# ogulcanaydogan/llm-slo-ebpf-toolkit

Measured on AMD Instinct MI355X. Metric: fault-replay attribution throughput through the agent's BPF-ring -> GPU path (events/s, node-wide); held-out attribution macro-F1 and agent CPU overhead % reported alongside, higher is better.
Workload: dtype fp64 posteriors / fp32 features (exact-int64 time joins)

## Files before the change

llm_slo_ebpf_toolkit_amd/ops/csrc/agent_bindings.cpp:

```cpp
#include <pybind11/numpy.h>
#include <pybind11/pybind11.h>
#include <pybind11/stl.h>

#include <cstring>
#include <memory>
#include <stdexcept>

#include "decodesli.h"
#include "drift.h"
#include "engine.h"
#include "errsli.h"
#include "exemplars.h"
#include "loadsli.h"
#include "satcurve.h"
#include "onset.h"
#include "openreq.h"
#include "podrank.h"
#include "retrsli.h"
#include "slisketch.h"

namespace py = pybind11;
using namespace mislo;

namespace {
// ... 1285 lines not shown
  });
  m.def("loadsli_device_bytes", [](int bins, int64_t span_cap, int group_cap) {
    return loadsli::device_bytes(bins, (int)span_cap, group_cap);
  });
  m.def("loadsli_ring_records_max", [](int bins, int64_t bin_us) { return loadsli::default_ring_records_max(bins, bin_us); });
  py::class_<PyLoadSliTracker>(m, "LoadSliTracker")
      .def(py::init<int, int64_t, int64_t, int64_t, int64_t, int64_t, int64_t, int64_t, int64_t, int64_t, int, int, int64_t,
                    bool>(),
           py::arg("device") = 0, py::arg("bins") = 1024, py::arg("bin_us") = 500000, py::arg("settle_bins") = 30,
           py::arg("recent_bins") = 30, py::arg("min_base_bins") = 60, py::arg("factor_milli") = 1500,
           py::arg("min_requests") = 20, py::arg("min_conc_milli") = 1000, py::arg("span_cap") = 16384,
           py::arg("group_cap") = 64, py::arg("n_buffers") = 3,
           py::arg("ring_records_max") = loadsli::default_ring_records_max(1024, 500000), py::arg("lds") = true)
      .def("step", &PyLoadSliTracker::step, py::arg("spans"), py::arg("cut_ns"), py::arg("n_groups"))
      .def("query", &PyLoadSliTracker::query)
      .def("results", &PyLoadSliTracker::results)
      .def("block", &PyLoadSliTracker::block)
      .def("step_ms", &PyLoadSliTracker::step_ms)
      .def("resident", &PyLoadSliTracker::resident)
      .def("sync", &PyLoadSliTracker::sync)
      .def("close", &PyLoadSliTracker::close);
  m.attr("SATCURVE_ROW_BYTES") = satcurve::kRowBytes;
  m.attr("SATCURVE_STATS") = (int)satcurve::kStats;
  m.attr("SATCURVE_LEVELS") = satcurve::kK;
  m.attr("SATCURVE_LDS_SLOTS") = satcurve::kLdsSlots;
  m.attr("SATCURVE_BINS") = py::make_tuple(satcurve::kMinBins, satcurve::kMaxBins);
  m.attr("SATCURVE_CURVE_RECORDS_MAX") = satcurve::kMaxCurveRecords;
  m.def("satcurve_level", [](int64_t busy_us, int64_t span_us) {
    if (span_us < 1) throw std::invalid_argument("saturation curve level: empty span");
    const uint32_t u = satcurve::u_of(busy_us, span_us);
    return py::make_tuple(u, satcurve::level_of_u(u));
  });
  m.def("satcurve_lower", [](uint32_t level) { return satcurve::lower_u(level); });
  m.def("satcurve_knee", [](py::array_t<uint64_t, py::array::c_style | py::array::forcecast> curve, int64_t budget_ppm,
                            int64_t min_requests) {
    if (curve.size() != satcurve::kK * 2) throw std::invalid_argument("saturation curve knee: the curve is [160, 2]");
    const satcurve::Knee k = satcurve::knee_of(curve.data(), budget_ppm, min_requests);
    return py::make_tuple(k.level, k.n, k.b, k.valid);
  });
  m.def("satcurve_state", [](bool recent_known, uint64_t n_total, int64_t min_requests, bool knee_valid, uint32_t recent_level,
                             uint32_t knee_level) {
    return satcurve::state_of(recent_known, n_total, min_requests, knee_valid, recent_level, knee_level);
  });
  m.def("satcurve_age", [](uint32_t state, uint32_t prev_age) { return satcurve::age_of(state, prev_age); });
  m.def("satcurve_fold", [](int64_t prev, int64_t q_hi, int64_t q_first, uint32_t bins) {
    const satcurve::Fold f = satcurve::fold_of(prev, q_hi, q_first, bins);
    return py::make_tuple(f.first, f.count, f.lo, f.hi);
  });
  m.def("satcurve_layout", [](int group_cap) {
    const satcurve::Layout l = satcurve::layout(group_cap);
    py::dict d;
    d["rows"] = l.rows, d["curve"] = l.curve, d["stats"] = l.stats, d["words"] = l.words;
    return d;
  });
  m.def("satcurve_device_bytes", [](int bins, int64_t span_cap, int group_cap) {
    return satcurve::device_bytes(bins, (int)span_cap, group_cap);
  });
  m.def("satcurve_ring_after", [](uint32_t bins, const std::vector<std::pair<int64_t, int64_t>>& steps, int64_t q_hi, int64_t n) {
    satcurve::RingPopulation p(bins, INT64_MAX);
    for (const auto& s : steps) p.take(s.first, (size_t)s.second);
    return p.after(q_hi, (size_t)n);
  });
  m.def("satcurve_curve_after", [](int64_t epoch_bins, const std::vector<std::pair<int64_t, int64_t>>& steps, int64_t q_hi,
                                   int64_t n) {
    if (epoch_bins < 1) throw std::invalid_argument("saturation curve: epoch_bins");
    satcurve::CurvePopulation p(epoch_bins, INT64_MAX);
    for (const auto& s : steps) p.take(s.first, (size_t)s.second);
    return p.after(q_hi, (size_t)n);
  });
  py::class_<PySaturationTracker>(m, "SaturationTracker")
      .def(py::init<int, int64_t, int64_t, int64_t, int64_t, int64_t, int64_t, int64_t, double, int64_t, int, int, int64_t,
                    int64_t, bool>(),
           py::arg("device") = 0, py::arg("bins") = 1024, py::arg("bin_us") = 500000, py::arg("settle_bins") = 30,
           py::arg("recent_bins") = 30, py::arg("epoch_bins") = 43200, py::arg("budget_ppm") = 10000,
           py::arg("min_requests") = 200, py::arg("slo_ms") = 800.0, py::arg("span_cap") = 16384, py::arg("group_cap") = 64,
           py::arg("n_buffers") = 3, py::arg("ring_records_max") = loadsli::default_ring_records_max(1024, 500000),
           py::arg("curve_records_max") = satcurve::kMaxCurveRecords, py::arg("lds") = true)
      .def("step", &PySaturationTracker::step, py::arg("spans"), py::arg("cut_ns"), py::arg("n_groups"))
      .def("query", &PySaturationTracker::query)
      .def("results", &PySaturationTracker::results)
      .def("block", &PySaturationTracker::block)
      .def("step_ms", &PySaturationTracker::step_ms)
      .def("resident", &PySaturationTracker::resident)
      .def("sync", &PySaturationTracker::sync)
      .def("close", &PySaturationTracker::close);
  m.attr("RETRSLI_K") = retrsli::kK;
  m.attr("RETRSLI_STATS") = (int)retrsli::kStats;
  m.attr("RETRSLI_CELLS") = retrsli::kCells;
  m.attr("RETRSLI_LDS_SLOTS") = retrsli::kLdsSlots;
  m.attr("RETRSLI_UNIT_MAX") = retrsli::kUnitMax;
  m.def("retrsli_units_of_ms", [](float ms) { return retrsli::units_of_ms(ms); });
  m.def("retrsli_budget_units", [](double ms) { return retrsli::budget_units(ms); });
  m.def("retrsli_cell_of", [](bool tb, uint32_t r, uint32_t m_u, uint32_t slo_u, uint32_t budget_u) {
    return retrsli::cell_of(tb, r, m_u, slo_u, budget_u);
  });
  m.def("retrsli_state_of", [](const std::vector<uint32_t>& cells, uint32_t sli, uint32_t min_requests, uint32_t coverage_ppm,
                               uint32_t budget_ppm, uint32_t dominance_ppm) {
    if (cells.size() != (size_t)retrsli::kCells) throw std::invalid_argument("retrieval sli: six cells");
    retrsli::Thresholds th;
    th.min_requests = min_requests;
    th.coverage_ppm = coverage_ppm;
    th.budget_ppm = budget_ppm;
    th.dominance_ppm = dominance_ppm;
    return retrsli::state_of(cells.data(), sli, th);
  });
  m.def("retrsli_age_of", [](uint32_t state, uint32_t prev_state, uint32_t prev_age) {
    return retrsli::age_of(state, prev_state, prev_age);
  });
  m.def("retrsli_layout", [](int group_cap) {
    const retrsli::Layout l = retrsli::layout(group_cap);
    return std::vector<size_t>{l.cells, l.cells_roll, l.sum_r, l.sum_t, l.sum_r_roll, l.sum_t_roll, l.sli, l.sli_roll, l.q_r_win,
                               l.q_r_roll, l.q_m_win, l.q_m_roll, l.state, l.age, l.stats, l.words};
  });
  py::class_<PyRetrievalSliTracker>(m, "RetrievalSliTracker")
      .def(py::init<int, int64_t, int, int, int, double, double, int64_t, int64_t, int64_t, int64_t, bool>(),
           py::arg("device") = 0, py::arg("span_cap") = 16384, py::arg("group_cap") = 64, py::arg("windows") = 150,
           py::arg("n_buffers") = 3, py::arg("slo_ms") = 800.0, py::arg("retrieval_budget_ms") = 200.0,
           py::arg("budget_ppm") = 10000, py::arg("coverage_ppm") = 500000, py::arg("dominance_ppm") = 667000,
           py::arg("min_requests") = 200, py::arg("lds") = true)
      .def("step", &PyRetrievalSliTracker::step, py::arg("spans"), py::arg("n_groups"))
      .def("query", &PyRetrievalSliTracker::query)
      .def("results", &PyRetrievalSliTracker::results)
      .def("block", &PyRetrievalSliTracker::block)
      .def("step_ms", &PyRetrievalSliTracker::step_ms)
      .def("resident", &PyRetrievalSliTracker::resident)
      .def("sync", &PyRetrievalSliTracker::sync)
      .def("close", &PyRetrievalSliTracker::close);
  py::class_<PyEngine>(m, "WindowEngine")
      .def(py::init<int, int, int, int, int, int, int, double, double, int, int, bool, bool, int, float, double, int,
                    int, int, int, int, bool>(),
           py::arg("device") = 0, py::arg("sig_cap") = 1 << 20, py::arg("span_cap") = 16384, py::arg("group_cap") = 64,
           py::arg("user_cap") = 1 << 18, py::arg("n_buffers") = 3, py::arg("max_ahead") = 3,
           py::arg("window_ms") = 2000.0, py::arg("threshold") = 0.7, py::arg("fanout") = 3, py::arg("group_mode") = 1,
           py::arg("use_graphs") = true, py::arg("device_refit") = true, py::arg("n_dom") = 10,
           py::arg("ttft_slo_ms") = 800.0f, py::arg("halo_ms") = 0.0, py::arg("import_cap") = 0,
           py::arg("xchg_cap") = 0, py::arg("shard_rank") = 0, py::arg("shard_world") = 1,
           py::arg("halo_windows") = 3, py::arg("split_rings") = false)
      .def("register_host", &PyEngine::register_host)
      .def("submit", &PyEngine::submit, py::arg("k"), py::arg("kernel"), py::arg("user"), py::arg("spans"),
           py::arg("n_groups"), py::arg("labels") = py::none(), py::arg("bases") = std::vector<int64_t>{},
           py::arg("with_labels") = true, py::arg("learn") = false, py::arg("user_rec") = 64)
      .def("submit_copy", &PyEngine::submit_copy, py::arg("k"), py::arg("kernel"), py::arg("user"), py::arg("spans"),
           py::arg("n_groups"), py::arg("labels") = py::none(), py::arg("bases") = std::vector<int64_t>{},
           py::arg("user_rec") = 64)
      .def("submit_chain", &PyEngine::submit_chain, py::arg("k"), py::arg("n_groups"), py::arg("with_labels") = true,
           py::arg("learn") = false)
      .def("h2d_done", &PyEngine::h2d_done)
      .def("wait_h2d", &PyEngine::wait_h2d)
      .def("query", &PyEngine::query)
      .def("wait", &PyEngine::wait)
      .def("packet", &PyEngine::packet)
      .def("results", &PyEngine::results)
      .def("window_ms", &PyEngine::window_ms)
      .def("copy_ms", [](PyEngine& p, int64_t k) {
        py::gil_scoped_release nogil;
        return p.eng().copy_ms(k);
      })
      .def("set_model_bytes", &PyEngine::set_model_bytes)
      .def("set_app_model", &PyEngine::set_app_model)
      .def("set_p0", &PyEngine::set_p0)
      .def("set_refit", &PyEngine::set_refit, py::arg("alpha") = 2.0, py::arg("prior_pseudo") = 1.0,
           py::arg("inv_temp") = 1.0, py::arg("min_count") = 0.0, py::arg("cap_dom") = -1, py::arg("ceil") = 1.0)
      .def("refit_now", &PyEngine::refit_now)
      .def("set_device_refit", [](PyEngine& p, bool on) { p.eng().set_device_refit(on); })
      .def("score", &PyEngine::score, py::arg("feat"), py::arg("labels") = py::none(), py::arg("app") = py::none())
      .def("set_pods", &PyEngine::set_pods)
      .def("inject_remote", &PyEngine::inject_remote)
      .def("results_all", &PyEngine::results_all)
      .def("set_join_params", &PyEngine::set_join_params)
      .def("init_comm", &PyEngine::init_comm)
      .def("totals", &PyEngine::totals)
      .def("reset_totals", &PyEngine::reset_totals)
      .def("stats_acc", &PyEngine::stats_acc)
      .def("model_bytes", &PyEngine::model_bytes)
      .def("restore", &PyEngine::restore)
      .def("sync", &PyEngine::sync)
      .def("import_state", &PyEngine::import_state)
      .def("sent_block", &PyEngine::sent_block)
      .def("close", &PyEngine::close)
      .def_property_readonly("buffers", &PyEngine::buffers)
      .def_property_readonly("copy_lanes", [](PyEngine& p) { return p.eng().copy_lanes(); })
      .def_property_readonly("copy_ahead", [](PyEngine& p) { return p.eng().copy_ahead(); })
      .def("take_copy_lanes", [](PyEngine& p) {
        py::gil_scoped_release nogil;
        return p.eng().take_copy_lanes();
      })
      .def_property_readonly("windows_folded", &PyEngine::folded)
      .def_property_readonly("graphs", &PyEngine::graphs)
      .def_property_readonly("host_issue_us", &PyEngine::host_issue_us)
      .def_property_readonly("host_wait_us", &PyEngine::host_wait_us)
      .def_property_readonly("host_dma_issue_us", &PyEngine::host_dma_issue_us)
      .def_property_readonly("host_launch_us", &PyEngine::host_launch_us)
      .def_property_readonly("host_pre_us", [](PyEngine& p) { return p.eng().host_pre_us(); })
      .def_property_readonly("host_dma_split_us", [](PyEngine& p) { return p.eng().host_dma_split_us(); })
      .def_property_readonly("host_tail_us", [](PyEngine& p) { return p.eng().host_tail_us(); })
      .def_property_readonly("has_comm", &PyEngine::has_comm)
      .def_property_readonly("rank", [](PyEngine& p) { return p.eng().rank(); })
      .def_property_readonly("world", [](PyEngine& p) { return p.eng().world(); })
      .def_property_readonly("staged_bytes", &PyEngine::staged_bytes)
      .def_property_readonly("direct_bytes", &PyEngine::direct_bytes);
}
```

llm_slo_ebpf_toolkit_amd/ops/csrc/decode.hip:

```cpp
#include "mislo_common.h"
#include "mislo_launch.h"
#include <stdexcept>

namespace mislo {

__constant__ Tables c_tab;

struct DecodeOut {
  SignalCols cols;
  uint32_t* hist;
  uint32_t* status_cnt;
  uint32_t* part_cnt;
  unsigned long long* misc;
  int blk_base = 0;
  uint32_t* sel_cnt = nullptr;
  unsigned long long* sel_mask = nullptr;
  int sel_stride = 0;
};

constexpr int kMiscSums = 2;

template <int NT>
__device__ __forceinline__ void store_counts(const uint32_t* lds, uint32_t* dst) {
  for (int i = threadIdx.x; i < kKeyTypes * kParts; i += NT) dst[i] = lds[i];
}

struct DecodeLds {
  alignas(16) Tables tab;
  static constexpr int kRep = 8, kPartRep = 4;
  static constexpr int kHS = kSlots * kBuckets + 1, kSS = kSlots * 3 + 1, kUS = kSlots + 1;
  static constexpr int kPS = kKeyTypes * kParts + 1;
  uint32_t hist[kRep * kHS];
  uint32_t status[kRep * kSS];
  uint32_t part[kPartRep * kPS];
  unsigned long long sum[kRep * kUS];
};

template <int NT>
__device__ __forceinline__ void lds_init(DecodeLds& L) {
  static_assert(sizeof(Tables) % 4 == 0 && offsetof(Tables, edges) % 16 == 0, "table layout");
  {
    const uint32_t* src = reinterpret_cast<const uint32_t*>(&c_tab);
    uint32_t* dst = reinterpret_cast<uint32_t*>(&L.tab);
    for (int i = threadIdx.x; i < (int)(sizeof(Tables) / 4); i += NT) dst[i] = src[i];
  }
  for (int i = threadIdx.x; i < DecodeLds::kPartRep * DecodeLds::kPS; i += NT) L.part[i] = 0;
  for (int i = threadIdx.x; i < DecodeLds::kRep * DecodeLds::kUS; i += NT) L.sum[i] = 0;
  for (int i = threadIdx.x; i < DecodeLds::kRep * DecodeLds::kHS; i += NT) L.hist[i] = 0;
  for (int i = threadIdx.x; i < DecodeLds::kRep * DecodeLds::kSS; i += NT) L.status[i] = 0;
  __syncthreads();
}

struct LdsLane {
  uint32_t *hist, *status, *part;
  unsigned long long* sum;
  const Tables* tab;
};
__device__ __forceinline__ LdsLane lds_lane(DecodeLds& L) {
  const int r = threadIdx.x & (DecodeLds::kRep - 1), q = threadIdx.x & (DecodeLds::kPartRep - 1);
  return LdsLane{L.hist + r * DecodeLds::kHS, L.status + r * DecodeLds::kSS, L.part + q * DecodeLds::kPS,
                 L.sum + r * DecodeLds::kUS, &L.tab};
}

template <int NT>
__device__ __forceinline__ void lds_flush(DecodeLds& L, const DecodeOut& o, int unsupported, int zero_ts) {
  __syncthreads();
  for (int i = threadIdx.x; i < kSlots * kBuckets; i += NT) {
    uint32_t v = 0;
#pragma unroll
    for (int r = 0; r < DecodeLds::kRep; ++r) v += L.hist[r * DecodeLds::kHS + i];
    if (v) atomicAdd(o.hist + i, v);
  }
  for (int i = threadIdx.x; i < kSlots * 3; i += NT) {
    uint32_t v = 0;
#pragma unroll
    for (int r = 0; r < DecodeLds::kRep; ++r) v += L.status[r * DecodeLds::kSS + i];
    if (v) atomicAdd(o.status_cnt + i, v);
  }
  if (threadIdx.x < kSlots) {
    unsigned long long v = 0;
#pragma unroll
    for (int r = 0; r < DecodeLds::kRep; ++r) v += L.sum[r * DecodeLds::kUS + threadIdx.x];
    if (v) atomicAdd(&o.misc[kMiscSums + threadIdx.x], v);
  }
  uint32_t* dst = o.part_cnt + (size_t)(o.blk_base + blockIdx.x) * kKeyTypes * kParts;
  for (int i = threadIdx.x; i < kKeyTypes * kParts; i += NT) {
    uint32_t v = 0;
#pragma unroll
    for (int q = 0; q < DecodeLds::kPartRep; ++q) v += L.part[q * DecodeLds::kPS + i];
    dst[i] = v;
  }
  for (int off = 32; off > 0; off >>= 1) {
    unsupported += __shfl_xor(unsupported, off);
    zero_ts += __shfl_xor(zero_ts, off);
  }
  if ((threadIdx.x & 63) == 0) {
    if (unsupported) atomicAdd(&o.misc[0], (unsigned long long)unsupported);
    if (zero_ts) atomicAdd(&o.misc[1], (unsigned long long)zero_ts);
  }
}

__device__ __forceinline__ void decode_one(int i, int cap, int64_t ts, float val, int slot,
                                           uint64_t trace_h, uint32_t pod, uint32_t pid, uint32_t svcnode,
                                           uint64_t conn_h, const DecodeOut& o, const LdsLane& l,
                                           int& unsupported, int& zero_ts, bool local, void* rec_dst,
                                           uint64_t* t_range = nullptr) {
  uint8_t st = 0;
  if (slot >= 0 && local) {
    const Tables& t = *l.tab;
    st = val >= t.err[slot] ? 2 : (val >= t.warn[slot] ? 1 : 0);
    const float4* row = reinterpret_cast<const float4*>(t.edges[slot]);
    const float4 r0 = row[0], r1 = row[1], r2 = row[2], r3 = row[3];
    const int b = (val > r0.x) + (val > r0.y) + (val > r0.z) + (val > r0.w) + (val > r1.x) + (val > r1.y) +
                  (val > r1.z) + (val > r1.w) + (val > r2.x) + (val > r2.y) + (val > r2.z) + (val > r2.w) +
                  (val > r3.x) + (val > r3.y) + (val > r3.z);
    atomicAdd(&l.hist[slot * kBuckets + b], 1u);
    atomicAdd(&l.status[slot * 3 + st], 1u);
    const double milli = rint((double)val * 1000.0);
    if (milli > 0.0) atomicAdd(&l.sum[slot], (unsigned long long)milli);
  } else if (slot >= 0) {
    st = val >= l.tab->err[slot] ? 2 : (val >= l.tab->warn[slot] ? 1 : 0);
  } else if (local) {
    ++unsupported;
  }
  o.cols.status[i] = st;
  {
    SigRec r;
    r.ts = ts;
    r.tr = trace_h;
    r.cn = conn_h;
    r.pod = pod;
    r.pid = pid;
    r.sn = svcnode;
    r.val = val;
    r.slot = slot >= 0 ? (uint32_t)slot : kNoSlot;
    const uint4* rs = reinterpret_cast<const uint4*>(&r);
    uint4* rd = static_cast<uint4*>(rec_dst);
#pragma unroll
    for (int q = 0; q < 4; ++q) rd[q] = rs[q];
  }
  const bool joinable = slot >= 0 && ts != 0;
  if (ts == 0 && local) ++zero_ts;
  if (t_range && joinable) {
    t_range[0] = min(t_range[0], ts_image(ts));
    t_range[1] = max(t_range[1], ts_image(ts));
  }
  PartCodes pc;
#pragma unroll
  for (int k = 0; k < kKeyTypes; ++k) {
    const uint64_t h = joinable ? key_hash(k, trace_h, pod, pid, conn_h, svcnode) : 0ull;
    pc.p[k] = h ? (uint16_t)part_of(h) : kNoPart;
    if (h) atomicAdd(&l.part[k * kParts + part_of(h)], 1u);
  }
  o.cols.part[i] = pc;
}

template <int NT>
__global__ __launch_bounds__(NT) void k_decode_events(const Event* __restrict__ ev, const int* __restrict__ n_ptr,
                                                      int cap, DecodeOut o) {
  __shared__ DecodeLds L;
  lds_init<NT>(L);
  const LdsLane l = lds_lane(L);

  const int n = min(*n_ptr, cap);
  const int n_local = n_ptr[3] > 0 ? min(n_ptr[3], n) : n;
  const int chunk = (n + gridDim.x - 1) / gridDim.x;
  const int beg = blockIdx.x * chunk, end = min(n, beg + chunk);
  int unsupported = 0, zero_ts = 0;
  for (int i = beg + threadIdx.x; i < end; i += NT) {
    const Event e = ev[i];
    const int st = e.signal_type;
    const int slot = st < kMaxTypes ? (int)L.tab.type_slot[st] : -1;
    const float val = slot >= 0 ? (float)((double)e.value * (double)L.tab.scale[slot]) : (float)e.value;
    const uint64_t ch = e.conn_h ? e.conn_h : conn_hash(e.src_port, e.dst_port, e.dst_ip);
    const uint32_t svcnode = ((uint32_t)e.svc_id << 16) | e.node_id;
    decode_one(i, cap, e.ts_ns, val, slot, e.trace_h, e.pod_id, e.pid, svcnode, ch, o, l, unsupported, zero_ts, i < n_local, o.cols.rec + i);
  }
  lds_flush<NT>(L, o, unsupported, zero_ts);
}

__device__ __forceinline__ bool shard_owns(uint32_t svcnode, int rank, int world) {
  if (world <= 1) return true;
  const uint32_t svc = svcnode >> 16;
  return (svc ? (int)((svc - 1u) % (uint32_t)world) : 0) == rank;
}

__device__ __forceinline__ uint64_t wire_trace(const EventC16& e) { return (uint64_t)(e.trace_id & kTraceIdMask); }
__device__ __forceinline__ int64_t wire_ts(const EventC16& e, const int64_t* base) {
  return e.ts_off == kTsZero ? 0 : base[e.trace_id >> kEpochTagShift] + (int64_t)e.ts_off;
}

template <int NT, class Rec>
__global__ __launch_bounds__(NT) void k_decode_wire(const Rec* __restrict__ ev, const int* __restrict__ n_ptr,
                                                    int cap, const uint4* __restrict__ ctx_tab, int n_ctx,
                                                    DecodeOut o) {
  __shared__ DecodeLds L;
  lds_init<NT>(L);
  const LdsLane l = lds_lane(L);

  const int n = min(*n_ptr, cap);
  const int n_local = n_ptr[3] > 0 ? min(n_ptr[3], n) : n;
  auto base_at = [&](int lo) { return (int64_t)(((uint64_t)(uint32_t)n_ptr[lo + 1] << 32) | (uint32_t)n_ptr[lo]); };
  const int64_t t_base[4] = {base_at(4), base_at(8), base_at(10), base_at(12)};
  if (n_ptr[6] > 0) n_ctx = min(n_ptr[6], n_ctx);
  const int chunk = (n + gridDim.x - 1) / gridDim.x;
  const int beg = blockIdx.x * chunk, end = min(n, beg + chunk);
  int unsupported = 0, zero_ts = 0;
  auto ctx_of = [&](const Rec& r) {
    const uint32_t cid = r.ctx_type >> 8;
    return cid < (uint32_t)n_ctx ? ctx_tab[cid] : make_uint4(0u, 0u, 0u, 0u);
  };
  __shared__ uint4 s_stage[NT * 5];
  const int lane = threadIdx.x & 63, wbase = threadIdx.x & ~63;
  const int trips = end > beg ? (end - beg + NT - 1) / NT : 0;
  int i = beg + threadIdx.x;
  Rec e_nx{};
  uint4 cx_nx = make_uint4(0u, 0u, 0u, 0u);
  if (i < end) {
    e_nx = ev[i];
    cx_nx = ctx_of(e_nx);
  }
  for (int it = 0; it < trips; ++it, i += NT) {
    const Rec e = e_nx;
    const uint4 cx = cx_nx;
    if (i + NT < end) {
      e_nx = ev[i + NT];
      cx_nx = ctx_of(e_nx);
    }
    if (i < end) {
      const int st = (int)(e.ctx_type & 0xFFu);
      const int slot = st < kMaxTypes ? (int)L.tab.type_slot[st] : -1;
      const float val = (float)((double)e.value_milli * 1e-3);
      const int64_t ts = wire_ts(e, t_base);
      const uint64_t tr = wire_trace(e);
      decode_one(i, cap, ts, val, slot, tr, cx.x, cx.y, cx.w, (uint64_t)cx.z, o, l, unsupported, zero_ts,
                 i < n_local, &s_stage[threadIdx.x * 5]);
    }
    __syncthreads();
    const int first = i - lane;
    const int nv = min(64, end - first);
    if (nv > 0) {
      const uint4* src = &s_stage[wbase * 5];
      uint4* dst = reinterpret_cast<uint4*>(o.cols.rec + first);
#pragma unroll
      for (int j = 0; j < 4; ++j) {
        const int q = lane + 64 * j;
        if ((q >> 2) < nv) dst[q] = src[(q >> 2) * 5 + (q & 3)];
      }
    }
    __syncthreads();
  }
  lds_flush<NT>(L, o, unsupported, zero_ts);
}


__global__ __launch_bounds__(256) void k_ring_defs(const uint8_t* __restrict__ framed, const int* __restrict__ n_ptr,
                                                   uint4* __restrict__ ctx_tab, uint32_t ctx_rows,
                                                   const uint32_t* __restrict__ pod_sn, uint32_t n_pods, TraceIds tt,
                                                   uint32_t* __restrict__ rs) {
  const int n = n_ptr[15];
  uint32_t foreign = 0, dctx = 0, dtr = 0, disc = 0, busy = 0xFFFFFFFFu;
  constexpr int kU = 4;
  const int stride = gridDim.x * 256;
  for (int i0 = blockIdx.x * 256 + threadIdx.x; i0 < n; i0 += stride * kU) {
    uint2 h[kU], a[kU], b[kU];
#pragma unroll
    for (int u = 0; u < kU; ++u) {
      const int i = i0 + u * stride;
      if (i < n) {
        const uint2* sl = reinterpret_cast<const uint2*>(framed + slot_off(i));
        h[u] = *reinterpret_cast<const uint2*>(framed + rec_off(i));
        a[u] = sl[0];
        b[u] = sl[1];
      } else {
        h[u] = make_uint2(kRecPayload, 0u);
        a[u] = b[u] = make_uint2(0u, 0u);
      }
    }
#pragma unroll
    for (int u = 0; u < kU; ++u) {
      const int i = i0 + u * stride;
      if (i >= n) continue;
      if (h[u].x & kRbBusy) {
        busy = min(busy, (uint32_t)i);
        continue;
      }
      if ((h[u].x & ~(kRbBusy | kRbDiscard)) != kRecPayload) {
        foreign += (i & 7) == 0;
        continue;
      }
      if (h[u].x & kRbDiscard) {
        disc += (i & 7) == 0;
        continue;
      }
      const uint32_t type = a[u].y & 0xFFu;
      if (type == kDefCtx) {
        const uint32_t id = a[u].y >> 8;
        if (id && id < ctx_rows) {
          ctx_tab[id] = make_uint4(b[u].x, b[u].y, a[u].x, b[u].x < n_pods ? pod_sn[b[u].x] : 0u);
          ++dctx;
        }
      } else if (type == kDefTrace) {
        const unsigned long long hash = (unsigned long long)b[u].x | ((unsigned long long)b[u].y << 32);
        if (hash && a[u].x && a[u].x < tt.n) {
          tt.hash[a[u].x] = hash;
          ++dtr;
        }
      }
    }
  }
  for (int off = 32; off > 0; off >>= 1) {
    foreign += __shfl_xor(foreign, off);
    dctx += __shfl_xor(dctx, off);
    dtr += __shfl_xor(dtr, off);
    disc += __shfl_xor(disc, off);
    busy = min(busy, (uint32_t)__shfl_xor((int)busy, off));
  }
  __shared__ uint32_t s_acc[5];
  if (threadIdx.x < 5) s_acc[threadIdx.x] = threadIdx.x == 0 ? 0xFFFFFFFFu : 0u;
  __syncthreads();
  if ((threadIdx.x & 63) == 0) {
    if (busy != 0xFFFFFFFFu) atomicMin(&s_acc[0], busy);
    if (foreign) atomicAdd(&s_acc[1], foreign);
    if (dctx) atomicAdd(&s_acc[2], dctx);
    if (dtr) atomicAdd(&s_acc[3], dtr);
    if (disc) atomicAdd(&s_acc[4], disc);
  }
  __syncthreads();
  if (threadIdx.x == 0) {
    if (s_acc[0] != 0xFFFFFFFFu) atomicMin(&rs[kRsFirstBusy], s_acc[0]);
    if (s_acc[1]) atomicAdd(&rs[kRsForeign], s_acc[1]);
    if (s_acc[2]) atomicAdd(&rs[kRsDefCtx], s_acc[2]);
    if (s_acc[3]) atomicAdd(&rs[kRsDefTrace], s_acc[3]);
    if (s_acc[4]) atomicAdd(&rs[kRsDiscard], s_acc[4]);
  }
}

template <int NT>
__global__ __launch_bounds__(NT) void k_decode_window(const uint8_t* __restrict__ framed,
                                                      const Event* __restrict__ user, const int* __restrict__ n_ptr,
                                                      const int* __restrict__ rows, int cap,
                                                      const SigRec* __restrict__ imp,
                                                      const uint4* __restrict__ ctx_tab, int n_ctx, TraceIds tt,
                                                      uint32_t* __restrict__ rs, unsigned long long* __restrict__ tmax,
                                                      const uint32_t* __restrict__ pod_sn, uint32_t n_pods, int seg,
                                                      int sh_rank, int sh_world, DecodeOut o) {
  __shared__ DecodeLds L;
  __shared__ uint32_t s_cnt2[3];
  __shared__ unsigned long long s_t[3];
  if (threadIdx.x == 0) {
    s_cnt2[0] = s_cnt2[1] = s_cnt2[2] = 0u;
    s_t[0] = 0ull;
    s_t[1] = ~0ull;
    s_t[2] = 0ull;
  }
  lds_init<NT>(L);
  const LdsLane l = lds_lane(L);
  const int r0 = min(rows[0], cap);
  const int seg_beg = seg ? r0 : 0;
  const int n = seg ? max(r0, min(rows[1], cap)) : r0;
  const int n_loc = min(n_ptr[0], r0);
  const int n_k = min(n_ptr[15], n_loc);
  const int user_rec = n_ptr[6];
  const int valid_k = min((int)min((uint32_t)n_k, rs[kRsFirstBusy]), n_k);
  auto base_at = [&](int lo) { return (int64_t)(((uint64_t)(uint32_t)n_ptr[lo + 1] << 32) | (uint32_t)n_ptr[lo]); };
  const int64_t t_base[4] = {base_at(4), base_at(8), base_at(10), base_at(12)};
  const int64_t u_base = max(max(t_base[0], t_base[1]), max(t_base[2], t_base[3]));
  const int chunk = (n - seg_beg + gridDim.x - 1) / gridDim.x;
  const int beg = seg_beg + blockIdx.x * chunk, end = min(n, beg + chunk);
  int unsupported = 0, zero_ts = 0, events = 0, other = 0;
  uint32_t n_sel = 0;
  unsigned long long t_hi = 0;
  uint64_t tr[2] = {~0ull, 0ull};
  const uint32_t cur = cur_slot(o.cols);
  SigRec* const rec_out = o.cols.rec + (size_t)cur * (size_t)o.cols.stride;
  __shared__ uint4 s_stage[NT * 5];
  const int lane = threadIdx.x & 63, wbase = threadIdx.x & ~63;
  const int trips = end > beg ? (end - beg + NT - 1) / NT : 0;
  int i = beg + threadIdx.x;
  for (int it = 0; it < trips; ++it, i += NT) {
    if (i < end) {
      if (i >= n_loc) {
        const SigRec& m = imp[i - n_loc];
        decode_one(i, cap, m.ts, m.val, m.slot == kNoSlot ? -1 : (int)m.slot, m.tr, m.pod, m.pid, m.sn, m.cn, o, l,
                   unsupported, zero_ts, false, &s_stage[threadIdx.x * 5], tr);
      } else if (i < n_k) {
        const uint2 h = *reinterpret_cast<const uint2*>(framed + rec_off(i));
        const uint2* sl = reinterpret_cast<const uint2*>(framed + slot_off(i));
        const uint2 a = sl[0], b = sl[1];
        const EventC16 e{a.x, a.y, b.x, b.y};
        bool ok = i < valid_k && h.x == kRecPayload && (e.ctx_type & 0xFFu) < kDefFirst;
        const uint32_t cid = e.ctx_type >> 8;
        uint4 cx = ok && cid < (uint32_t)n_ctx ? ctx_tab[cid] : make_uint4(0u, 0u, 0u, 0u);
        const uint32_t sn_now = cx.x < n_pods ? pod_sn[cx.x] : 0u;
        if (sn_now) cx.w = sn_now;
        if (ok && !shard_owns(cx.w, sh_rank, sh_world)) {
          ok = false;
          ++other;
        }
        if (ok) {
          const int st = (int)(e.ctx_type & 0xFFu);
          const int slot = st < kMaxTypes ? (int)L.tab.type_slot[st] : -1;
          const int64_t ts = wire_ts(e, t_base);
          decode_one(i, cap, ts, (float)((double)e.value_milli * 1e-3), slot, trace_of(tt, (uint32_t)wire_trace(e)),
                     cx.x, cx.y, cx.w, (uint64_t)cx.z, o, l, unsupported, zero_ts, true, &s_stage[threadIdx.x * 5], tr);
          if (slot >= 0 && ts > 0) t_hi = max(t_hi, (unsigned long long)ts);
          ++events;
        } else {
          decode_one(i, cap, 0, 0.f, -1, 0, 0, 0, 0, 0, o, l, unsupported, zero_ts, false, &s_stage[threadIdx.x * 5], tr);
        }
      } else if (user_rec == 16) {
        const int j = i - n_k;
        const uint4 u = reinterpret_cast<const uint4*>(user)[j];
        const uint32_t pod = u.w & 0xFFFFFu;
        const uint32_t sn = pod < n_pods ? pod_sn[pod] : 0u;
        if (u.z == kUser16Cont) {
          decode_one(i, cap, 0, 0.f, -1, 0, 0, 0, 0, 0, o, l, unsupported, zero_ts, false, &s_stage[threadIdx.x * 5], tr);
        } else if (!shard_owns(sn, sh_rank, sh_world)) {
          ++other;
          decode_one(i, cap, 0, 0.f, -1, 0, 0, 0, 0, 0, o, l, unsupported, zero_ts, false, &s_stage[threadIdx.x * 5], tr);
        } else {
          uint64_t trh = 0;
          if ((u.z & kUser16Trace) && i + 1 < n_loc) {
            const uint4 c = reinterpret_cast<const uint4*>(user)[j + 1];
            if (c.z == kUser16Cont) trh = ((uint64_t)c.y << 32) | c.x;
          }
          const uint32_t ps = u.z & ~kUser16Trace;
          const int st = (int)((ps >> 22) & 0x7Fu);
          const int slot = (int)L.tab.type_slot[st];
          const int64_t ts = user24_ts(u.x, u.w, ps, u_base);
          decode_one(i, cap, ts, (float)((double)u.y * 1e-3), slot, trh, pod, ps & 0x3FFFFFu, sn, 0ull, o, l,
                     unsupported, zero_ts, true, &s_stage[threadIdx.x * 5], tr);
          if (slot >= 0 && ts > 0) t_hi = max(t_hi, (unsigned long long)ts);
          ++events;
        }
      } else if (user_rec == 24) {
        const uint2* u = reinterpret_cast<const uint2*>(reinterpret_cast<const uint8_t*>(user) + (size_t)(i - n_k) * 24);
        const uint2 a = u[0], b = u[1], c = u[2];
        const int st = (int)((c.x >> 22) & 0x7Fu);
        const int slot = (int)L.tab.type_slot[st];
        const uint32_t pod = c.y & 0xFFFFFu;
        const uint32_t sn = pod < n_pods ? pod_sn[pod] : 0u;
        const int64_t ts = user24_ts(b.y, c.y, c.x, u_base);
        if (!shard_owns(sn, sh_rank, sh_world)) {
          ++other;
          decode_one(i, cap, 0, 0.f, -1, 0, 0, 0, 0, 0, o, l, unsupported, zero_ts, false, &s_stage[threadIdx.x * 5], tr);
        } else {
        decode_one(i, cap, ts, (float)((double)b.x * 1e-3), slot, ((uint64_t)a.y << 32) | a.x, pod, c.x & 0x3FFFFFu, sn,
                   0ull, o, l, unsupported, zero_ts, true, &s_stage[threadIdx.x * 5], tr);
        if (slot >= 0 && ts > 0) t_hi = max(t_hi, (unsigned long long)ts);
        ++events;
        }
      } else if (user_rec == 32) {
        const User32 e = reinterpret_cast<const User32*>(user)[i - n_k];
        const int st = e.signal_type;
        const int slot = st < kMaxTypes ? (int)L.tab.type_slot[st] : -1;
        const uint32_t sn = e.pod_id < n_pods ? pod_sn[e.pod_id] : 0u;
        if (!shard_owns(sn, sh_rank, sh_world)) {
          ++other;
          decode_one(i, cap, 0, 0.f, -1, 0, 0, 0, 0, 0, o, l, unsupported, zero_ts, false, &s_stage[threadIdx.x * 5], tr);
        } else {
        decode_one(i, cap, e.ts_ns, (float)((double)e.value_milli * 1e-3), slot, e.trace_h, e.pod_id, e.pid, sn, 0ull,
                   o, l, unsupported, zero_ts, true, &s_stage[threadIdx.x * 5], tr);
        if (slot >= 0 && e.ts_ns > 0) t_hi = max(t_hi, (unsigned long long)e.ts_ns);
        ++events;
        }
      } else {
        const Event e = user[i - n_k];
        const int st = e.signal_type;
        const int slot = st < kMaxTypes ? (int)L.tab.type_slot[st] : -1;
        const float val = slot >= 0 ? (float)((double)e.value * (double)L.tab.scale[slot]) : (float)e.value;
        const uint64_t ck = e.conn_h ? e.conn_h : conn_hash(e.src_port, e.dst_port, e.dst_ip);
        const uint32_t svcnode = ((uint32_t)e.svc_id << 16) | e.node_id;
        if (!shard_owns(svcnode, sh_rank, sh_world)) {
          ++other;
          decode_one(i, cap, 0, 0.f, -1, 0, 0, 0, 0, 0, o, l, unsupported, zero_ts, false, &s_stage[threadIdx.x * 5], tr);
        } else {
          decode_one(i, cap, e.ts_ns, val, slot, e.trace_h, e.pod_id, e.pid, svcnode, conn32(ck), o, l, unsupported,
                     zero_ts, true, &s_stage[threadIdx.x * 5], tr);
          if (slot >= 0 && e.ts_ns > 0) t_hi = max(t_hi, (unsigned long long)e.ts_ns);
          ++events;
        }
      }
    }
    __syncthreads();
    if (o.sel_mask) {
      bool sel = false;
      if (i < end && i < n_loc) {
        const SigRec& r = *reinterpret_cast<const SigRec*>(&s_stage[threadIdx.x * 5]);
        sel = r.slot != kNoSlot && r.ts != 0 && r.tr != 0 && (r.val >= L.tab.err[r.slot] || r.val >= L.tab.warn[r.slot]);
      }
      const unsigned long long m = __ballot(sel);
      if (lane == 0) {
        o.sel_mask[(size_t)blockIdx.x * o.sel_stride + (size_t)it * (NT / 64) + (threadIdx.x >> 6)] = m;
        n_sel += (uint32_t)__popcll(m);
      }
    }
    const int first = i - lane;
    const int nv = min(64, end - first);
    if (nv > 0) {
      const uint4* src = &s_stage[wbase * 5];
      uint4* dst = reinterpret_cast<uint4*>(rec_out + first);
#pragma unroll
      for (int j = 0; j < 4; ++j) {
        const int q = lane + 64 * j;
        if ((q >> 2) < nv) dst[q] = src[(q >> 2) * 5 + (q & 3)];
      }
    }
    __syncthreads();
  }
  for (int off = 32; off > 0; off >>= 1) {
    events += __shfl_xor(events, off);
    other += __shfl_xor(other, off);
    t_hi = max(t_hi, (unsigned long long)__shfl_xor((long long)t_hi, off));
    tr[0] = min(tr[0], (uint64_t)__shfl_xor((long long)tr[0], off));
    tr[1] = max(tr[1], (uint64_t)__shfl_xor((long long)tr[1], off));
  }
  if ((threadIdx.x & 63) == 0) {
    if (events) atomicAdd(&s_cnt2[0], (uint32_t)events);
    if (other) atomicAdd(&s_cnt2[1], (uint32_t)other);
    if (n_sel) atomicAdd(&s_cnt2[2], n_sel);
    if (t_hi) atomicMax(&s_t[0], t_hi);
    if (tr[0] <= tr[1]) {
      atomicMin(&s_t[1], (unsigned long long)tr[0]);
      atomicMax(&s_t[2], (unsigned long long)tr[1]);
    }
  }
  lds_flush<NT>(L, o, unsupported, zero_ts);
  if (threadIdx.x == 0) {
    if (s_cnt2[0]) atomicAdd(&rs[kRsEvents], s_cnt2[0]);
    if (s_cnt2[1]) atomicAdd(&rs[kRsOtherShard], s_cnt2[1]);
    if (o.sel_cnt) o.sel_cnt[blockIdx.x] = s_cnt2[2];
    if (s_t[0]) atomicMax(tmax, s_t[0]);
    if (o.cols.gen && s_t[1] <= s_t[2]) {
      atomicMin(reinterpret_cast<unsigned long long*>(&o.cols.gen->tlo[cur]), s_t[1]);
      atomicMax(reinterpret_cast<unsigned long long*>(&o.cols.gen->thi[cur]), s_t[2]);
    }
  }
}

template <int NT>
__global__ __launch_bounds__(NT) void k_decode_ref(const RefEvent* __restrict__ ev, const int* __restrict__ n_ptr,
                                                   int cap, uint32_t pod, uint32_t svcnode, uint64_t trace_h,
                                                   DecodeOut o) {
  __shared__ DecodeLds L;
  lds_init<NT>(L);
  const LdsLane l = lds_lane(L);
  const int n = min(*n_ptr, cap);
  const int n_local = n_ptr[3] > 0 ? min(n_ptr[3], n) : n;
  const int chunk = (n + gridDim.x - 1) / gridDim.x;
  const int beg = blockIdx.x * chunk, end = min(n, beg + chunk);
  int unsupported = 0, zero_ts = 0;
  for (int i = beg + threadIdx.x; i < end; i += NT) {
    const RefEvent e = ev[i];
    const uint32_t st = e.signal_type;
    int slot = (st >= 1 && st <= 9) ? (int)L.tab.type_slot[st] : -1;
    float val;
    if (st == 2 || st == 6) val = (float)e.value_ns;
    else val = (float)((double)e.value_ns / 1e6);
    const uint64_t ch = conn_hash(e.conn_src_port, e.conn_dst_port, e.conn_dst_ip);
    decode_one(i, cap, (int64_t)e.timestamp_ns, val, slot, trace_h, pod, e.pid, svcnode, ch, o, l, unsupported, zero_ts, i < n_local, o.cols.rec + i);
  }
  lds_flush<NT>(L, o, unsupported, zero_ts);
}

constexpr int kSliLds = 1024;

template <int NT>
__global__ __launch_bounds__(NT) void k_decode_spans(const void* __restrict__ sp_raw, const int* __restrict__ n_ptr,
                                                     int cap, SpanCols c, uint32_t* part_cnt,
                                                     const uint4* __restrict__ ctx_tab, int n_ctx, SpanMap sm) {
  const Span* __restrict__ sp = static_cast<const Span*>(sp_raw);
  const SpanC20* __restrict__ sp20 = static_cast<const SpanC20*>(sp_raw);
  const bool compact = n_ptr[6] == 20;
  if (n_ptr[5] > 0) n_ctx = min(n_ptr[5], n_ctx);
  __shared__ uint32_t s_part[kKeyTypes * kParts];
  __shared__ uint32_t s_sli[2 * kSliLds];
  __shared__ uint32_t s_app[2 * kSliLds];
  __shared__ uint32_t s_late[kSliLds];
  const bool sli_lds = sm.grp_sli && sm.n_groups <= kSliLds;
  const bool app_lds = sm.grp_app && sm.n_groups <= kSliLds;
  for (int i = threadIdx.x; i < kKeyTypes * kParts; i += NT) s_part[i] = 0;
  if (sli_lds)
    for (int i = threadIdx.x; i < 2 * sm.n_groups; i += NT) s_sli[i] = 0;
  if (app_lds)
    for (int i = threadIdx.x; i < 2 * sm.n_groups; i += NT) s_app[i] = 0;
  const bool late_lds = sm.grp_late && sm.n_groups <= kSliLds;
  if (late_lds)
    for (int i = threadIdx.x; i < sm.n_groups; i += NT) s_late[i] = 0;
  __syncthreads();
  const int n = min(*n_ptr, cap);
  const int chunk = (n + gridDim.x - 1) / gridDim.x;
  const int beg = blockIdx.x * chunk, end = min(n, beg + chunk);
  uint64_t t_lo = ~0ull, t_hi = 0ull;
  for (int i = beg + threadIdx.x; i < end; i += NT) {
    SpanRec r;
    if (compact) {
      const SpanC20 s = sp20[i];
      const uint4 cx = s.ctx_id < (uint32_t)n_ctx ? ctx_tab[s.ctx_id] : make_uint4(0u, 0u, 0u, 0u);
      r.ts = s.ts_ns;
      r.tr = s.trace_id;
      r.cn = cx.z;
      r.pod = cx.x;
      r.pid = cx.y;
      r.sn = cx.w;
      r.grp = s.group_id;
      if (sm.sh_world > 1) {
        if (r.grp % (uint32_t)sm.sh_world != (uint32_t)sm.sh_rank) r.ts = 0;
        r.grp /= (uint32_t)sm.sh_world;
      }
    } else {
      const Span s = sp[i];
      r.ts = s.ts_ns;
      r.tr = s.trace_h;
      r.cn = sm.native ? (uint64_t)conn32(s.conn_h) : s.conn_h;
      uint32_t grp = s.group_id;
      bool mine = true;
      if (sm.sh_world > 1) {
        mine = grp % (uint32_t)sm.sh_world == (uint32_t)sm.sh_rank;
        grp /= (uint32_t)sm.sh_world;
        if (!mine) r.ts = 0;
      }
      if (mine && sm.grp_sli && grp < (uint32_t)sm.n_groups && !(s.flags & kSpanNoSli)) {
        const bool breach = s.ttft_ms > sm.ttft_slo_ms;
        if (breach && (s.flags & kSpanLate) && sm.grp_late) {
          if (late_lds) atomicAdd(&s_late[grp], 1u);
          else atomicAdd(&sm.grp_late[2 * grp], 1u);
        } else {
          uint32_t* sli = sli_lds ? s_sli : sm.grp_sli;
          atomicAdd(&sli[2 * grp], 1u);
          if (breach) atomicAdd(&sli[2 * grp + 1], 1u);
        }
      }
      if (mine && sm.grp_app && grp < (uint32_t)sm.n_groups && s.retr_ms > 0.f && s.retr_ms < 1e7f) {
        uint32_t* app = app_lds ? s_app : sm.grp_app;
        atomicAdd(&app[2 * grp], 1u);
        atomicAdd(&app[2 * grp + 1], (uint32_t)rint((double)s.retr_ms * kAppUnitsPerMs));
      }
      r.pod = s.pod_id;
      r.pid = s.pid;
      r.sn = ((uint32_t)s.svc_id << 16) | s.node_id;
      r.grp = grp;
    }
    c.rec[i] = r;
    if (r.ts != 0) {
      t_lo = min(t_lo, ts_image(r.ts));
      t_hi = max(t_hi, ts_image(r.ts));
    }
    PartCodes pc;
#pragma unroll
    for (int k = 0; k < kKeyTypes; ++k) {
      const uint64_t h = r.ts != 0 ? key_hash(k, r.tr, r.pod, r.pid, r.cn, r.sn) : 0ull;
      pc.p[k] = h ? (uint16_t)part_of(h) : kNoPart;
      if (h) atomicAdd(&s_part[k * kParts + part_of(h)], 1u);
    }
    c.part[i] = pc;
  }
  if (sm.gen) {
    for (int off = 32; off > 0; off >>= 1) {
      t_lo = min(t_lo, (uint64_t)__shfl_xor((long long)t_lo, off));
      t_hi = max(t_hi, (uint64_t)__shfl_xor((long long)t_hi, off));
    }
    if ((threadIdx.x & 63) == 0 && t_lo <= t_hi) {
      atomicMin(reinterpret_cast<unsigned long long*>(&sm.gen->span_lo), (unsigned long long)t_lo);
      atomicMax(reinterpret_cast<unsigned long long*>(&sm.gen->span_hi), (unsigned long long)t_hi);
    }
  }
  __syncthreads();
  store_counts<NT>(s_part, part_cnt + (size_t)blockIdx.x * kKeyTypes * kParts);
  if (sli_lds)
    for (int i = threadIdx.x; i < 2 * sm.n_groups; i += NT)
      if (s_sli[i]) atomicAdd(&sm.grp_sli[i], s_sli[i]);
  if (app_lds)
    for (int i = threadIdx.x; i < 2 * sm.n_groups; i += NT)
      if (s_app[i]) atomicAdd(&sm.grp_app[i], s_app[i]);
  if (late_lds)
    for (int i = threadIdx.x; i < sm.n_groups; i += NT)
      if (s_late[i]) atomicAdd(&sm.grp_late[2 * i], s_late[i]);
}

constexpr int kDecodeNT = 1024;

int decode_sel_stride(int cap) {
  const long long g = decode_grid(cap), chunk = ((long long)cap + g - 1) / g;
  return (int)((chunk + kDecodeNT - 1) / kDecodeNT) * (kDecodeNT / 64);
}

int decode_grid(int cap) {
  long long g = ((long long)cap + 1023) / 1024;
  if (g < 1) g = 1;
  if (g > kPartBlocks) g = kPartBlocks;
  return (int)g;
}

void set_tables(const Tables* host_tables) {
  (void)hipMemcpyToSymbol(HIP_SYMBOL(c_tab), host_tables, sizeof(Tables), 0, hipMemcpyHostToDevice);
}

void launch_decode_events(const void* ev, const int* n_dev, int cap, const SignalCols& cols, uint32_t* hist,
                          uint32_t* status_cnt, uint32_t* part_cnt, unsigned long long* misc, hipStream_t stream) {
  DecodeOut o{cols, hist, status_cnt, part_cnt, misc};
  constexpr int NT = kDecodeNT;
  hipLaunchKernelGGL((k_decode_events<NT>), dim3(decode_grid(cap)), dim3(NT), 0, stream,
                     (const Event*)ev, n_dev, cap, o);
}

void launch_decode_wire(const void* ev, const int* n_dev, int cap, const uint32_t* ctx_tab, int n_ctx,
                        const SignalCols& cols, uint32_t* hist, uint32_t* status_cnt, uint32_t* part_cnt,
                        unsigned long long* misc, hipStream_t stream) {
  DecodeOut o{cols, hist, status_cnt, part_cnt, misc};
  constexpr int NT = kDecodeNT;
  hipLaunchKernelGGL((k_decode_wire<NT, EventC16>), dim3(decode_grid(cap)), dim3(NT), 0, stream,
                     (const EventC16*)ev, n_dev, cap, reinterpret_cast<const uint4*>(ctx_tab), n_ctx, o);
}

void launch_decode_ref(const void* ev, const int* n_dev, int cap, uint32_t pod, uint32_t svcnode, uint64_t trace_h,
                       const SignalCols& cols, uint32_t* hist, uint32_t* status_cnt, uint32_t* part_cnt,
                       unsigned long long* misc, hipStream_t stream) {
  DecodeOut o{cols, hist, status_cnt, part_cnt, misc};
  constexpr int NT = kDecodeNT;
  hipLaunchKernelGGL((k_decode_ref<NT>), dim3(decode_grid(cap)), dim3(NT), 0, stream,
                     (const RefEvent*)ev, n_dev, cap, pod, svcnode, trace_h, o);
}

void launch_decode_spans(const void* sp, const int* n_dev, int cap, const SpanCols& cols, uint32_t* part_cnt,
                         const uint32_t* ctx_tab, int n_ctx, hipStream_t stream, const SpanMap* sm) {
  constexpr int NT = 1024;
  SpanMap m{};
  if (sm) m = *sm;
  hipLaunchKernelGGL((k_decode_spans<NT>), dim3(decode_grid(cap)), dim3(NT), 0, stream, sp, n_dev, cap, cols,
                     part_cnt, reinterpret_cast<const uint4*>(ctx_tab), n_ctx, m);
}

void launch_ring_defs(const uint8_t* framed, const int* n_dev, int cap, uint32_t* ctx_tab, uint32_t ctx_rows,
                      const uint32_t* pod_sn, uint32_t n_pods, const TraceIds& tt, uint32_t* ring_state,
                      hipStream_t stream) {
  int g = (cap + 1023) / 1024;
  g = g < 1 ? 1 : (g > 2048 ? 2048 : g);
  hipLaunchKernelGGL(k_ring_defs, dim3(g), dim3(256), 0, stream, framed, n_dev, reinterpret_cast<uint4*>(ctx_tab),
                     ctx_rows, pod_sn, n_pods, tt, ring_state);
}

void launch_decode_window(const uint8_t* framed, const void* user, const int* n_dev, const int* rows, int cap,
                          const SigRec* imp, const uint32_t* ctx_tab, int n_ctx, const TraceIds& tt,
                          uint32_t* ring_state, unsigned long long* tmax, const uint32_t* pod_sn, uint32_t n_pods,
                          const SignalCols& cols, uint32_t* hist, uint32_t* status_cnt, uint32_t* part_cnt,
                          unsigned long long* misc, hipStream_t stream, int seg, int grid, int blk_base, int sh_rank,
                          int sh_world, uint32_t* sel_cnt, unsigned long long* sel_mask, int sel_stride) {
  if (sel_mask != nullptr && (grid != 0 || sel_stride != decode_sel_stride(cap)))
    throw std::invalid_argument("launch_decode_window: the fused selection needs the default decode grid");
  DecodeOut o{cols, hist, status_cnt, part_cnt, misc, blk_base, sel_cnt, sel_mask, sel_stride};
  constexpr int NT = kDecodeNT;
  hipLaunchKernelGGL((k_decode_window<NT>), dim3(grid > 0 ? grid : decode_grid(cap)), dim3(NT), 0, stream, framed,
                     (const Event*)user, n_dev, rows, cap, imp, reinterpret_cast<const uint4*>(ctx_tab), n_ctx, tt,
                     ring_state, tmax, pod_sn, n_pods, seg, sh_rank, sh_world, o);
}

}
```

llm_slo_ebpf_toolkit_amd/ops/csrc/engine.h:

```cpp
#pragma once

#include <hip/hip_runtime.h>
#include <rccl/rccl.h>

#include <map>
#include <tuple>
#include <type_traits>
#include <vector>

#include "copylanes.h"
#include "mislo_launch.h"
#include "mislo_packet.h"

namespace mislo {

constexpr uint32_t kCtxRows = 1u << 24;
constexpr uint32_t kPodRows = 1u << 20;
constexpr uint32_t kTraceIdRows = 1u << 24;
constexpr int kHeadBytes = 64;

struct Seg {
  const void* ptr;
  size_t bytes;
};

struct EngineConfig {
  int device = 0;
  int sig_cap = 1 << 20, span_cap = 16384, group_cap = 64;
  int user_cap = 1 << 18;
  int n_buffers = 3, max_ahead = 3;
  double window_ms = 2000.0, threshold = 0.7;
  int fanout = 3, group_mode = 1;
  bool use_graphs = true;
  bool device_refit = true;
  double alpha = 2.0, prior_pseudo = 1.0;
  double inv_temp = 1.0, min_count = 0.0;
  int cap_dom = -1;
  double lik_ceil = 1.0;
  int n_dom = 10;
  float ttft_slo_ms = 800.0f;
  double halo_ms = 0.0;
  int halo_windows = 3;
  int import_cap = 0;
  int xchg_cap = 0;
  int shard_rank = 0, shard_world = 1;
  bool split_rings = false;
};

template <class Byte>
struct ResultViewT {
  template <class T>
  using P = std::conditional_t<std::is_const_v<Byte>, const T, T>*;
  P<double> post;
  P<double> gconf;
  P<float> feat;
  P<int32_t> pred;
  P<uint32_t> evbits;
  P<uint32_t> sli;
  P<uint32_t> app;
  P<uint32_t> late;
};
using ResultView = ResultViewT<const uint8_t>;

struct ResultLayout {
  size_t G;
  size_t gconf() const { return 16 * G * 8; }
  size_t feat() const { return gconf() + G * 8; }
  size_t pred() const { return feat() + 16 * G * 4; }
  size_t evbits() const { return pred() + G * 4; }
  size_t sli() const { return evbits() + 16 * G * 4; }
  size_t bytes() const { return sli() + 6 * G * 4; }
  template <class Byte>
  ResultViewT<Byte> view(Byte* r) const {
    ResultViewT<Byte> v;
    auto set = [r](auto& p, size_t off) { p = reinterpret_cast<std::remove_reference_t<decltype(p)>>(r + off); };
    set(v.post, 0), set(v.gconf, gconf()), set(v.feat, feat()), set(v.pred, pred()), set(v.evbits, evbits());
    set(v.sli, sli()), set(v.app, sli() + 2 * G * 4), set(v.late, sli() + 4 * G * 4);
    return v;
  }
};

struct WindowInput {
  std::vector<Seg> kernel;
  std::vector<Seg> user;
  int user_rec = 64;
  std::vector<Seg> spans;
  int n_groups = 0;
  const int32_t* labels = nullptr;
  int64_t bases[4] = {0, 0, 0, 0};
};

class WindowEngine {
 public:
  explicit WindowEngine(const EngineConfig& cfg);
  ~WindowEngine();
  WindowEngine(const WindowEngine&) = delete;
  WindowEngine& operator=(const WindowEngine&) = delete;

  const EngineConfig& config() const { return cfg_; }
  int buffers() const { return nb_; }

  bool register_host(const void* ptr, size_t bytes);
  void submit(int64_t k, const WindowInput& in, bool with_labels, bool learn);
  void submit_copy(int64_t k, const WindowInput& in);
  void submit_chain(int64_t k, int n_groups, bool with_labels, bool learn);
  bool copy_ahead() const { return copy_ahead_; }
  bool h2d_done(int64_t k);
  void wait_h2d(int64_t k);
  int copy_lanes() const { return lanes_; }
  bool take_copy_lanes();
  bool query(int64_t k);
  void wait(int64_t k);
  const double* packet(int64_t k) const { return bufs_[k % nb_].packet_host; }
  ResultView results(int64_t k) const { return layout().view<const uint8_t>(bufs_[k % nb_].res_host); }
  ResultLayout layout() const { return ResultLayout{(size_t)cfg_.group_cap}; }
  std::pair<float, float> window_ms(int64_t k);
  std::vector<float> copy_ms(int64_t k);

  void set_model_bytes(const void* bytes, size_t n);
  void set_refit(double alpha, double prior_pseudo, double inv_temp, double min_count, int cap_dom = -1,
                 double ceil = 1.0);
  void refit_now();
  void set_device_refit(bool on) { cfg_.device_refit = on; }
  void score_features(const float* feat, int n, const int32_t* labels, double* post, int32_t* pred, double* conf,
                      uint32_t* evbits, uint32_t* confusion, const uint32_t* app_cnt = nullptr);
  void set_app_model(const void* bytes, size_t n);
  void set_p0(const double* p0, size_t n);
  void set_pods(const uint32_t* pods, const uint32_t* svcnode, size_t n);
  void inject_remote(const void* blocks, size_t stride, int world, int me);
  void set_join_params(double window_ms, double threshold, int fanout, int group_mode);
  void init_comm(const ncclUniqueId& id, int rank, int world);
  bool has_comm() const { return comm_ != nullptr; }
  int rank() const { return rank_; }
  int world() const { return world_; }
  const uint8_t* results_all(int64_t k) const { return comm_ ? bufs_[k % nb_].res_all_host : bufs_[k % nb_].res_host; }
  size_t result_bytes() const { return layout().bytes(); }

  void totals(double* out);
  void reset_totals();
  void stats_acc(double* out);
  void restore(const double* stats, const void* model, size_t model_bytes, int64_t folded);
  void model_bytes(void* out);
  void sync();
  std::vector<int64_t> import_state();
  std::vector<uint8_t> sent_block();
  int64_t windows_folded() const { return folded_; }
  size_t staged_bytes() const { return staged_bytes_; }
  size_t direct_bytes() const { return direct_bytes_; }
  size_t graphs() const { return graphs_.size(); }
  double host_issue_us() const { return issue_n_ ? issue_us_ / issue_n_ : 0.0; }
  double host_wait_us() const { return issue_n_ ? wait_us_ / issue_n_ : 0.0; }
  double host_dma_issue_us() const { return issue_n_ ? dma_us_ / issue_n_ : 0.0; }
  double host_launch_us() const { return issue_n_ ? launch_us_ / issue_n_ : 0.0; }
  double host_pre_us() const { return issue_n_ ? pre_us_ / issue_n_ : 0.0; }
  double host_tail_us() const { return issue_n_ ? tail_us_ / issue_n_ : 0.0; }

 private:
  int rec_shard_rank() const { return cfg_.split_rings ? 0 : cfg_.shard_rank; }
  int rec_shard_world() const { return cfg_.split_rings ? 1 : cfg_.shard_world; }
  struct Buf;
  enum class Stage : int { Window, Records, Join, XchgSpans, XchgHead, Front, Back };
  static constexpr int kStageSlots = 8;
  void alloc();
  void enable_span_branch();
  void run_begin(const Buf& buf, hipStream_t st);
  void run_part1(const Buf& buf, hipStream_t st, bool xchg);
  void run_join_front(const Buf& buf, hipStream_t st, bool xchg);
  void run_join_back(const Buf& buf, int n_groups, bool with_labels, bool learn, hipStream_t st);
  void run_span_branch(const Buf& buf, hipStream_t st);
  void run_spans(const Buf& buf, hipStream_t st);
  void launch_part(Stage part, const Buf& buf, int n_groups, bool with_labels, bool learn);
  void merge_remote(const Buf& buf, const uint8_t* blocks, size_t stride, int world, int me, hipStream_t st);
  void refit(const double* add);
  SignalCols sig_cols(const Buf& buf) const;
  SpanCols span_cols(const Buf& buf) const;
  bool registered(const void* p, size_t n) const;
  size_t dma(const std::vector<Seg>& segs, uint8_t* dst, size_t cap, uint8_t*& staging, size_t& st_off,
             hipStream_t st);
  struct Owner {
    std::vector<hipEvent_t> events;
    std::vector<void*> dev, host;
    std::vector<hipStream_t> streams;
    void free_dev(void* p);
    ~Owner();
  } own_;
  template <class T>
  T* dalloc(size_t n, bool zero = false);
  void* host_alloc(size_t bytes, unsigned flags);
  void* host_block(size_t bytes);
  hipEvent_t mk_event(unsigned flags);
  hipStream_t mk_stream(bool high_priority = false);

  EngineConfig cfg_;
  int nb_, max_ahead_;
  size_t off_kern_ = 0, off_user_ = 0, off_span_ = 0, in_bytes_ = 0;
  size_t kern_bytes() const { return (size_t)kRecStride * (((size_t)cfg_.sig_cap + kBatchSlots - 1) / kBatchSlots); }
  std::vector<std::pair<const uint8_t*, size_t>> registered_;
  size_t staged_bytes_ = 0, direct_bytes_ = 0;
  uint32_t *pod_sn_ = nullptr, *pod_host_ = nullptr;
  unsigned long long* trace_hash_ = nullptr;
  AppModel* app_dev_ = nullptr;
  int n_rows_ = 0;
  int gens_ = 1;
  int slots_ = 1;
  unsigned long long* tmax_ = nullptr;
  KeyTs* g_keys_ = nullptr;
  uint32_t *remote_n_ = nullptr, *sel_cnt_ = nullptr, *sel_off_ = nullptr;
  unsigned long long* sel_mask_ = nullptr;
  int sel_stride_ = 0;
  uint8_t *xsend_ = nullptr, *xrecv_ = nullptr;
  size_t xstride_ = 0, xrecv_bytes_ = 0;
  int nblk_imp_ = 0;
  bool spin_ = false;
  std::vector<uint8_t> inject_;
  size_t inject_stride_ = 0;
  int inject_world_ = 0, inject_me_ = 0;
  int rank_ = 0, world_ = 1;
  hipStream_t side_ = nullptr;
  hipStream_t front_ = nullptr;
  bool overlap_ = false;
  struct BufSet {
    GenMeta* gen;
    int* rows;
    uint32_t *ring_state, *hist, *status, *confusion, *cnt, *gcnt;
    unsigned long long *misc, *dbg, *top3, *gsum;
    double *stats, *stats_count;
    SpanRec* s_rec;
    PartCodes* s_part;
    uint32_t *s_items, *s_part_base, *probe_work;
    PreSpan* s_pre;
  };
  std::vector<BufSet> sets_;
  struct Buf {
    int b;
    uint8_t* in;
    uint8_t* head_host;
    uint8_t* staging;
    double *packet_dev, *packet_host;
    uint8_t *res_dev, *res_host;
    uint8_t *res_all_dev, *res_all_host;
    ResultViewT<uint8_t> res;
    SigRec* imp;
    uint32_t* remote_n;
    const BufSet* set;
    const GenMeta* gen_prev;
    hipEvent_t head_done, front_done, compute_done, comm_done, xchg_done;
    hipEvent_t t_comp0, t_comp1, t_end;
    const int* counts() const { return reinterpret_cast<const int*>(in); }
  };
  std::vector<Buf> bufs_;
  struct CopyMark {
    hipEvent_t t_start, h2d_done;
  };
  std::vector<CopyMark> marks_;
  const CopyMark& mark(int64_t k) const { return marks_[copy_mark_slot(k, nb_)]; }
  hipEvent_t ev_fork_ = nullptr, ev_sigbase_ = nullptr, ev_spans_ = nullptr;
  bool branch_ = false;
  bool xspan_ = false;
  bool exchange() const { return comm_ && cfg_.xchg_cap > 0 && cfg_.import_cap > 0; }
  JoinParams jp_{};
  int nblk_sig_ = 1, nblk_span_ = 1;
  hipStream_t copy_[kMaxCopyLanes] = {nullptr, nullptr};
  int lanes_ = 1;
  bool copy_ahead_ = false;
  bool lane_on_request_ = false;
  bool copy_open_ = false;
  int copy_groups_ = 0;
  int64_t copied_windows() const { return submitted_ + (copy_open_ ? 1 : 0); }
  CopiedUpTo copied_;
  bool copied_ready(int64_t w, bool block);
  hipStream_t compute_ = nullptr, comm_stream_ = nullptr;
  ncclComm_t comm_ = nullptr;
  ncclComm_t xcomm_ = nullptr;
  uint32_t* ctx_tab_ = nullptr;
  double *totals_ = nullptr, *stats_acc_ = nullptr, *p0_ = nullptr;
  uint8_t* model_dev_ = nullptr;
  std::vector<uint8_t*> model_host_;
  int model_slot_ = 0;
  uint8_t* g_status_ = nullptr;
  PartCodes* g_part_ = nullptr;
  uint32_t *g_part_blk_ = nullptr, *g_part_off_ = nullptr, *g_part_tot_ = nullptr, *g_part_base_ = nullptr,
           *g_items_ = nullptr;
  SigRec* g_rec_ = nullptr;
  uint32_t *s_part_blk_ = nullptr, *s_part_off_ = nullptr, *s_part_tot_ = nullptr;
  float *attrs_ = nullptr, *conf_ = nullptr, *kernel_ms_ = nullptr;
  std::map<std::tuple<int, int, bool, bool>, hipGraphExec_t> graphs_;
  std::vector<bool> warm_;
  std::vector<hipGraph_t> graph_defs_;
  int64_t submitted_ = 0, folded_ = 0;
  double issue_us_ = 0, wait_us_ = 0, dma_us_ = 0, launch_us_ = 0, pre_us_ = 0, tail_us_ = 0;
  double split_us_[4] = {0, 0, 0, 0};

 public:
  std::vector<double> host_dma_split_us() const {
    std::vector<double> v;
    for (double x : split_us_) v.push_back(issue_n_ ? x / issue_n_ : 0.0);
    return v;
  }

 private:
  int64_t issue_n_ = 0;
};

void engine_set_tables(const Tables& t);

}
```

llm_slo_ebpf_toolkit_amd/ops/csrc/engine.hip:

```cpp
#include "engine.h"
#include "mislo_packet_kernels.h"

#include <algorithm>
#include <chrono>
#include <cstdlib>
#include <cmath>
#include <cstring>
#include <stdexcept>
#include <string>

namespace mislo {

namespace {

#define HIPCHECK(x)                                                                                  \
  do {                                                                                               \
    hipError_t _e = (x);                                                                             \
    if (_e != hipSuccess) throw std::runtime_error(std::string("HIP error: ") + hipGetErrorString(_e) + \
                                                   " at " #x);                                       \
  } while (0)

#define NCCLCHECK(x)                                                                                        \
  do {                                                                                                      \
    ncclResult_t _r = (x);                                                                                  \
// ... 15 lines not shown
                                                    const unsigned long long* misc, const unsigned long long* dbg,
                                                    const uint32_t* confusion, const double* stats, const double* count,
                                                    const uint32_t* ring, double* __restrict__ packet,
                                                    double* __restrict__ totals, double* __restrict__ packet_host,
                                                    const uint4* __restrict__ res, uint4* __restrict__ res_host,
                                                    size_t res16) {
  const size_t t = blockIdx.x * (size_t)blockDim.x + threadIdx.x, stride = (size_t)gridDim.x * blockDim.x;
  if (t < (size_t)kPacketLen) {
    const double v = packet_value((int)t, hist, status, misc, dbg, confusion, stats, count, ring);
    packet[t] = v;
    totals[t] += v;
    packet_host[t] = v;
  }
  for (size_t i = t; i < res16; i += stride) res_host[i] = res[i];
}

__global__ void k_to_host(const uint4* __restrict__ src, uint4* __restrict__ dst, size_t n16) {
  for (size_t i = blockIdx.x * (size_t)blockDim.x + threadIdx.x; i < n16; i += (size_t)gridDim.x * blockDim.x)
    dst[i] = src[i];
}

void to_host(const void* src, void* dst, size_t bytes, hipStream_t st) {
  const size_t n16 = (bytes + 15) / 16;
  const int g = (int)std::min<size_t>(64, (n16 + 255) / 256);
  hipLaunchKernelGGL(k_to_host, dim3(g > 0 ? g : 1), dim3(256), 0, st, static_cast<const uint4*>(src),
                     static_cast<uint4*>(dst), n16);
}

constexpr int kCopyAheadDefault = 1;
constexpr unsigned kEvWait = hipEventDisableTiming | hipEventBlockingSync;
int env_int(const char* name, int unset) {
  const char* v = getenv(name);
  return v ? atoi(v) : unset;
}

struct Lap {
  using clock = std::chrono::steady_clock;
  clock::time_point t = clock::now();
  void operator()(double& acc) {
    const auto n = clock::now();
    acc += std::chrono::duration<double, std::micro>(n - t).count();
    t = n;
  }
};

}

void engine_set_tables(const Tables& t) { set_tables(&t); }

template <class T>
T* WindowEngine::dalloc(size_t n, bool zero) {
  void* p = nullptr;
  HIPCHECK(hipMalloc(&p, n * sizeof(T) + 64));
  own_.dev.push_back(p);
  if (zero) HIPCHECK(hipMemset(p, 0, n * sizeof(T)));
  return static_cast<T*>(p);
}

void* WindowEngine::host_alloc(size_t bytes, unsigned flags) {
  void* h = nullptr;
  HIPCHECK(hipHostMalloc(&h, bytes, flags));
  own_.host.push_back(h);
  return h;
}

void* WindowEngine::host_block(size_t bytes) {
  void* h = host_alloc((bytes + 15) & ~size_t(15), hipHostMallocCoherent | hipHostMallocMapped);
  std::memset(h, 0, bytes);
  return h;
}

hipEvent_t WindowEngine::mk_event(unsigned flags) {
  hipEvent_t e;
  HIPCHECK(hipEventCreateWithFlags(&e, flags));
  own_.events.push_back(e);
  return e;
}

hipStream_t WindowEngine::mk_stream(bool high_priority) {
  hipStream_t s;
  int lo = 0, hi = 0;
  if (high_priority) {
    HIPCHECK(hipDeviceGetStreamPriorityRange(&lo, &hi));
    HIPCHECK(hipStreamCreateWithPriority(&s, hipStreamNonBlocking, hi));
  } else {
    HIPCHECK(hipStreamCreateWithFlags(&s, hipStreamNonBlocking));
  }
  own_.streams.push_back(s);
  return s;
}

void WindowEngine::Owner::free_dev(void* p) {
  if (!p) return;
  dev.erase(std::find(dev.begin(), dev.end(), p));
  HIPCHECK(hipFree(p));
}

WindowEngine::Owner::~Owner() {
  for (hipEvent_t e : events) (void)hipEventDestroy(e);
  for (void* p : host) (void)hipHostFree(p);
  for (void* p : dev) (void)hipFree(p);
  for (hipStream_t s : streams) (void)hipStreamDestroy(s);
}

WindowEngine::WindowEngine(const EngineConfig& cfg) : cfg_(cfg) {
  if (cfg.sig_cap <= 0 || cfg.span_cap <= 0 || cfg.group_cap <= 0 || cfg.group_cap > 4096)
    throw std::invalid_argument("capacities out of range");
  if (cfg.sig_cap >= (1 << 27)) throw std::invalid_argument("sig_cap must be < 2^27 (top-3 key packing)");
  nb_ = std::max(2, cfg.n_buffers);
  max_ahead_ = std::min(nb_, std::max(1, cfg.max_ahead));
  if (cfg.user_cap <= 0 || cfg.user_cap > cfg.sig_cap) throw std::invalid_argument("user_cap must be in [1, sig_cap]");
  if (cfg.import_cap < 0 || cfg.xchg_cap < 0 || cfg.halo_ms < 0) throw std::invalid_argument("negative import sizes");
  if (cfg.halo_windows < 1 || cfg.halo_windows >= kMaxGens)
    throw std::invalid_argument("halo_windows must be in [1, 3] (resident generations)");
  gens_ = cfg.halo_ms > 0 ? 1 + cfg.halo_windows : 1;
  if (2LL * gens_ * ((long long)cfg.sig_cap + cfg.import_cap) >= (1LL << 27))
    throw std::invalid_argument("2 x generations x (sig_cap + import_cap) must be < 2^27 (top-3 key packing)");
  HIPCHECK(hipSetDevice(cfg.device));
  set_join_params(cfg.window_ms, cfg.threshold, cfg.fanout, cfg.group_mode);
  alloc();
}

void WindowEngine::set_join_params(double window_ms, double threshold, int fanout, int group_mode) {
  const int64_t ms = 1000000;
  int64_t outer = (int64_t)llround(window_ms * ms);
  if (outer <= 0) outer = 2000 * ms;
  if (outer >= (1LL << 35)) throw std::invalid_argument("window too large for top-3 key packing (< 34 s)");
  jp_.outer_ns = outer;
  const int64_t tw[4] = {outer, 100 * ms, 250 * ms, 500 * ms};
  for (int k = 0; k < 4; ++k) jp_.win_ns[k] = std::min(outer, tw[k]);
  const float cf[4] = {1.0f, 0.9f, 0.8f, 0.65f};
  for (int k = 0; k < 4; ++k) jp_.conf[k] = cf[k];
  jp_.threshold = threshold > 0 ? (float)threshold : 0.7f;
  if (fanout <= 0) fanout = 3;
  if (fanout > 3) throw std::invalid_argument("GPU join keeps at most 3 candidates per span");
  jp_.fanout = fanout;
  jp_.group_mode = group_mode;
  graphs_.clear();
}

void WindowEngine::alloc() {
  const int64_t S = cfg_.span_cap, G = cfg_.group_cap;
  n_rows_ = cfg_.sig_cap + cfg_.import_cap;
  const int64_t N = n_rows_;
  nblk_sig_ = decode_grid((int)N);
  nblk_span_ = decode_grid((int)S);
  const bool one_stream = env_int("MISLO_ONE_STREAM", 0) == 1;
  compute_ = mk_stream();
  copy_[0] = one_stream ? compute_ : mk_stream();
  spin_ = env_int("MISLO_SPIN_WAIT", 0) == 1;
  overlap_ = env_int("MISLO_WINDOW_OVERLAP", !one_stream) == 1 && !one_stream &&
             !(cfg_.xchg_cap > 0 && cfg_.import_cap > 0);
  if (overlap_) front_ = mk_stream();
  copy_ahead_ = overlap_ && env_int("MISLO_COPY_AHEAD", kCopyAheadDefault) == 1;
  const char* lanes_env = getenv("MISLO_COPY_LANES");
  lanes_ = overlap_ && (lanes_env ? atoi(lanes_env) == 2 : nb_ >= 4) ? 2 : 1;
  lane_on_request_ = copy_ahead_ && !lanes_env && lanes_ == 1 && nb_ >= 3;
  copy_[1] = lanes_ == 2 ? mk_stream(env_int("MISLO_COPY_LANE_PRIO", 1) != 0) : copy_[0];
  slots_ = gens_ + (overlap_ ? 1 : 0);
  {
    if (env_int("MISLO_SPAN_STREAM", !one_stream && !overlap_) == 1) enable_span_branch();
  }
  comm_stream_ = compute_;
  const size_t head = (kHeadBytes + 4 * (size_t)G + 63) & ~size_t(63);
  off_kern_ = head;
  off_user_ = (off_kern_ + kern_bytes() + 63) & ~size_t(63);
  off_span_ = off_user_ + 64 * (size_t)cfg_.user_cap;
  in_bytes_ = off_span_ + 64 * (size_t)S;
  const ResultLayout lay = layout();
  bufs_.assign(nb_, Buf{});
  for (Buf& buf : bufs_) {
    buf.in = dalloc<uint8_t>(in_bytes_, true);
    buf.head_host = static_cast<uint8_t*>(host_block(head));
    buf.packet_dev = dalloc<double>(kPacketLen, true);
    buf.packet_host = static_cast<double*>(host_block(kPacketLen * sizeof(double)));
    for (hipEvent_t* e : {&buf.head_done, &buf.compute_done, &buf.comm_done, &buf.front_done, &buf.xchg_done})
      *e = mk_event(kEvWait);
    for (hipEvent_t* e : {&buf.t_comp0, &buf.t_comp1, &buf.t_end}) *e = mk_event(hipEventDefault);
    buf.res_host = static_cast<uint8_t*>(host_block(lay.bytes()));
    buf.res_dev = dalloc<uint8_t>(lay.bytes(), true);
    buf.res = lay.view(buf.res_dev);
    buf.imp = cfg_.import_cap ? dalloc<SigRec>(cfg_.import_cap) : nullptr;
  }
  marks_.assign((size_t)copy_mark_slots(nb_), CopyMark{});
  for (CopyMark& m : marks_) {
    m.t_start = mk_event(hipEventDefault);
    m.h2d_done = mk_event(hipEventBlockingSync);
  }
  warm_.assign(kStageSlots * nb_, false);
  pod_sn_ = dalloc<uint32_t>(kPodRows, true);
  pod_host_ = static_cast<uint32_t*>(host_alloc(kPodRows * 4, hipHostMallocDefault));
  std::memset(pod_host_, 0, kPodRows * 4);
  trace_hash_ = dalloc<unsigned long long>(kTraceIdRows, true);
  tmax_ = dalloc<unsigned long long>(1, true);
  remote_n_ = dalloc<uint32_t>(nb_, true);
  for (int i = 0; i < (overlap_ ? nb_ : 1); ++i) {
    BufSet s{};
    s.rows = dalloc<int>(16, true);
    s.ring_state = dalloc<uint32_t>(kRsLen);
    s.gen = dalloc<GenMeta>(1);
    GenMeta g{};
    g.cur = (uint32_t)slots_ - 1;
    for (int a = 0; a < kMaxGens; ++a) g.cut[a] = INT64_MAX;
    HIPCHECK(hipMemcpy(s.gen, &g, sizeof(g), hipMemcpyHostToDevice));
    s.s_part = dalloc<PartCodes>(S);
    s.s_part_base = dalloc<uint32_t>(kKeyTypes * kParts + 1);
    s.s_items = dalloc<uint32_t>(kKeyTypes * S);
    s.s_pre = dalloc<PreSpan>((size_t)kKeyTypes * S);
    s.s_rec = dalloc<SpanRec>(S);
    s.probe_work = dalloc<uint32_t>(kProbeWorkLen, true);
    s.top3 = dalloc<unsigned long long>(3 * S);
    s.cnt = dalloc<uint32_t>(S);
    s.gsum = dalloc<unsigned long long>((size_t)kGroupStripes * G * kSlots);
    s.gcnt = dalloc<uint32_t>((size_t)kGroupStripes * G * kSlots);
    s.hist = dalloc<uint32_t>(kSlots * kBuckets);
    s.status = dalloc<uint32_t>(kSlots * 3);
    s.misc = dalloc<unsigned long long>(kPacketMisc);
    s.dbg = dalloc<unsigned long long>(kPacketDbg);
    s.confusion = dalloc<uint32_t>(kMaxDomains * kMaxDomains);
    s.stats = dalloc<double>(32 * 32);
    s.stats_count = dalloc<double>(kMaxDomains);
    sets_.push_back(s);
  }
  for (int b = 0; b < nb_; ++b) {
    bufs_[b].b = b;
    bufs_[b].set = &sets_[overlap_ ? b : 0];
    bufs_[b].gen_prev = sets_[overlap_ ? (b + nb_ - 1) % nb_ : 0].gen;
    bufs_[b].remote_n = remote_n_ + b;
  }
  sel_cnt_ = dalloc<uint32_t>(1024);
  sel_off_ = dalloc<uint32_t>(1024);
  xstride_ = sizeof(XRec) * (1 + (size_t)cfg_.xchg_cap);
  if (cfg_.xchg_cap) {
    xsend_ = dalloc<uint8_t>(xstride_, true);
    if (env_int("MISLO_SEL_TWO_PASS", 0) != 1) {
      sel_stride_ = decode_sel_stride(n_rows_);
      sel_mask_ = dalloc<unsigned long long>((size_t)decode_grid(n_rows_) * (size_t)sel_stride_);
    }
  }
  ctx_tab_ = dalloc<uint32_t>((size_t)kCtxRows * 4, true);
  totals_ = dalloc<double>(kPacketLen, true);
  stats_acc_ = dalloc<double>(kStatsLen, true);
  p0_ = dalloc<double>(2 * kSlots * 16, true);
  model_dev_ = dalloc<uint8_t>(sizeof(PosteriorModel), true);
  app_dev_ = dalloc<AppModel>(1, true);
  for (int i = 0; i < max_ahead_ + 2; ++i)
    model_host_.push_back(static_cast<uint8_t*>(host_alloc(sizeof(PosteriorModel), hipHostMallocDefault)));
  g_status_ = dalloc<uint8_t>(N);
  g_part_ = dalloc<PartCodes>(N);
  nblk_imp_ = cfg_.xchg_cap ? decode_grid(7 * cfg_.xchg_cap) : 0;
  g_part_blk_ = dalloc<uint32_t>((size_t)(nblk_sig_ + nblk_imp_) * kKeyTypes * kParts);
  g_part_off_ = dalloc<uint32_t>((size_t)(nblk_sig_ + nblk_imp_) * kKeyTypes * kParts);
  g_part_tot_ = dalloc<uint32_t>(kKeyTypes * kParts);
  g_part_base_ = dalloc<uint32_t>((size_t)slots_ * kBaseLen);
  g_items_ = dalloc<uint32_t>((size_t)slots_ * kKeyTypes * N);
  g_keys_ = dalloc<KeyTs>((size_t)slots_ * kKeyTypes * N);
  g_rec_ = dalloc<SigRec>((size_t)slots_ * N);
  s_part_blk_ = dalloc<uint32_t>((size_t)nblk_span_ * kKeyTypes * kParts);
  s_part_off_ = dalloc<uint32_t>((size_t)nblk_span_ * kKeyTypes * kParts);
  s_part_tot_ = dalloc<uint32_t>(kKeyTypes * kParts);
  attrs_ = dalloc<float>(S * kSlots);
  conf_ = dalloc<float>(S);
  kernel_ms_ = dalloc<float>(S);
  HIPCHECK(hipDeviceSynchronize());
}

WindowEngine::~WindowEngine() {
  (void)hipDeviceSynchronize();
  for (auto& kv : graphs_) (void)hipGraphExecDestroy(kv.second);
  for (auto g : graph_defs_) (void)hipGraphDestroy(g);
  if (xcomm_) ncclCommDestroy(xcomm_);
  if (comm_) ncclCommDestroy(comm_);
  for (auto& r : registered_) (void)hipHostUnregister(const_cast<uint8_t*>(r.first));
}

void WindowEngine::enable_span_branch() {
  if (branch_) return;
  side_ = mk_stream(env_int("MISLO_SPAN_STREAM_PRIO", 0) == 1);
  for (hipEvent_t* e : {&ev_fork_, &ev_sigbase_, &ev_spans_}) *e = mk_event(hipEventDisableTiming);
  xspan_ = env_int("MISLO_XCHG_SPAN_SIDE", 1) != 0;
  branch_ = true;
}

SignalCols WindowEngine::sig_cols(const Buf& buf) const {
  return SignalCols{g_rec_, g_status_, g_part_, g_items_, g_keys_, g_part_base_, buf.set->gen, (int64_t)n_rows_, gens_,
                    slots_};
}
SpanCols WindowEngine::span_cols(const Buf& buf) const { return SpanCols{buf.set->s_rec, buf.set->s_part}; }

bool WindowEngine::register_host(const void* ptr, size_t bytes) {
  if (!ptr || !bytes) return false;
  if (registered(ptr, bytes)) return true;
  if (hipHostRegister(const_cast<void*>(ptr), bytes, hipHostRegisterDefault) != hipSuccess) {
    (void)hipGetLastError();
    return false;
  }
  registered_.emplace_back(static_cast<const uint8_t*>(ptr), bytes);
  return true;
}

bool WindowEngine::registered(const void* p, size_t n) const {
  const uint8_t* q = static_cast<const uint8_t*>(p);
  for (const auto& r : registered_)
    if (q >= r.first && q + n <= r.first + r.second) return true;
  return false;
}

size_t WindowEngine::dma(const std::vector<Seg>& segs, uint8_t* dst, size_t cap, uint8_t*& staging, size_t& st_off,
                         hipStream_t st) {
  size_t off = 0;
  for (const Seg& s : segs) {
    if (!s.bytes) continue;
    if (off + s.bytes > cap) throw std::invalid_argument("window input exceeds the engine's capacity");
    const void* src = s.ptr;
    if (!registered(s.ptr, s.bytes)) {
      if (!staging) staging = static_cast<uint8_t*>(host_alloc(in_bytes_ - off_kern_, hipHostMallocDefault));
      std::memcpy(staging + st_off, s.ptr, s.bytes);
      src = staging + st_off;
      st_off += s.bytes;
      staged_bytes_ += s.bytes;
    } else {
      direct_bytes_ += s.bytes;
    }
    HIPCHECK(hipMemcpyAsync(dst + off, src, s.bytes, hipMemcpyHostToDevice, st));
    off += s.bytes;
  }
  return off;
}

bool WindowEngine::copied_ready(int64_t w, bool block) {
  const hipEvent_t ev = mark(w).h2d_done;
  if (block) {
    HIPCHECK(hipEventSynchronize(ev));
    return true;
  }
  const hipError_t e = hipEventQuery(ev);
  if (e == hipErrorNotReady) return false;
  HIPCHECK(e);
  return true;
}

bool WindowEngine::h2d_done(int64_t k) {
  if (k < 0 || k >= copied_windows()) return false;
  return copied_.done(k, lanes_, [this](int64_t w) { return copied_ready(w, false); });
}

void WindowEngine::wait_h2d(int64_t k) {
  if (k < 0 || k >= copied_windows()) throw std::invalid_argument("wait_h2d: the window has not been submitted");
  copied_.done(k, lanes_, [this](int64_t w) { return copied_ready(w, true); });
}

void WindowEngine::run_begin(const Buf& buf, hipStream_t st) {
  const BufSet& s = *buf.set;
  const int S = cfg_.span_cap, G = cfg_.group_cap;
  FillList fl{};
  auto add = [&](void* p, size_t bytes, uint32_t v) { fl.seg[fl.count++] = FillSeg{(uint32_t*)p, (uint32_t)(bytes / 4), v}; };
  add(s.hist, kSlots * kBuckets * 4, 0);
  add(s.status, kSlots * 3 * 4, 0);
  add(s.misc, kPacketMisc * 8, 0);
  add(s.dbg, kPacketDbg * 8, 0);
  add(s.confusion, kMaxDomains * kMaxDomains * 4, 0);
  add(s.stats, 32 * 32 * 8, 0);
  add(s.stats_count, kMaxDomains * 8, 0);
  add(s.top3, 3 * (size_t)S * 8, 0xFFFFFFFFu);
  add(s.cnt, (size_t)S * 4, 0);
  add(s.gsum, (size_t)kGroupStripes * G * kSlots * 8, 0);
  add(s.gcnt, (size_t)kGroupStripes * G * kSlots * 4, 0);
  add(buf.res.sli, (size_t)G * 6 * 4, 0);
  launch_window_begin(fl, s.gen, buf.gen_prev, tmax_, gens_, slots_, (long long)llround(cfg_.halo_ms * 1e6),
                      s.ring_state, buf.remote_n, buf.counts(), n_rows_, s.rows, st);
}

void WindowEngine::run_part1(const Buf& buf, hipStream_t st, bool xchg) {
  const BufSet& s = *buf.set;
  const int* counts = buf.counts();
  const int N = n_rows_;
  if (!(xchg && xspan_)) run_begin(buf, st);
  if (branch_ && !xchg) run_span_branch(buf, st);
  const TraceIds tt{trace_hash_, kTraceIdRows};
  launch_ring_defs(buf.in + off_kern_, counts, cfg_.sig_cap, ctx_tab_, kCtxRows, pod_sn_, kPodRows, tt, s.ring_state,
                   st);
  const bool fused_sel = xchg && sel_mask_;
  launch_decode_window(buf.in + off_kern_, buf.in + off_user_, counts, s.rows, N, buf.imp, ctx_tab_, (int)kCtxRows, tt,
                       s.ring_state, tmax_, pod_sn_, kPodRows, sig_cols(buf), s.hist, s.status, g_part_blk_, s.misc, st,
                       0, 0, 0, rec_shard_rank(), rec_shard_world(), fused_sel ? sel_cnt_ : nullptr,
                       fused_sel ? sel_mask_ : nullptr, sel_stride_);
  if (fused_sel)
    launch_select_masked(sig_cols(buf), s.rows, N, sel_cnt_, sel_off_, sel_mask_, sel_stride_,
                         reinterpret_cast<XRec*>(xsend_ + sizeof(XRec)), reinterpret_cast<uint32_t*>(xsend_),
                         (uint32_t)cfg_.xchg_cap, st, s.dbg + kDbgXchgDropped);
  else if (xchg)
    launch_select(sig_cols(buf), s.rows, counts, N, sel_cnt_, sel_off_, reinterpret_cast<XRec*>(xsend_ + sizeof(XRec)),
                  reinterpret_cast<uint32_t*>(xsend_), (uint32_t)cfg_.xchg_cap, st, s.dbg + kDbgXchgDropped);
}

void WindowEngine::run_join_front(const Buf& buf, hipStream_t st, bool xchg) {
  const BufSet& s = *buf.set;
  const int N = n_rows_;
  if (xchg) {
    const TraceIds tt{trace_hash_, kTraceIdRows};
    launch_decode_window(buf.in + off_kern_, buf.in + off_user_, buf.counts(), s.rows, N, buf.imp, ctx_tab_,
                         (int)kCtxRows, tt, s.ring_state, tmax_, pod_sn_, kPodRows, sig_cols(buf), s.hist, s.status,
                         g_part_blk_, s.misc, st, 1, nblk_imp_, nblk_sig_, rec_shard_rank(), rec_shard_world());
  }
  const bool branched = branch_ && !xchg;
  hipEvent_t sig_base = branched ? ev_sigbase_ : nullptr;
  if (!branched && !(xchg && xspan_)) run_spans(buf, st);
  const uint32_t* wspan = branched ? nullptr : s.s_part_base;
  const JoinParams* wjp = branched ? nullptr : &jp_;
  uint32_t* wlist = branched ? nullptr : s.probe_work;
  launch_partition_sig(sig_cols(buf), s.rows, N, nblk_sig_ + (xchg ? nblk_imp_ : 0), g_part_blk_, g_part_off_,
                       g_part_tot_, st, xchg ? nblk_sig_ : 0, sig_base, wspan, wjp, wlist);
  if (branched) {
    HIPCHECK(hipStreamWaitEvent(side_, ev_sigbase_, 0));
    launch_probe_work(s.s_part_base, sig_cols(buf), jp_, s.probe_work, side_);
    HIPCHECK(hipEventRecord(ev_spans_, side_));
    HIPCHECK(hipStreamWaitEvent(st, ev_spans_, 0));
  }
}

void WindowEngine::run_join_back(const Buf& buf, int n_groups, bool with_labels, bool learn, hipStream_t st) {
  const BufSet& s = *buf.set;
  const ResultViewT<uint8_t>& r = buf.res;
  const int* counts = buf.counts();
  const int32_t* labels = reinterpret_cast<const int32_t*>(buf.in + kHeadBytes);
  const int S = cfg_.span_cap, G = cfg_.group_cap;
  launch_probe(span_cols(buf), s.s_items, s.s_part_base, sig_cols(buf), S, jp_, s.top3, s.cnt, n_groups, s.gsum, s.gcnt,
               s.dbg, s.probe_work, s.s_pre, st);
  launch_finalize(counts + 1, S, s.top3, s.cnt, sig_cols(buf), span_cols(buf), jp_, nullptr, attrs_, conf_, kernel_ms_,
                  n_groups, s.gsum, s.gcnt, r.feat, s.dbg, st);
  const PosteriorModel* pm = reinterpret_cast<const PosteriorModel*>(model_dev_);
  if (learn)
    launch_posterior_stats(r.feat, counts + 2, G, pm, with_labels ? labels : nullptr, r.post, r.pred, r.gconf, r.evbits,
                           s.confusion, labels, nullptr, s.stats, s.stats_count, st, app_dev_, r.app);
  else
    launch_posterior(r.feat, counts + 2, G, pm, with_labels ? labels : nullptr, r.post, r.pred, r.gconf, r.evbits,
                     s.confusion, st, app_dev_, r.app);
  if (!comm_) {
    const size_t res16 = (result_bytes() + 15) / 16;
    const int g = (int)std::max<size_t>((kPacketLen + 255) / 256, std::min<size_t>(64, (res16 + 255) / 256));
    hipLaunchKernelGGL(k_window_end, dim3(g), dim3(256), 0, st, s.hist, s.status, s.misc, s.dbg, s.confusion, s.stats,
                       s.stats_count, s.ring_state, buf.packet_dev, totals_, buf.packet_host,
                       reinterpret_cast<const uint4*>(buf.res_dev), reinterpret_cast<uint4*>(buf.res_host), res16);
    return;
  }
  hipLaunchKernelGGL(k_pack, dim3((kPacketLen + 255) / 256), dim3(256), 0, st, s.hist, s.status, s.misc, s.dbg,
                     s.confusion, s.stats, s.stats_count, s.ring_state, buf.packet_dev);
}

void WindowEngine::run_spans(const Buf& buf, hipStream_t st) {
  const BufSet& s = *buf.set;
  const int* counts = buf.counts();
  const int S = cfg_.span_cap, G = cfg_.group_cap;
  const SpanMap sm{1, buf.res.sli, G, cfg_.ttft_slo_ms, cfg_.shard_rank, cfg_.shard_world,
                   s.gen, buf.res.app, buf.res.late};
  launch_decode_spans(buf.in + off_span_, counts + 1, S, span_cols(buf), s_part_blk_, ctx_tab_, (int)kCtxRows, st, &sm);
  launch_partition(s.s_part, counts + 1, S, nblk_span_, s_part_blk_, s_part_off_, s_part_tot_, s.s_part_base, s.s_items,
                   st);
  launch_span_sort(span_cols(buf), s.s_items, s.s_part_base, s.s_pre, st);
}

void WindowEngine::run_span_branch(const Buf& buf, hipStream_t st) {
  HIPCHECK(hipEventRecord(ev_fork_, st));
  HIPCHECK(hipStreamWaitEvent(side_, ev_fork_, 0));
  run_spans(buf, side_);
}

void WindowEngine::launch_part(Stage part, const Buf& buf, int n_groups, bool with_labels, bool learn) {
  hipStream_t cs = part == Stage::XchgSpans ? side_ : part == Stage::Front ? front_ : compute_;
  auto run = [&] {
    switch (part) {
      case Stage::Window:
        run_part1(buf, cs, false);
        run_join_front(buf, cs, false);
        return run_join_back(buf, n_groups, with_labels, learn, cs);
      case Stage::Records: return run_part1(buf, cs, true);
      case Stage::Join:
        run_join_front(buf, cs, true);
        return run_join_back(buf, n_groups, with_labels, learn, cs);
      case Stage::XchgSpans: return run_spans(buf, cs);
      case Stage::XchgHead: return run_begin(buf, cs);
      case Stage::Front:
        run_part1(buf, cs, false);
        return run_join_front(buf, cs, false);
      case Stage::Back: return run_join_back(buf, n_groups, with_labels, learn, cs);
    }
  };
  if (!cfg_.use_graphs) return run();
  const int slot = buf.b * kStageSlots + (int)part;
  auto key = part == Stage::Front ? std::make_tuple(slot, 0, false, false)
                                  : std::make_tuple(slot, n_groups, with_labels, learn);
  auto it = graphs_.find(key);
  if (it == graphs_.end() && !warm_[slot]) {
    run();
    warm_[slot] = true;
    return;
  }
  if (it == graphs_.end()) {
    hipGraph_t g;
    HIPCHECK(hipStreamBeginCapture(cs, hipStreamCaptureModeThreadLocal));
    run();
    HIPCHECK(hipStreamEndCapture(cs, &g));
    hipGraphExec_t ex;
    HIPCHECK(hipGraphInstantiate(&ex, g, nullptr, nullptr, 0));
    graph_defs_.push_back(g);
    it = graphs_.emplace(key, ex).first;
  }
  HIPCHECK(hipGraphLaunch(it->second, cs));
}

void WindowEngine::merge_remote(const Buf& buf, const uint8_t* blocks, size_t stride, int world, int me,
                                hipStream_t st) {
  launch_remote_merge(blocks, stride, world, me, buf.imp, buf.remote_n, (uint32_t)cfg_.import_cap, cfg_.xchg_cap, st,
                      buf.set->dbg + kDbgXchgDropped);
  launch_window_rows(buf.counts(), buf.remote_n, n_rows_, buf.set->rows, buf.set->gen, st);
}

void WindowEngine::refit(const double* add) {
  launch_refit_nb(stats_acc_, add, p0_, cfg_.alpha, cfg_.prior_pseudo, cfg_.n_dom,
                  reinterpret_cast<PosteriorModel*>(model_dev_), compute_, cfg_.inv_temp, cfg_.min_count,
                  p0_ + kSlots * 16, cfg_.cap_dom, cfg_.lik_ceil);
}

bool WindowEngine::take_copy_lanes() {
  if (!lane_on_request_ || copy_open_) return lanes_ == 2;
  lane_on_request_ = false;
  HIPCHECK(hipSetDevice(cfg_.device));
  const hipStream_t lane = mk_stream(env_int("MISLO_COPY_LANE_PRIO", 1) != 0);
  const size_t n = std::min<size_t>(in_bytes_ - off_kern_, size_t(64) << 20);
  void *h = nullptr, *d = nullptr;
  hipError_t e = hipHostMalloc(&h, 2 * n, hipHostMallocDefault);
  if (e == hipSuccess) e = hipMalloc(&d, 2 * n);
  if (e == hipSuccess) {
    std::memset(h, 0, 2 * n);
    uint8_t *hp = static_cast<uint8_t*>(h), *dp = static_cast<uint8_t*>(d);
    for (int round = 0; round < 2 && e == hipSuccess; ++round) {
      e = hipMemcpyAsync(dp, hp, n, hipMemcpyHostToDevice, copy_[0]);
      if (e == hipSuccess) e = hipMemcpyAsync(dp + n, hp + n, n, hipMemcpyHostToDevice, lane);
    }
    const hipError_t e0 = hipStreamSynchronize(copy_[0]), e1 = hipStreamSynchronize(lane);
    if (e == hipSuccess) e = e0 != hipSuccess ? e0 : e1;
  }
  if (d) (void)hipFree(d);
  if (h) (void)hipHostFree(h);
  HIPCHECK(e);
  copy_[1] = lane;
  lanes_ = 2;
  return true;
}

void WindowEngine::submit(int64_t k, const WindowInput& in, bool with_labels, bool learn) {
  submit_copy(k, in);
  submit_chain(k, in.n_groups, with_labels, learn);
}

void WindowEngine::submit_copy(int64_t k, const WindowInput& in) {
  Lap whole;
  if (k != submitted_) throw std::invalid_argument("windows must be submitted in order");
  if (copy_open_) throw std::logic_error("submit_copy: the window's chain phase has not been queued");
  const int n_groups = in.n_groups;
  if (n_groups < 0 || n_groups > cfg_.group_cap) throw std::invalid_argument("n_groups exceeds group capacity");
  size_t kb = 0, ub = 0, sb = 0;
  for (const Seg& s : in.kernel) kb += s.bytes;
  for (const Seg& s : in.user) ub += s.bytes;
  for (const Seg& s : in.spans) sb += s.bytes;
  if (in.user_rec != 64 && in.user_rec != 32 && in.user_rec != 24 && in.user_rec != 16)
    throw std::invalid_argument("user records are 64, 32, 24 or 16 bytes");
  if (kb % kRecStride || ub % in.user_rec || sb % 64) throw std::invalid_argument("segments must hold whole records");
  const size_t n_k = kb / kRecStride * kBatchSlots, n_u = ub / in.user_rec, n_s = sb / 64;
  if (n_k + n_u > (size_t)cfg_.sig_cap || n_u > (size_t)cfg_.user_cap || n_s > (size_t)cfg_.span_cap)
    throw std::invalid_argument("window exceeds the engine's capacity (events / user records / spans)");
  Buf& buf = bufs_[k % nb_];
  const CopyMark& mk = mark(k);
  Lap phase;
  if (!copy_ahead_ && k >= max_ahead_) HIPCHECK(hipEventSynchronize(bufs_[(k - max_ahead_) % nb_].compute_done));
  if (k >= nb_) {
    HIPCHECK(hipEventSynchronize(mark(k - nb_).h2d_done));
    copied_.reused(k, nb_);
    HIPCHECK(hipEventSynchronize(buf.head_done));
    if (copy_ahead_) HIPCHECK(hipEventSynchronize(buf.front_done));
  }
  phase(wait_us_);
  int32_t* c = reinterpret_cast<int32_t*>(buf.head_host);
  std::memset(c, 0, kHeadBytes);
  c[0] = (int32_t)(n_k + n_u);
  c[1] = (int32_t)n_s;
  c[2] = n_groups;
  c[4] = (int32_t)(uint32_t)(uint64_t)in.bases[0];
  c[5] = (int32_t)(uint32_t)((uint64_t)in.bases[0] >> 32);
  c[6] = in.user_rec;
  c[7] = 64;
  for (int q = 1; q < 4; ++q) {
    c[8 + 2 * (q - 1)] = (int32_t)(uint32_t)(uint64_t)in.bases[q];
    c[9 + 2 * (q - 1)] = (int32_t)(uint32_t)((uint64_t)in.bases[q] >> 32);
  }
  c[15] = (int32_t)n_k;
  int32_t* lab = reinterpret_cast<int32_t*>(buf.head_host + kHeadBytes);
  for (int g = 0; g < cfg_.group_cap; ++g) lab[g] = (in.labels && g < n_groups) ? in.labels[g] : -1;
  const hipStream_t cs = copy_[copy_lane(k, lanes_)];
  HIPCHECK(hipEventRecord(mk.t_start, cs));
  size_t st_off = 0;
  Lap part;
  dma(in.kernel, buf.in + off_kern_, kern_bytes(), buf.staging, st_off, cs);
  part(split_us_[0]);
  part(split_us_[1]);
  dma(in.user, buf.in + off_user_, 64 * (size_t)cfg_.user_cap, buf.staging, st_off, cs);
  part(split_us_[2]);
  dma(in.spans, buf.in + off_span_, 64 * (size_t)cfg_.span_cap, buf.staging, st_off, cs);
  part(split_us_[3]);
  HIPCHECK(hipEventRecord(mk.h2d_done, cs));
  phase(dma_us_);
  copy_open_ = true;
  copy_groups_ = n_groups;
  whole(issue_us_);
}

void WindowEngine::submit_chain(int64_t k, int n_groups, bool with_labels, bool learn) {
  Lap whole;
  if (!copy_open_ || k != submitted_) throw std::logic_error("submit_chain: not the window submit_copy queued last");
  if (n_groups != copy_groups_) throw std::invalid_argument("submit_chain: n_groups differs from the copy phase's");
  Buf& buf = bufs_[k % nb_];
  const CopyMark& mk = mark(k);
  Lap phase;
  if (copy_ahead_ && k >= max_ahead_) HIPCHECK(hipEventSynchronize(bufs_[(k - max_ahead_) % nb_].compute_done));
  phase(wait_us_);
  hipStream_t fs = overlap_ ? front_ : compute_;
  HIPCHECK(hipStreamWaitEvent(fs, mk.h2d_done, 0));
  if (overlap_ && k >= 2) HIPCHECK(hipStreamWaitEvent(fs, bufs_[(k - 2) % nb_].compute_done, 0));
  HIPCHECK(hipStreamWaitEvent(compute_, buf.comm_done, 0));
  const bool injected = !inject_.empty();
  if (injected) {
    HIPCHECK(hipMemcpyAsync(xrecv_, inject_.data(), inject_.size(), hipMemcpyHostToDevice, compute_));
    HIPCHECK(hipStreamSynchronize(compute_));
  }
  HIPCHECK(hipEventRecord(buf.t_comp0, fs));
  to_host(buf.head_host, buf.in, off_kern_, fs);
  HIPCHECK(hipEventRecord(buf.head_done, fs));
  if (cfg_.device_refit && k >= nb_) {
    refit(buf.packet_dev + kStatsOff);
    ++folded_;
  }
  const bool xchg = exchange() || injected;
  phase(pre_us_);
  if (overlap_) {
    if (xchg) throw std::logic_error("the exchange path does not run with overlapped windows");
    launch_part(Stage::Front, buf, n_groups, with_labels, learn);
    HIPCHECK(hipEventRecord(buf.front_done, front_));
    HIPCHECK(hipStreamWaitEvent(compute_, buf.front_done, 0));
    launch_part(Stage::Back, buf, n_groups, with_labels, learn);
  } else if (!xchg) {
    launch_part(Stage::Window, buf, n_groups, with_labels, learn);
  } else {
    if (xspan_) {
      launch_part(Stage::XchgHead, buf, n_groups, with_labels, learn);
      HIPCHECK(hipEventRecord(ev_fork_, compute_));
      HIPCHECK(hipStreamWaitEvent(side_, ev_fork_, 0));
      launch_part(Stage::XchgSpans, buf, n_groups, with_labels, learn);
      HIPCHECK(hipEventRecord(ev_spans_, side_));
    }
    launch_part(Stage::Records, buf, n_groups, with_labels, learn);
    if (injected) {
      merge_remote(buf, xrecv_, inject_stride_, inject_world_, inject_me_, compute_);
      inject_.clear();
    } else if (xcomm_) {
      NCCLCHECK(ncclAllGather(xsend_, xrecv_, xstride_, ncclUint8, xcomm_, compute_));
      merge_remote(buf, xrecv_, xstride_, world_, rank_, compute_);
    } else {
      HIPCHECK(hipEventRecord(buf.xchg_done, compute_));
      HIPCHECK(hipStreamWaitEvent(comm_stream_, buf.xchg_done, 0));
      NCCLCHECK(ncclAllGather(xsend_, xrecv_, xstride_, ncclUint8, comm_, comm_stream_));
      merge_remote(buf, xrecv_, xstride_, world_, rank_, comm_stream_);
      HIPCHECK(hipEventRecord(buf.xchg_done, comm_stream_));
      HIPCHECK(hipStreamWaitEvent(compute_, buf.xchg_done, 0));
    }
    if (xspan_) HIPCHECK(hipStreamWaitEvent(compute_, ev_spans_, 0));
    launch_part(Stage::Join, buf, n_groups, with_labels, learn);
  }
  phase(launch_us_);
  const size_t res_bytes = result_bytes();
  if (comm_) to_host(buf.res_dev, buf.res_host, res_bytes, compute_);
  HIPCHECK(hipEventRecord(buf.t_comp1, compute_));
  HIPCHECK(hipEventRecord(buf.compute_done, compute_));
  HIPCHECK(hipStreamWaitEvent(comm_stream_, buf.compute_done, 0));
  if (comm_) {
    NCCLCHECK(ncclGroupStart());
    NCCLCHECK(ncclAllReduce(buf.packet_dev, buf.packet_dev, kPacketLen - kPacketRing, ncclFloat64, ncclSum, comm_,
                            comm_stream_));
    NCCLCHECK(ncclAllGather(buf.res_dev, buf.res_all_dev, res_bytes, ncclUint8, comm_, comm_stream_));
    NCCLCHECK(ncclGroupEnd());
    to_host(buf.res_all_dev, buf.res_all_host, res_bytes * world_, comm_stream_);
    hipLaunchKernelGGL(k_accumulate, dim3((kPacketLen + 255) / 256), dim3(256), 0, comm_stream_, buf.packet_dev,
                       totals_, kPacketLen, buf.packet_host);
  }
  HIPCHECK(hipEventRecord(buf.t_end, comm_stream_));
  HIPCHECK(hipEventRecord(buf.comm_done, comm_stream_));
  ++submitted_;
  copy_open_ = false;
  phase(tail_us_);
  whole(issue_us_);
  ++issue_n_;
}

bool WindowEngine::query(int64_t k) {
  const hipError_t e = hipEventQuery(bufs_[k % nb_].comm_done);
  if (e == hipSuccess) return true;
  if (e == hipErrorNotReady) return false;
  HIPCHECK(e);
  return false;
}

void WindowEngine::wait(int64_t k) {
  if (spin_) {
    while (!query(k)) {
    }
    return;
  }
  HIPCHECK(hipEventSynchronize(bufs_[k % nb_].comm_done));
}

std::vector<float> WindowEngine::copy_ms(int64_t k) {
  const CopyMark& mk = mark(k);
  float dur = 0.f, gap = -1.f;
  HIPCHECK(hipEventSynchronize(mk.h2d_done));
  HIPCHECK(hipEventElapsedTime(&dur, mk.t_start, mk.h2d_done));
  if (k >= 1) HIPCHECK(hipEventElapsedTime(&gap, mark(k - 1).h2d_done, mk.t_start));
  return {dur, gap};
}

std::pair<float, float> WindowEngine::window_ms(int64_t k) {
  const Buf& buf = bufs_[k % nb_];
  float total = 0.f, comp = 0.f;
  HIPCHECK(hipEventSynchronize(buf.t_end));
  HIPCHECK(hipEventElapsedTime(&total, mark(k).t_start, buf.t_end));
  HIPCHECK(hipEventElapsedTime(&comp, buf.t_comp0, buf.t_comp1));
  return {total, comp};
}

void WindowEngine::set_model_bytes(const void* bytes, size_t n) {
  if (n != sizeof(PosteriorModel)) throw std::invalid_argument("model image must be POSTERIOR_MODEL_BYTES bytes");
  uint8_t* h = model_host_[model_slot_++ % model_host_.size()];
  std::memcpy(h, bytes, n);
  HIPCHECK(hipMemcpyAsync(model_dev_, h, n, hipMemcpyHostToDevice, compute_));
}

void WindowEngine::set_app_model(const void* bytes, size_t n) {
  if (n != sizeof(AppModel)) throw std::invalid_argument("application model must be APP_MODEL_BYTES bytes");
  uint8_t* h = model_host_[model_slot_++ % model_host_.size()];
  static_assert(sizeof(AppModel) <= sizeof(PosteriorModel), "the staging slots fit the application model");
  std::memcpy(h, bytes, n);
  HIPCHECK(hipMemcpyAsync(app_dev_, h, n, hipMemcpyHostToDevice, compute_));
}

void WindowEngine::set_p0(const double* p0, size_t n) {
  if (n != (size_t)kSlots * 16 && n != 2 * (size_t)kSlots * 16) throw std::invalid_argument("p0 must be f64[256] or [512]");
  HIPCHECK(hipMemset(p0_ + kSlots * 16, 0, kSlots * 16 * sizeof(double)));
  HIPCHECK(hipMemcpy(p0_, p0, n * sizeof(double), hipMemcpyHostToDevice));
}

void WindowEngine::set_refit(double alpha, double prior_pseudo, double inv_temp, double min_count, int cap_dom,
                             double ceil) {
  if (!(alpha > 0.0) || !(prior_pseudo >= 0.0) || !(inv_temp > 0.0) || !(min_count >= 0.0) || cap_dom >= cfg_.n_dom ||
      !(ceil > 0.0 && ceil <= 1.0))
    throw std::invalid_argument("refit parameters");
  cfg_.lik_ceil = ceil;
  cfg_.cap_dom = cap_dom < 0 ? -1 : cap_dom;
  cfg_.alpha = alpha;
  cfg_.prior_pseudo = prior_pseudo;
  cfg_.inv_temp = inv_temp;
  cfg_.min_count = min_count;
}

void WindowEngine::refit_now() { refit(nullptr); }

void WindowEngine::score_features(const float* feat, int n, const int32_t* labels, double* post, int32_t* pred,
                                  double* conf, uint32_t* evbits, uint32_t* confusion, const uint32_t* app_cnt) {
  if (n < 0) throw std::invalid_argument("n");
  sync();
  if (n == 0) return;
  const size_t o_n = (size_t)n * 16 * 4, o_lab = o_n + 64, o_post = (o_lab + (size_t)n * 4 + 63) & ~size_t(63);
  const size_t o_pred = o_post + (size_t)n * 16 * 8, o_conf = (o_pred + (size_t)n * 4 + 63) & ~size_t(63);
  const size_t o_ev = o_conf + (size_t)n * 8, o_cm = o_ev + (size_t)n * 16 * 4, o_app = o_cm + 16 * 16 * 4;
  const size_t bytes = o_app + (size_t)n * 2 * 4;
  uint8_t* d = dalloc<uint8_t>(bytes, true);
  HIPCHECK(hipMemcpy(d, feat, o_n, hipMemcpyHostToDevice));
  HIPCHECK(hipMemcpy(d + o_n, &n, sizeof(int), hipMemcpyHostToDevice));
  if (labels) HIPCHECK(hipMemcpy(d + o_lab, labels, (size_t)n * 4, hipMemcpyHostToDevice));
  if (app_cnt) HIPCHECK(hipMemcpy(d + o_app, app_cnt, (size_t)n * 2 * 4, hipMemcpyHostToDevice));
  launch_posterior(reinterpret_cast<const float*>(d), reinterpret_cast<const int*>(d + o_n), n,
                   reinterpret_cast<const PosteriorModel*>(model_dev_),
                   labels ? reinterpret_cast<const int32_t*>(d + o_lab) : nullptr, reinterpret_cast<double*>(d + o_post),
                   reinterpret_cast<int32_t*>(d + o_pred), reinterpret_cast<double*>(d + o_conf),
                   reinterpret_cast<uint32_t*>(d + o_ev), reinterpret_cast<uint32_t*>(d + o_cm), compute_,
                   app_cnt ? app_dev_ : nullptr, app_cnt ? reinterpret_cast<const uint32_t*>(d + o_app) : nullptr);
  HIPCHECK(hipStreamSynchronize(compute_));
  HIPCHECK(hipMemcpy(post, d + o_post, (size_t)n * 16 * 8, hipMemcpyDeviceToHost));
  HIPCHECK(hipMemcpy(pred, d + o_pred, (size_t)n * 4, hipMemcpyDeviceToHost));
  HIPCHECK(hipMemcpy(conf, d + o_conf, (size_t)n * 8, hipMemcpyDeviceToHost));
  HIPCHECK(hipMemcpy(evbits, d + o_ev, (size_t)n * 16 * 4, hipMemcpyDeviceToHost));
  HIPCHECK(hipMemcpy(confusion, d + o_cm, 16 * 16 * 4, hipMemcpyDeviceToHost));
  own_.free_dev(d);
}

void WindowEngine::set_pods(const uint32_t* pods, const uint32_t* svcnode, size_t n) {
  hipStream_t st = overlap_ ? front_ : compute_;
  HIPCHECK(hipStreamSynchronize(st));
  for (size_t i = 0; i < n; ++i)
    if (pods[i] < kPodRows) pod_host_[pods[i]] = svcnode[i];
  HIPCHECK(hipMemcpyAsync(pod_sn_, pod_host_, kPodRows * 4, hipMemcpyHostToDevice, st));
}

std::vector<uint8_t> WindowEngine::sent_block() {
  sync();
  std::vector<uint8_t> out(xsend_ ? xstride_ : 0);
  if (xsend_) HIPCHECK(hipMemcpy(out.data(), xsend_, xstride_, hipMemcpyDeviceToHost));
  return out;
}

std::vector<int64_t> WindowEngine::import_state() {
  sync();
  int rows[2];
  unsigned long long tmax = 0;
  GenMeta g{};
  std::vector<uint32_t> r(nb_);
  const BufSet& s = *bufs_[submitted_ ? (submitted_ - 1) % nb_ : 0].set;
  HIPCHECK(hipMemcpy(rows, s.rows, sizeof(rows), hipMemcpyDeviceToHost));
  HIPCHECK(hipMemcpy(&tmax, tmax_, 8, hipMemcpyDeviceToHost));
  HIPCHECK(hipMemcpy(&g, s.gen, sizeof(g), hipMemcpyDeviceToHost));
  HIPCHECK(hipMemcpy(r.data(), remote_n_, 4 * nb_, hipMemcpyDeviceToHost));
  std::vector<int64_t> out{rows[0], rows[1], (int64_t)tmax, gens_, g.cur, g.filled};
  for (int a = 0; a < kMaxGens; ++a) out.push_back(g.cut[a]);
  for (int a = 0; a < kMaxGens; ++a) out.push_back(a < gens_ ? g.n_rows[(g.cur + slots_ - a) % slots_] : 0);
  for (int b = 0; b < nb_; ++b) out.push_back(r[b]);
  return out;
}

void WindowEngine::inject_remote(const void* blocks, size_t stride, int world, int me) {
  if (!cfg_.import_cap || !cfg_.xchg_cap) throw std::logic_error("inject_remote needs import_cap and xchg_cap > 0");
  if (world < 1 || me < 0 || me >= world || stride < sizeof(XRec)) throw std::invalid_argument("bad exchange blocks");
  const uint8_t* h = static_cast<const uint8_t*>(blocks);
  for (int r = 0; r < world; ++r) {
    uint32_t c;
    std::memcpy(&c, h + (size_t)r * stride, 4);
    if ((size_t)c * sizeof(XRec) + sizeof(XRec) > stride) throw std::invalid_argument("block row count exceeds stride");
    if (r != me && c > (uint32_t)cfg_.xchg_cap) throw std::invalid_argument("block holds more rows than xchg_cap");
  }
  if (stride * world > xrecv_bytes_) {
    sync();
    own_.free_dev(xrecv_);
    xrecv_ = dalloc<uint8_t>(stride * world);
    xrecv_bytes_ = stride * world;
  }
  inject_.assign(h, h + stride * world);
  inject_stride_ = stride;
  inject_world_ = world;
  inject_me_ = me;
}

void WindowEngine::init_comm(const ncclUniqueId& id, int rank, int world) {
  if (comm_) throw std::logic_error("communicator already initialised");
  if (world < 1 || rank < 0 || rank >= world) throw std::invalid_argument("communicator rank / world");
  if (submitted_ || copy_open_) throw std::logic_error("init_comm before the first window");
  HIPCHECK(hipSetDevice(cfg_.device));
  if (overlap_) {
    HIPCHECK(hipStreamSynchronize(front_));
    overlap_ = false;
    copy_ahead_ = lane_on_request_ = false;
    lanes_ = 1;
    if (!getenv("MISLO_SPAN_STREAM")) enable_span_branch();
  }
  NCCLCHECK(ncclCommInitRank(&comm_, world, id, rank));
  {
    comm_stream_ = mk_stream(env_int("MISLO_COMM_STREAM_PRIO", 1) != 0);
  }
  rank_ = rank;
  world_ = world;
  for (Buf& buf : bufs_) {
    buf.res_all_dev = dalloc<uint8_t>(result_bytes() * world);
    buf.res_all_host = static_cast<uint8_t*>(host_block(result_bytes() * world));
  }
  if (cfg_.xchg_cap) {
    if (world > 8) throw std::invalid_argument("the exchange is sized for <= 8 GPUs per node");
    own_.free_dev(xrecv_);
    xrecv_bytes_ = xstride_ * world;
    xrecv_ = dalloc<uint8_t>(xrecv_bytes_, true);
    const char* xv = getenv("MISLO_XCHG_STREAM");
    int split = (xv && std::strcmp(xv, "compute") == 0) ? 1 : 0;
    int* d_split = dalloc<int>(1);
    HIPCHECK(hipMemcpy(d_split, &split, sizeof(int), hipMemcpyHostToDevice));
    NCCLCHECK(ncclBroadcast(d_split, d_split, 1, ncclInt32, 0, comm_, comm_stream_));
    HIPCHECK(hipStreamSynchronize(comm_stream_));
// ... 49 lines not shown
```

llm_slo_ebpf_toolkit_amd/ops/csrc/join.hip:

```cpp
#include <cstdlib>

#include "mislo_common.h"
#include "mislo_launch.h"

namespace mislo {

constexpr int kSigBits = 27;
constexpr int kChunk = 256;


constexpr int kScanCols = 32, kScanRG = 32;
__global__ __launch_bounds__(kScanCols * kScanRG) void k_part_scan(const uint32_t* __restrict__ part_blk, int nblk,
                                                                  uint32_t* __restrict__ part_off,
                                                                  uint32_t* __restrict__ part_tot) {
  __shared__ uint32_t s_sum[kScanRG][kScanCols];
  const int cl = threadIdx.x % kScanCols, r = threadIdx.x / kScanCols;
  const int c = blockIdx.x * kScanCols + cl;
  const int per = (nblk + kScanRG - 1) / kScanRG;
  const int b0 = min(nblk, r * per), b1 = min(nblk, b0 + per);
  constexpr size_t W = (size_t)kKeyTypes * kParts;
  uint32_t sum = 0;
  for (int b = b0; b < b1; ++b) sum += part_blk[(size_t)b * W + c];
  s_sum[r][cl] = sum;
  __syncthreads();
  uint32_t run = 0, tot = 0;
  for (int q = 0; q < kScanRG; ++q) {
    const uint32_t v = s_sum[q][cl];
    run += q < r ? v : 0u;
    tot += v;
  }
  for (int b = b0; b < b1; ++b) {
    const size_t idx = (size_t)b * W + c;
    const uint32_t v = part_blk[idx];
    part_off[idx] = run;
    run += v;
  }
  if (r == 0) part_tot[c] = tot;
}

constexpr int kBaseNT = kKeyTypes * kParts / 4;
__global__ __launch_bounds__(kBaseNT) void k_base_scan(const uint32_t* __restrict__ tot, uint32_t* __restrict__ base,
                                                      const GenMeta* __restrict__ gen) {
  if (gen) base += (size_t)gen->cur * kBaseLen;
  __shared__ uint32_t s[kBaseNT];
  const int t = threadIdx.x;
  uint32_t v[4];
  uint32_t sum = 0;
#pragma unroll
  for (int j = 0; j < 4; ++j) {
    v[j] = tot[t * 4 + j];
    sum += v[j];
  }
  s[t] = sum;
  __syncthreads();
  for (int off = 1; off < kBaseNT; off <<= 1) {
    uint32_t x = t >= off ? s[t - off] : 0;
    __syncthreads();
    s[t] += x;
    __syncthreads();
  }
  uint32_t run = s[t] - sum;
#pragma unroll
  for (int j = 0; j < 4; ++j) {
    base[t * 4 + j] = run;
    run += v[j];
  }
  if (t == kBaseNT - 1) base[kKeyTypes * kParts] = s[kBaseNT - 1];
}

template <int NT>
__global__ __launch_bounds__(NT) void k_scatter(const PartCodes* __restrict__ codes, const int* __restrict__ n_ptr,
                                                int cap, const uint32_t* __restrict__ part_off,
                                                const uint32_t* __restrict__ base, uint32_t* __restrict__ items,
                                                int nblk_a) {
  __shared__ uint32_t s_pos[kKeyTypes * kParts];
  {
    const uint32_t* my_off = part_off + (size_t)blockIdx.x * kKeyTypes * kParts;
    for (int i = threadIdx.x; i < kKeyTypes * kParts; i += NT) s_pos[i] = base[i] + my_off[i];
  }
  __syncthreads();
  const int n0 = min(n_ptr[0], cap);
  const bool two = nblk_a < (int)gridDim.x;
  const bool second = two && (int)blockIdx.x >= nblk_a;
  const int s_beg = second ? n0 : 0;
  const int s_end = second ? max(n0, min(n_ptr[1], cap)) : n0;
  const int g = two ? (second ? (int)gridDim.x - nblk_a : nblk_a) : (int)gridDim.x;
  const int bi = second ? (int)blockIdx.x - nblk_a : (int)blockIdx.x;
  const int chunk = (s_end - s_beg + g - 1) / g;
  const int beg = s_beg + bi * chunk, end = min(s_end, beg + chunk);
  for (int i = beg + threadIdx.x; i < end; i += NT) {
    const PartCodes pc = codes[i];
#pragma unroll
    for (int k = 0; k < kKeyTypes; ++k) {
      if (pc.p[k] == kNoPart) continue;
      items[atomicAdd(&s_pos[k * kParts + pc.p[k]], 1u)] = (uint32_t)i;
    }
  }
}

template <int NT>
__device__ __forceinline__ void scatter_sig_body(const SignalCols& gc, const int* __restrict__ n_ptr, int cap,
                                                 const uint32_t* __restrict__ part_off, int nblk_a, int bid,
                                                 int nblk, uint32_t* s_pos) {
  const uint32_t cur = cur_slot(gc);
  const SigRec* rec = gc.rec + (size_t)cur * (size_t)gc.stride;
  const uint32_t* base = gc.base + (size_t)cur * kBaseLen;
  uint32_t* items = gc.items + (size_t)cur * kKeyTypes * (size_t)gc.stride;
  KeyTs* keys = gc.keys + (size_t)cur * kKeyTypes * (size_t)gc.stride;
  {
    const uint32_t* my_off = part_off + (size_t)bid * kKeyTypes * kParts;
    for (int i = threadIdx.x; i < kKeyTypes * kParts; i += NT) s_pos[i] = base[i] + my_off[i];
  }
  __syncthreads();
  const int n0 = min(n_ptr[0], cap);
  const bool two = nblk_a < nblk;
  const bool second = two && bid >= nblk_a;
  const int s_beg = second ? n0 : 0;
  const int s_end = second ? max(n0, min(n_ptr[1], cap)) : n0;
  const int g = two ? (second ? nblk - nblk_a : nblk_a) : nblk;
  const int bi = second ? bid - nblk_a : bid;
  const int chunk = (s_end - s_beg + g - 1) / g;
  const int beg = s_beg + bi * chunk, end = min(s_end, beg + chunk);
  constexpr int kU = 4;
  const PartCodes* __restrict__ part = gc.part;
  for (int i0 = beg + threadIdx.x; i0 < end; i0 += NT * kU) {
    PartCodes pc[kU];
    uint4 a[kU], b[kU], c4[kU];
#pragma unroll
    for (int u = 0; u < kU; ++u) {
      const int i = i0 + u * NT;
      if (i < end) {
        pc[u] = part[i];
        const uint4* v = reinterpret_cast<const uint4*>(rec + i);
        a[u] = v[0];
        b[u] = v[1];
        c4[u] = v[2];
      } else {
        pc[u].p[0] = pc[u].p[1] = pc[u].p[2] = pc[u].p[3] = kNoPart;
      }
    }
#pragma unroll
    for (int u = 0; u < kU; ++u) {
      if ((pc[u].p[0] & pc[u].p[1] & pc[u].p[2] & pc[u].p[3]) == kNoPart) continue;
      const int64_t ts = (int64_t)(((uint64_t)a[u].y << 32) | a[u].x);
      const uint64_t tr = ((uint64_t)a[u].w << 32) | a[u].z, cn = ((uint64_t)b[u].y << 32) | b[u].x;
#pragma unroll
      for (int k = 0; k < kKeyTypes; ++k) {
        if (pc[u].p[k] == kNoPart) continue;
        const uint32_t pos = atomicAdd(&s_pos[k * kParts + pc[u].p[k]], 1u);
        items[pos] = (uint32_t)(i0 + u * NT);
        keys[pos] = KeyTs{key_hash(k, tr, b[u].z, b[u].w, cn, c4[u].x), ts};
      }
    }
  }
}

template <int NT>
__global__ __launch_bounds__(NT) void k_scatter_sig(SignalCols gc, const int* __restrict__ n_ptr, int cap,
                                                    const uint32_t* __restrict__ part_off, int nblk_a) {
  __shared__ uint32_t s_pos[kKeyTypes * kParts];
  scatter_sig_body<NT>(gc, n_ptr, cap, part_off, nblk_a, (int)blockIdx.x, (int)gridDim.x, s_pos);
}


__device__ __forceinline__ bool less_ht(uint64_t h1, int64_t t1, uint64_t h2, int64_t t2) {
  return h1 < h2 || (h1 == h2 && t1 < t2);
}

__device__ __forceinline__ void top3_insert(unsigned long long* slot3, unsigned long long key) {
#pragma unroll
  for (int j = 0; j < 3; ++j) {
    const unsigned long long old = atomicMin(slot3 + j, key);
    if (old == kEmpty) return;
    key = old > key ? old : key;
  }
}

__device__ __forceinline__ int64_t iabs64(int64_t x) { return x < 0 ? -x : x; }

struct SigHot {
  int64_t ts;
  uint64_t tr, cn;
  uint32_t pod, pid, sn;
  float val;
  uint32_t slot;
};
__device__ __forceinline__ SigHot load_hot(const SigRec* p) {
  const uint4* v = reinterpret_cast<const uint4*>(p);
  const uint4 a = v[0], b = v[1], c = v[2];
  SigHot h;
  h.ts = (int64_t)(((uint64_t)a.y << 32) | a.x);
  h.tr = ((uint64_t)a.w << 32) | a.z;
  h.cn = ((uint64_t)b.y << 32) | b.x;
  h.pod = b.z;
  h.pid = b.w;
  h.sn = c.x;
  h.val = __uint_as_float(c.y);
  h.slot = c.z;
  return h;
}

struct alignas(16) SpanKT {
  uint64_t h;
  int64_t t;
};
struct alignas(16) SpanTC {
  uint64_t tr;
  uint64_t cn;
};
struct alignas(16) SpanPP {
  uint32_t pod, pid, sn, grp;
};

constexpr int kLdsGroups = 64;
constexpr int kProbeGrid = 512;
constexpr int kSigPerItem = 6144;

__device__ __forceinline__ uint32_t probe_item_class(int k, uint32_t n_sig, uint32_t n_span) {
  constexpr uint32_t kPerSig[kKeyTypes] = {90, 40, 85, 60};
  const uint32_t cost = 24000u + 64u * min(n_span, 256u) + n_sig * kPerSig[k];
  return min(cost >> 13, 63u);
}

__device__ __forceinline__ void probe_work_body(const uint32_t* __restrict__ span_base, const SignalCols& gc,
                                                const JoinParams& jp, int sig_per_item, uint32_t* __restrict__ work,
                                                unsigned long long* s, unsigned long long* s2, uint32_t* s_cls) {
  const int p = threadIdx.x;
  if (p < 64) s_cls[p] = 0u;
  const uint32_t cur = cur_slot(gc);
  const GenMeta* gm = gc.gen;
  const int64_t s_lo = gm ? ts_of_image(gm->span_lo) : INT64_MIN, s_hi = gm ? ts_of_image(gm->span_hi) : INT64_MAX;
  uint32_t ns[kKeyTypes], ng[kKeyTypes][kMaxGens], n[kKeyTypes][kMaxGens], nk[kKeyTypes];
  uint32_t b_lo[kKeyTypes][kMaxGens], b_hi[kKeyTypes][kMaxGens];
#pragma unroll
  for (int a = 0; a < kMaxGens; ++a) {
    const uint32_t* b = gc.base + (size_t)(a < gc.gens ? age_slot(gc, cur, a) : 0u) * kBaseLen;
#pragma unroll
    for (int k = 0; k < kKeyTypes; ++k) {
      b_lo[k][a] = a < gc.gens ? b[k * kParts + p] : 0u;
      b_hi[k][a] = a < gc.gens ? b[k * kParts + p + 1] : 0u;
    }
  }
#pragma unroll
  for (int k = 0; k < kKeyTypes; ++k) {
    const int c = k * kParts + p;
    ns[k] = span_base[c + 1] - span_base[c];
    nk[k] = 0;
    const int64_t w = jp.win_ns[k];
#pragma unroll
    for (int a = 0; a < kMaxGens; ++a) {
// ... 84 lines not shown
__global__ __launch_bounds__(NT) void k_scatter_sig_work(SignalCols gc, const int* __restrict__ n_ptr, int cap,
                                                         const uint32_t* __restrict__ part_off, int nblk_a,
                                                         const uint32_t* __restrict__ span_base, JoinParams jp,
                                                         int sig_per_item, uint32_t* __restrict__ work) {
  static_assert(NT == kParts, "the work-list block runs one thread per partition");
  static_assert(2 * kParts * 8 + 64 * 4 >= kKeyTypes * kParts * 4, "one LDS buffer serves both");
  __shared__ unsigned long long s_buf[2 * kParts + 32];
  if (blockIdx.x == 0) {
    probe_work_body(span_base, gc, jp, sig_per_item, work, s_buf, s_buf + kParts,
                    reinterpret_cast<uint32_t*>(s_buf + 2 * kParts));
    return;
  }
  scatter_sig_body<NT>(gc, n_ptr, cap, part_off, nblk_a, (int)blockIdx.x - 1, (int)gridDim.x - 1,
                       reinterpret_cast<uint32_t*>(s_buf));
}

template <int NT>
__device__ __forceinline__ void block_inclusive_scan(int* v, int n, int* wsum) {
  const int t = threadIdx.x, lane = t & 63, wave = t >> 6;
  const int i0 = 2 * t, i1 = 2 * t + 1;
  const int a = i0 < n ? v[i0] : 0, b = i1 < n ? v[i1] : 0;
  const int local = a + b;
  int incl = local;
  for (int off = 1; off < 64; off <<= 1) {
    const int y = __shfl_up(incl, off);
    if (lane >= off) incl += y;
  }
  if (lane == 63) wsum[wave] = incl;
  __syncthreads();
  int base = 0;
  for (int w = 0; w < wave; ++w) base += wsum[w];
  const int excl = base + incl - local;
  if (i0 < n) v[i0] = excl + a;
  if (i1 < n) v[i1] = excl + a + b;
  __syncthreads();
}

__device__ __forceinline__ int lower_ht(const SpanKT* kt, int lo, int hi, uint64_t h0, int64_t t0) {
  while (lo < hi) {
    const int mid = (lo + hi) >> 1;
    const SpanKT e = kt[mid];
    if (less_ht(e.h, e.t, h0, t0)) lo = mid + 1; else hi = mid;
  }
  return lo;
}
__device__ __forceinline__ int upper_ht(const SpanKT* kt, int lo, int hi, uint64_t h0, int64_t t0) {
  while (lo < hi) {
    const int mid = (lo + hi) >> 1;
    const SpanKT e = kt[mid];
    if (less_ht(h0, t0, e.h, e.t)) hi = mid; else lo = mid + 1;
  }
  return lo;
}
__device__ __forceinline__ int lower_u16(const uint16_t* v, int n, int x) {
  int lo = 0, hi = n;
  while (lo < hi) {
    const int mid = (lo + hi) >> 1;
    if ((int)v[mid] < x) lo = mid + 1; else hi = mid;
  }
  return lo;
}

__device__ __forceinline__ void store_prespan(PreSpan* dst_p, uint64_t h, int64_t t, const SpanRec& rr, uint32_t idx,
                                              uint32_t run) {
  PreSpan ps;
  ps.h = h;
  ps.t = t;
  ps.tr = rr.tr;
  ps.cn = rr.cn;
  ps.pod = rr.pod;
  ps.pid = rr.pid;
  ps.sn = rr.sn;
  ps.grp = rr.grp;
  ps.idx = idx;
  ps.run = run;
  ps.pad[0] = ps.pad[1] = 0u;
  const uint4* src = reinterpret_cast<const uint4*>(&ps);
  uint4* dst = reinterpret_cast<uint4*>(dst_p);
#pragma unroll
  for (int q = 0; q < 4; ++q) dst[q] = src[q];
}

template <int NT>
__global__ __launch_bounds__(NT) void k_span_sort(SpanCols sc, const uint32_t* __restrict__ span_items,
                                                  const uint32_t* __restrict__ span_base, PreSpan* __restrict__ out) {
  static_assert(kChunk == NT, "one span per thread");
  __shared__ SpanKT s_kt[kChunk];
  __shared__ SpanTC s_tc[kChunk];
  __shared__ SpanPP s_pp[kChunk];
  __shared__ uint16_t s_pos[kChunk];
  __shared__ uint16_t s_inv[kChunk];
  __shared__ int s_aux[kChunk];
  __shared__ uint32_t s_ok[kChunk];
  __shared__ int s_wsum[NT / 64];
  const int c = blockIdx.x, k = c / kParts;
  const uint32_t sp0 = span_base[c], sp1 = span_base[c + 1];
  const int ti = threadIdx.x;
  for (uint32_t c0 = sp0; c0 < sp1; c0 += kChunk) {
    const int m = (int)min((uint32_t)kChunk, sp1 - c0);
    int M = 1;
    while (M < m) M <<= 1;
    __syncthreads();
    SpanRec rr{};
    uint32_t my_s = 0xFFFFFFFFu;
    if (ti < m) {
      my_s = span_items[c0 + ti];
      rr = sc.rec[my_s];
    }
    if (ti < M) {
      s_kt[ti] = ti < m ? SpanKT{key_hash(k, rr.tr, rr.pod, rr.pid, rr.cn, rr.sn), rr.ts} : SpanKT{~0ull, INT64_MAX};
      s_pos[ti] = (uint16_t)ti;
    }
    __syncthreads();
    for (int size = 2; size <= M; size <<= 1) {
      for (int stride = size >> 1; stride > 0; stride >>= 1) {
        for (int t = threadIdx.x; t < (M >> 1); t += NT) {
          const int i = 2 * t - (t & (stride - 1));
          const int j = i + stride;
          const bool up = (i & size) == 0;
          const SpanKT ei = s_kt[i], ej = s_kt[j];
          const bool gt = less_ht(ej.h, ej.t, ei.h, ei.t);
          if (gt == up) {
            s_kt[i] = ej; s_kt[j] = ei;
            const uint16_t tp = s_pos[i]; s_pos[i] = s_pos[j]; s_pos[j] = tp;
          }
        }
        __syncthreads();
      }
    }
    if (ti < m) s_inv[s_pos[ti]] = (uint16_t)ti;
    __syncthreads();
    int i = 0;
    if (ti < m) {
      i = s_inv[ti];
      s_tc[i] = SpanTC{rr.tr, rr.cn};
      s_pp[i] = SpanPP{rr.pod, rr.pid, rr.sn, rr.grp};
      s_ok[i] = 1u;
      s_aux[i] = (i == 0 || s_kt[i].h != s_kt[i - 1].h) ? 1 : 0;
    }
    __syncthreads();
    block_inclusive_scan<NT>(s_aux, m, s_wsum);
    if (ti < m && i > 0 && s_kt[i].h == s_kt[i - 1].h) {
      const SpanPP a = s_pp[i], b = s_pp[i - 1];
      const SpanTC x = s_tc[i], y = s_tc[i - 1];
      if (a.pod != b.pod || a.pid != b.pid || a.sn != b.sn || a.grp != b.grp || (k == 2 && x.cn != y.cn))
        atomicAnd(&s_ok[s_aux[i] - 1], 0u);
    }
    __syncthreads();
    if (ti < m) {
      const uint32_t rid = (uint32_t)(s_aux[i] - 1);
      store_prespan(out + c0 + i, s_kt[i].h, s_kt[i].t, rr, my_s, rid | (s_ok[rid] << 16));
    }
  }
}

template <int NT, bool LG>
__global__ __launch_bounds__(NT, LG ? 4 : 6) void k_probe(const PreSpan* __restrict__ pre,
                                              const uint32_t* __restrict__ span_base, SignalCols gc, int span_cap,
                                              JoinParams jp, unsigned long long* __restrict__ top3,
                                              uint32_t* __restrict__ cnt, int n_groups,
                                              unsigned long long* __restrict__ gsum, uint32_t* __restrict__ gcnt,
                                              unsigned long long* __restrict__ dbg, uint32_t* __restrict__ work,
                                              int phase) {
  static_assert(kChunk == NT, "staging keeps one span per thread");
  __shared__ SpanKT s_kt[kChunk];
  __shared__ SpanTC s_tc[kChunk];
  __shared__ SpanPP s_pp[kChunk];
  __shared__ uint32_t s_i[kChunk];
  __shared__ unsigned long long s_top[kChunk * 3];
  __shared__ unsigned long long s_seed3[kChunk];
  __shared__ int s_diff[kChunk + 1];
  __shared__ int s_aux[kChunk];
  __shared__ uint16_t s_rid[kChunk];
  __shared__ uint32_t s_runok[kChunk];
  __shared__ uint16_t s_needy[kChunk];
  __shared__ int s_wsum[NT / 64];
  __shared__ int s_nneedy;
  __shared__ uint32_t s_item;
  constexpr int kLg = LG ? kLdsGroups * kSlots : 1;
  __shared__ unsigned long long s_gsum[kLg];
  __shared__ uint32_t s_gcnt[kLg];

  {
    const size_t stripe = (size_t)(blockIdx.x & (kGroupStripes - 1)) * (size_t)n_groups * kSlots;
    gsum += stripe;
    gcnt += stripe;
  }
  const bool grp_lds = LG && n_groups <= kLdsGroups;
  const bool any_groups = jp.group_mode == 1 && n_groups > 0;
  if (grp_lds && any_groups) {
    for (int i = threadIdx.x; i < kLdsGroups * kSlots; i += NT) {
      s_gsum[i] = 0ull;
      s_gcnt[i] = 0u;
    }
  }
  const bool cand1 = jp.conf[1] >= jp.threshold, cand2 = jp.conf[2] >= jp.threshold;
  unsigned long long n_cand = 0, n_low = 0, n_overlap = 0;
  const uint32_t n_work = work[phase];
  const uint32_t* items = work + 4 + (phase ? kProbePhaseItems : 0);
  const uint32_t cur = cur_slot(gc);

  for (;;) {
    __syncthreads();
    if (threadIdx.x == 0) s_item = atomicAdd(&work[2 + phase], 1u);
    __syncthreads();
    const uint32_t it = s_item;
    if (it >= n_work) break;
#ifdef MISLO_PROBE_PROFILE
    unsigned long long pt = clock64(), p_stage = 0, p_sig = 0, p_flush = 0;
#endif
    const uint32_t code = items[it];
    const int k = (int)(code >> 30);
    const int age = (int)((code >> 28) & 3u);
    const int part = (int)((code >> 16) & 0x3FF);
    const uint32_t si = (code >> 8) & 0xFF, nsplit = code & 0xFF;
    const int c = k * kParts + part;
    const uint32_t sp0 = span_base[c], sp1 = span_base[c + 1];
    const uint32_t gslot = age_slot(gc, cur, age);
    const uint32_t* sig_base = gc.base + (size_t)gslot * kBaseLen;
    const uint32_t* sig_items = gc.items + (size_t)gslot * kKeyTypes * (size_t)gc.stride;
    const KeyTs* sig_keys = gc.keys + (size_t)gslot * kKeyTypes * (size_t)gc.stride;
    const SigRec* grec = gc.rec + (size_t)gslot * (size_t)gc.stride;
    const int64_t cut = gc.gen ? gc.gen->cut[age] : INT64_MIN;
    const uint32_t n_loc = gc.gen ? gc.gen->n_local[gslot] : 0xFFFFFFFFu;
    const uint32_t cls_loc = (uint32_t)age * (uint32_t)gc.stride;
    const uint32_t cls_rem = (uint32_t)(2 * gc.gens - 1 - age) * (uint32_t)gc.stride;
    const uint32_t gb0 = sig_base[c], gb1 = sig_base[c + 1];
    const uint32_t per = (gb1 - gb0 + nsplit - 1) / nsplit;
    const uint32_t sg0 = gb0 + si * per;
    const uint32_t sg1 = min(gb1, sg0 + per);

    const int64_t w = jp.win_ns[k];
    const bool cand_tier = jp.conf[k] >= jp.threshold;
    const bool count_only = (k == 3) && !cand_tier;
    const bool track_overlap = (k < 3) && (jp.conf[3] < jp.threshold);
    const bool do_groups = cand_tier && any_groups;
    const bool ranged = (k == 1 || k == 2);

    auto add_group = [&](uint32_t grp, int slot, unsigned long long milli, uint32_t n) {
      if (grp >= (uint32_t)n_groups || n == 0) return;
      if (grp_lds) {
        atomicAdd(&s_gsum[grp * kSlots + slot], milli * n);
        atomicAdd(&s_gcnt[grp * kSlots + slot], n);
      } else {
        atomicAdd(gsum + (size_t)grp * kSlots + slot, milli * n);
        atomicAdd(gcnt + (size_t)grp * kSlots + slot, n);
      }
    };
    auto add_range = [&](int a, int b) {
      if (a < b) {
        atomicAdd(&s_diff[a], 1);
        atomicAdd(&s_diff[b], -1);
      }
    };

  for (uint32_t c0 = sp0; c0 < sp1; c0 += kChunk) {
    const int m = (int)min((uint32_t)kChunk, sp1 - c0);
    __syncthreads();
    const int ti = threadIdx.x;
    if (ti < m) {
      const uint4* src = reinterpret_cast<const uint4*>(pre + c0 + ti);
      const uint4 a = src[0], b = src[1], cc = src[2], d = src[3];
      const uint32_t my_s = d.x;
      s_kt[ti] = SpanKT{((uint64_t)a.y << 32) | a.x, (int64_t)(((uint64_t)a.w << 32) | a.z)};
      s_i[ti] = my_s;
      if (!count_only) {
        s_tc[ti] = SpanTC{((uint64_t)b.y << 32) | b.x, ((uint64_t)b.w << 32) | b.z};
        s_pp[ti] = SpanPP{cc.x, cc.y, cc.z, cc.w};
        s_top[3 * ti] = kEmpty;
        s_top[3 * ti + 1] = kEmpty;
        s_top[3 * ti + 2] = kEmpty;
        s_seed3[ti] = k > 0 ? top3[3ull * my_s + 2] : kEmpty;
        s_diff[ti] = 0;
        s_rid[ti] = (uint16_t)(d.y & 0xFFFFu);
        s_runok[d.y & 0xFFFFu] = d.y >> 16;
      }
    }
    if (threadIdx.x == 0 && !count_only) s_diff[m] = 0;
    __syncthreads();
    if (!count_only) {
      if (ranged) {
        for (int i = threadIdx.x; i < m; i += NT) {
          const unsigned long long seed = s_seed3[i];
          s_aux[i] = (cand_tier && (seed == kEmpty || (int)(seed >> 62) >= k)) ? 1 : 0;
        }
        __syncthreads();
        block_inclusive_scan<NT>(s_aux, m, s_wsum);
        for (int i = threadIdx.x; i < m; i += NT) {
          const int prev = i ? s_aux[i - 1] : 0;
          if (s_aux[i] != prev) s_needy[prev] = (uint16_t)i;
        }
        if (threadIdx.x == 0) s_nneedy = s_aux[m - 1];
        __syncthreads();
      }
    }
    const int n_needy = ranged && !count_only ? s_nneedy : 0;
#ifdef MISLO_PROBE_PROFILE
    { const unsigned long long t = clock64(); p_stage += t - pt; pt = t; }
#endif

    constexpr int kDepth = 1;
    uint32_t q = sg0 + threadIdx.x;
    KeyTs kq[kDepth];
    uint32_t iq[kDepth];
#pragma unroll
    for (int d = 0; d < kDepth; ++d) {
// ... 232 lines not shown
    }
  }
  for (int off = 32; off > 0; off >>= 1) {
    n_cand += __shfl_xor(n_cand, off);
    n_low += __shfl_xor(n_low, off);
    n_overlap += __shfl_xor(n_overlap, off);
  }
  if ((threadIdx.x & 63) == 0) {
    if (n_cand) atomicAdd(&dbg[0], n_cand);
    if (n_low) atomicAdd(&dbg[1], n_low);
    if (n_overlap) atomicAdd(&dbg[2], n_overlap);
  }
}


template <int NT>
__global__ __launch_bounds__(NT) void k_finalize(const int* __restrict__ ns_ptr, int span_cap,
                                                 const unsigned long long* __restrict__ top3,
                                                 const uint32_t* __restrict__ cnt, SignalCols gc, SpanCols sc,
                                                 JoinParams jp, const float* __restrict__ base_attrs,
                                                 float* __restrict__ attrs, float* __restrict__ conf,
                                                 float* __restrict__ kernel_ms, int n_groups,
                                                 unsigned long long* __restrict__ gsum, uint32_t* __restrict__ gcnt,
                                                 unsigned long long* __restrict__ dbg) {
  const int ns = min(*ns_ptr, span_cap);
  const int s = blockIdx.x * NT + threadIdx.x;
  {
    const size_t stripe = (size_t)(blockIdx.x & (kGroupStripes - 1)) * (size_t)n_groups * kSlots;
    gsum += stripe;
    gcnt += stripe;
  }
  unsigned long long dropped = 0, enriched = 0;
  const uint32_t cur = cur_slot(gc);
  if (s < ns) {
    float a[kSlots];
#pragma unroll
    for (int j = 0; j < kSlots; ++j) a[j] = base_attrs ? base_attrs[(size_t)s * kSlots + j] : __builtin_nanf("");
    float mc = 0.f;
    const int keep = jp.fanout;
#pragma unroll
    for (int j = 0; j < 3; ++j) {
      const unsigned long long key = top3[3ull * s + j];
      if (key == kEmpty || j >= keep) continue;
      const int tier = (int)(key >> 62);
      const uint32_t g = (uint32_t)(key & ((1ull << kSigBits) - 1));
      const uint32_t cls = g / (uint32_t)gc.stride, row = g - cls * (uint32_t)gc.stride;
      const int age = (int)cls < gc.gens ? (int)cls : 2 * gc.gens - 1 - (int)cls;
      const SigRec& r = gc.rec[(size_t)age_slot(gc, cur, age) * (size_t)gc.stride + row];
      const int slot = (int)r.slot;
      const float v = r.val;
      float cur = a[0];
#pragma unroll
      for (int q = 0; q < kSlots; ++q) if (q == slot) cur = a[q];
      const bool take = (cur != cur) || v > cur;
#pragma unroll
      for (int q = 0; q < kSlots; ++q) if (q == slot && take) a[q] = v;
      mc = fmaxf(mc, jp.conf[tier]);
    }
    const uint32_t c = cnt[s];
    if ((int)c > keep) dropped = c - keep;
    if (mc > 0.f) enriched = 1;
    conf[s] = mc;
    float km = 0.f;
    if (a[0] == a[0]) km += a[0];
    if (a[3] == a[3]) km += a[3];
    if (a[5] == a[5]) km += a[5];
    kernel_ms[s] = km > 0.f ? km : __builtin_nanf("");
#pragma unroll
    for (int j = 0; j < kSlots; ++j) attrs[(size_t)s * kSlots + j] = a[j];
    const uint32_t grp = sc.rec[s].grp;
    if (jp.group_mode == 0 && n_groups > 0 && grp < (uint32_t)n_groups) {
#pragma unroll
      for (int j = 0; j < kSlots; ++j) {
        if (a[j] == a[j]) {
          atomicAdd(gsum + (size_t)grp * kSlots + j, milli_units(a[j]));
          atomicAdd(gcnt + (size_t)grp * kSlots + j, 1u);
        }
      }
    }
  }
  for (int off = 32; off > 0; off >>= 1) {
    dropped += __shfl_xor(dropped, off);
    enriched += __shfl_xor(enriched, off);
  }
  if ((threadIdx.x & 63) == 0) {
    if (dropped) atomicAdd(&dbg[3], dropped);
    if (enriched) atomicAdd(&dbg[4], enriched);
  }
}

__device__ __forceinline__ float group_feature(unsigned long long sum, uint32_t c) {
  return c ? (float)(((double)sum * 1e-3) / (double)c) : __builtin_nanf("");
}

__global__ __launch_bounds__(256) void k_fold_groups(int n, unsigned long long* __restrict__ gsum,
                                                     uint32_t* __restrict__ gcnt, float* __restrict__ feat) {
  const int i = blockIdx.x * 256 + threadIdx.x;
  if (i >= n) return;
  unsigned long long s = gsum[i];
  uint32_t c = gcnt[i];
#pragma unroll
  for (int r = 1; r < kGroupStripes; ++r) {
    s += gsum[(size_t)r * n + i];
    c += gcnt[(size_t)r * n + i];
  }
  gsum[i] = s;
  gcnt[i] = c;
  feat[i] = group_feature(s, c);
}

__global__ __launch_bounds__(256) void k_group_features(int n, const unsigned long long* __restrict__ gsum,
                                                        const uint32_t* __restrict__ gcnt, float* __restrict__ feat) {
  const int i = blockIdx.x * 256 + threadIdx.x;
  if (i >= n) return;
  feat[i] = group_feature(gsum[i], gcnt[i]);
}


static int probe_item_signals() {
  static const int per_item = [] {
    const char* v = getenv("MISLO_PROBE_ITEM");
    const int x = v ? atoi(v) : kSigPerItem;
    return x >= 1 ? x : kSigPerItem;
  }();
  return per_item;
}

void launch_partition_sig(const SignalCols& gc, const int* n_dev, int cap, int nblk, const uint32_t* part_blk,
                          uint32_t* part_off, uint32_t* part_tot, hipStream_t stream, int nblk_a, hipEvent_t bases_done,
                          const uint32_t* work_span_base, const JoinParams* work_jp, uint32_t* work) {
  hipLaunchKernelGGL(k_part_scan, dim3(kKeyTypes * kParts / kScanCols), dim3(kScanCols * kScanRG), 0, stream,
                     part_blk, nblk, part_off, part_tot);
  hipLaunchKernelGGL(k_base_scan, dim3(1), dim3(kBaseNT), 0, stream, part_tot, gc.base, gc.gen);
  if (bases_done) (void)hipEventRecord(bases_done, stream);
  const int na = nblk_a > 0 && nblk_a < nblk ? nblk_a : nblk;
  if (work != nullptr && work_jp != nullptr && work_span_base != nullptr)
    hipLaunchKernelGGL((k_scatter_sig_work<1024>), dim3(nblk + 1), dim3(1024), 0, stream, gc, n_dev, cap, part_off,
                       na, work_span_base, *work_jp, probe_item_signals(), work);
  else
    hipLaunchKernelGGL((k_scatter_sig<1024>), dim3(nblk), dim3(1024), 0, stream, gc, n_dev, cap, part_off, na);
}

void launch_partition(const PartCodes* codes, const int* n_dev, int cap, int nblk, const uint32_t* part_blk,
                      uint32_t* part_off, uint32_t* part_tot, uint32_t* part_base, uint32_t* items,
                      hipStream_t stream, int nblk_a) {
  static_assert((kKeyTypes * kParts) % kScanCols == 0, "scan columns tile the partition matrix");
  hipLaunchKernelGGL(k_part_scan, dim3(kKeyTypes * kParts / kScanCols), dim3(kScanCols * kScanRG), 0, stream,
                     part_blk, nblk, part_off, part_tot);
  hipLaunchKernelGGL(k_base_scan, dim3(1), dim3(kBaseNT), 0, stream, part_tot, part_base, nullptr);
  hipLaunchKernelGGL((k_scatter<1024>), dim3(nblk), dim3(1024), 0, stream, codes, n_dev, cap, part_off, part_base,
                     items, nblk_a > 0 && nblk_a < nblk ? nblk_a : nblk);
}

void launch_probe(const SpanCols& sc, const uint32_t* span_items, const uint32_t* span_base, const SignalCols& gc,
                  int span_cap, const JoinParams& jp, unsigned long long* top3, uint32_t* cnt, int n_groups,
                  unsigned long long* gsum, uint32_t* gcnt, unsigned long long* dbg, uint32_t* work,
                  PreSpan* span_pre, hipStream_t stream) {
  static const int grid = [] {
    const char* v = getenv("MISLO_PROBE_GRID");
    const int x = v ? atoi(v) : kProbeGrid;
    return x >= 1 && x <= 65536 ? x : kProbeGrid;
  }();
  static const int per_item = [] {
    const char* v = getenv("MISLO_PROBE_ITEM");
    const int x = v ? atoi(v) : kSigPerItem;
    return x >= 1 ? x : kSigPerItem;
  }();
  (void)sc, (void)span_items, (void)per_item;
  static const bool lds_groups = [] {
    const char* v = getenv("MISLO_PROBE_LDS_GROUPS");
    return !(v && atoi(v) == 0);
  }();
  for (int phase = 0; phase < 2; ++phase) {
    if (lds_groups)
      hipLaunchKernelGGL((k_probe<256, true>), dim3(grid), dim3(256), 0, stream, span_pre, span_base, gc, span_cap, jp,
                         top3, cnt, n_groups, gsum, gcnt, dbg, work, phase);
    else
      hipLaunchKernelGGL((k_probe<256, false>), dim3(grid), dim3(256), 0, stream, span_pre, span_base, gc, span_cap, jp,
                         top3, cnt, n_groups, gsum, gcnt, dbg, work, phase);
  }
}

void launch_span_sort(const SpanCols& sc, const uint32_t* span_items, const uint32_t* span_base, PreSpan* span_pre,
                      hipStream_t stream) {
  hipLaunchKernelGGL((k_span_sort<kChunk>), dim3(kKeyTypes * kParts), dim3(kChunk), 0, stream, sc, span_items,
                     span_base, span_pre);
}

void launch_probe_work(const uint32_t* span_base, const SignalCols& gc, const JoinParams& jp, uint32_t* work,
                       hipStream_t stream) {
  hipLaunchKernelGGL(k_probe_work, dim3(1), dim3(kParts), 0, stream, span_base, gc, jp, probe_item_signals(), work);
}

void launch_finalize(const int* ns_dev, int span_cap, const unsigned long long* top3, const uint32_t* cnt,
                     const SignalCols& gc, const SpanCols& sc, const JoinParams& jp, const float* base_attrs,
                     float* attrs, float* conf, float* kernel_ms, int n_groups, unsigned long long* gsum, uint32_t* gcnt,
                     float* feat, unsigned long long* dbg, hipStream_t stream) {
  hipLaunchKernelGGL((k_finalize<256>), dim3((span_cap + 255) / 256), dim3(256), 0, stream, ns_dev, span_cap, top3,
                     cnt, gc, sc, jp, base_attrs, attrs, conf, kernel_ms, n_groups, gsum, gcnt, dbg);
  if (n_groups > 0) {
    const int n = n_groups * kSlots;
    hipLaunchKernelGGL(k_fold_groups, dim3((n + 255) / 256), dim3(256), 0, stream, n, gsum, gcnt, feat);
  }
}

void launch_group_features(int n_groups, const unsigned long long* gsum, const uint32_t* gcnt, float* feat, hipStream_t stream) {
  if (n_groups <= 0) return;
  const int n = n_groups * kSlots;
  hipLaunchKernelGGL(k_group_features, dim3((n + 255) / 256), dim3(256), 0, stream, n, gsum, gcnt, feat);
}

}
```

llm_slo_ebpf_toolkit_amd/ops/csrc/mislo_launch.h:

```cpp
#pragma once

#include <hip/hip_runtime.h>
#include <stdint.h>

#include "mislo_common.h"
#include "mislo_packet.h"

namespace mislo {

struct PosteriorModel {
  double w[kSlots][kMaxDomains];
  double bias[kMaxDomains];
  double mean[kSlots];
  double nominal[kSlots];
  float thr[kSlots];
  uint32_t dom_mask[kMaxDomains];
  uint32_t table_mask;
  int32_t mode;
  int32_t n_pairs;
  double pair_rho;
  double w2[kSlots][kMaxPairs];
  double bias2[kMaxPairs];
  uint8_t pair_a[kMaxPairs];
  uint8_t pair_b[kMaxPairs];
};

constexpr int kAppBit = 16;
struct AppModel {
  double w[kMaxDomains];
  double b[kMaxDomains];
  double w2[kMaxPairs];
  double b2[kMaxPairs];
  double thr_ms;
  uint32_t dom_mask;
  int32_t on;
};

void set_tables(const Tables* host_tables);
int decode_grid(int cap);
void launch_decode_events(const void* ev, const int* n_dev, int cap, const SignalCols& cols, uint32_t* hist,
                          uint32_t* status_cnt, uint32_t* part_cnt, unsigned long long* misc, hipStream_t stream);
void launch_decode_wire(const void* ev, const int* n_dev, int cap, const uint32_t* ctx_tab, int n_ctx,
                        const SignalCols& cols, uint32_t* hist, uint32_t* status_cnt, uint32_t* part_cnt,
                        unsigned long long* misc, hipStream_t stream);
void launch_decode_ref(const void* ev, const int* n_dev, int cap, uint32_t pod, uint32_t svcnode, uint64_t trace_h,
                       const SignalCols& cols, uint32_t* hist, uint32_t* status_cnt, uint32_t* part_cnt,
                       unsigned long long* misc, hipStream_t stream);
struct SpanMap {
  int native;
  uint32_t* grp_sli;
  int n_groups;
  float ttft_slo_ms;
  int sh_rank = 0, sh_world = 1;
  GenMeta* gen = nullptr;
  uint32_t* grp_app = nullptr;
  uint32_t* grp_late = nullptr;
};
constexpr double kAppUnitsPerMs = 100.0;
void launch_decode_spans(const void* sp, const int* n_dev, int cap, const SpanCols& cols, uint32_t* part_cnt,
                         const uint32_t* ctx_tab, int n_ctx, hipStream_t stream, const SpanMap* sm = nullptr);
void launch_ring_defs(const uint8_t* framed, const int* n_dev, int cap, uint32_t* ctx_tab, uint32_t ctx_rows,
                      const uint32_t* pod_sn, uint32_t n_pods, const TraceIds& tt, uint32_t* ring_state,
                      hipStream_t stream);
void launch_decode_window(const uint8_t* framed, const void* user, const int* n_dev, const int* rows, int cap,
                          const SigRec* imp, const uint32_t* ctx_tab, int n_ctx, const TraceIds& tt,
                          uint32_t* ring_state, unsigned long long* tmax, const uint32_t* pod_sn, uint32_t n_pods,
                          const SignalCols& cols, uint32_t* hist, uint32_t* status_cnt, uint32_t* part_cnt,
                          unsigned long long* misc, hipStream_t stream, int seg = 0, int grid = 0, int blk_base = 0,
                          int sh_rank = 0, int sh_world = 1, uint32_t* sel_cnt = nullptr,
                          unsigned long long* sel_mask = nullptr, int sel_stride = 0);
int decode_sel_stride(int cap);

int select_grid(int cap);
struct XRec {
  int64_t ts;
  uint64_t tr;
  float val;
  uint32_t slot;
};
static_assert(sizeof(XRec) == 24, "exchange rows are 24 bytes");
void launch_select(const SignalCols& gc, const int* rows, const int* counts, int cap, uint32_t* blk_cnt,
                   uint32_t* blk_off, XRec* out, uint32_t* n_out, uint32_t out_cap, hipStream_t stream,
                   unsigned long long* dropped = nullptr);
void launch_select_masked(const SignalCols& gc, const int* rows, int cap, const uint32_t* blk_cnt, uint32_t* blk_off,
                          const unsigned long long* mask, int mask_stride, XRec* out, uint32_t* n_out,
                          uint32_t out_cap, hipStream_t stream, unsigned long long* dropped = nullptr);
void launch_remote_merge(const uint8_t* xrecv, size_t stride, int world, int me, SigRec* imp, uint32_t* remote_n,
                         uint32_t imp_cap, int max_rows, hipStream_t stream, unsigned long long* dropped = nullptr);
void launch_window_rows(const int* counts, const uint32_t* remote_n, int cap, int* rows, GenMeta* gen,
                        hipStream_t stream);
void launch_window_begin(const FillList& fl, GenMeta* gen, const GenMeta* gen_prev, unsigned long long* tmax, int gens,
                         int slots, long long halo_ns, uint32_t* ring_state, uint32_t* remote_n, const int* counts,
                         int cap, int* rows, hipStream_t stream);

void launch_partition(const PartCodes* codes, const int* n_dev, int cap, int nblk, const uint32_t* part_blk,
                      uint32_t* part_off, uint32_t* part_tot, uint32_t* part_base, uint32_t* items,
                      hipStream_t stream, int nblk_a = 0);
struct JoinParams;
void launch_partition_sig(const SignalCols& gc, const int* n_dev, int cap, int nblk, const uint32_t* part_blk,
                          uint32_t* part_off, uint32_t* part_tot, hipStream_t stream, int nblk_a = 0,
                          hipEvent_t bases_done = nullptr, const uint32_t* work_span_base = nullptr,
                          const JoinParams* work_jp = nullptr, uint32_t* work = nullptr);
struct alignas(64) PreSpan {
  uint64_t h;
  int64_t t;
  uint64_t tr, cn;
  uint32_t pod, pid, sn, grp;
  uint32_t idx, run;
  uint32_t pad[2];
};
static_assert(sizeof(PreSpan) == 64, "one cache line per staged span");
void launch_probe(const SpanCols& sc, const uint32_t* span_items, const uint32_t* span_base, const SignalCols& gc,
                  int span_cap, const JoinParams& jp, unsigned long long* top3, uint32_t* cnt, int n_groups,
                  unsigned long long* gsum, uint32_t* gcnt, unsigned long long* dbg, uint32_t* work,
                  PreSpan* span_pre, hipStream_t stream);
void launch_span_sort(const SpanCols& sc, const uint32_t* span_items, const uint32_t* span_base, PreSpan* span_pre,
                      hipStream_t stream);
void launch_probe_work(const uint32_t* span_base, const SignalCols& gc, const JoinParams& jp, uint32_t* work,
                       hipStream_t stream);
constexpr int kProbeMaxSplit = 64;
constexpr int kProbePhaseItems = kMaxGens * kParts * kProbeMaxSplit;
constexpr int kProbeProfOff = 4 + 4 * kProbePhaseItems;
constexpr int kProbeWorkLen = kProbeProfOff + 64;
void launch_finalize(const int* ns_dev, int span_cap, const unsigned long long* top3, const uint32_t* cnt,
                     const SignalCols& gc, const SpanCols& sc, const JoinParams& jp, const float* base_attrs,
                     float* attrs, float* conf, float* kernel_ms, int n_groups, unsigned long long* gsum, uint32_t* gcnt,
                     float* feat, unsigned long long* dbg, hipStream_t stream);

void launch_group_features(int n_groups, const unsigned long long* gsum, const uint32_t* gcnt, float* feat, hipStream_t stream);

void launch_posterior(const float* feat, const int* ng_dev, int cap, const PosteriorModel* pm, const int32_t* labels,
                      double* post, int32_t* pred, double* conf, uint32_t* evbits, uint32_t* confusion,
                      hipStream_t stream, const AppModel* app = nullptr, const uint32_t* app_cnt = nullptr);
void launch_stats(const float* feat, const int* ng_dev, int cap, const PosteriorModel* pm, const int32_t* labels,
                  const float* weights, double* out, double* count, hipStream_t stream);

void launch_posterior_stats(const float* feat, const int* ng_dev, int cap, const PosteriorModel* pm,
                            const int32_t* labels, double* post, int32_t* pred, double* conf, uint32_t* evbits,
                            uint32_t* confusion, const int32_t* stat_labels, const float* weights, double* out,
                            double* count, hipStream_t stream, const AppModel* app = nullptr,
                            const uint32_t* app_cnt = nullptr);
void launch_refit_nb(double* stats, const double* add, const double* p0, double alpha, double prior_pseudo, int n_dom,
                     PosteriorModel* pm, hipStream_t stream, double inv_temp = 1.0, double min_count = 0.0,
                     const double* floor_tab = nullptr, int cap_dom = -1, double ceil = 1.0);

int boot_max_n();
void launch_boot_quantile(const double* sorted_c, int nc, const double* sorted_b, int nb, double q, int iters,
                          uint64_t seed, double* out, hipStream_t stream);
void launch_rank_counts(const double* vals, int n_all, int nx, uint32_t* out, hipStream_t stream);

void launch_storm_counts(const uint64_t* keys, const int64_t* ts, int n, int64_t window_ns, uint32_t threshold,
                         uint32_t* counts, unsigned long long* n_storm, hipStream_t stream);

}
```

Measured before the change: 2.580 billion.

## Co-schedule independent front-end stages in shared horizontally fused launches

Result: slower. 2.355 billion (-8.7%).

```diff
diff --git a/llm_slo_ebpf_toolkit_amd/ops/csrc/agent_bindings.cpp b/llm_slo_ebpf_toolkit_amd/ops/csrc/agent_bindings.cpp
--- a/llm_slo_ebpf_toolkit_amd/ops/csrc/agent_bindings.cpp
+++ b/llm_slo_ebpf_toolkit_amd/ops/csrc/agent_bindings.cpp
@@ -1461,6 +1461,11 @@
       .def("packet", &PyEngine::packet)
       .def("results", &PyEngine::results)
       .def("window_ms", &PyEngine::window_ms)
+      .def("front_ms", [](PyEngine& p, int64_t k) {
+        py::gil_scoped_release nogil;
+        return p.eng().front_ms(k);
+      })
+      .def_property_readonly("front_fused", [](PyEngine& p) { return p.eng().front_fused(); })
       .def("copy_ms", [](PyEngine& p, int64_t k) {
         py::gil_scoped_release nogil;
         return p.eng().copy_ms(k);
diff --git a/llm_slo_ebpf_toolkit_amd/ops/csrc/decode.hip b/llm_slo_ebpf_toolkit_amd/ops/csrc/decode.hip
--- a/llm_slo_ebpf_toolkit_amd/ops/csrc/decode.hip
+++ b/llm_slo_ebpf_toolkit_amd/ops/csrc/decode.hip
@@ -1,5 +1,6 @@
 #include "mislo_common.h"
 #include "mislo_launch.h"
+#include "mislo_scan.h"
 #include <stdexcept>
 
 namespace mislo {
@@ -63,7 +64,7 @@
 }
 
 template <int NT>
-__device__ __forceinline__ void lds_flush(DecodeLds& L, const DecodeOut& o, int unsupported, int zero_ts) {
+__device__ __forceinline__ void lds_flush(DecodeLds& L, const DecodeOut& o, int unsupported, int zero_ts, int bid) {
   __syncthreads();
   for (int i = threadIdx.x; i < kSlots * kBuckets; i += NT) {
     uint32_t v = 0;
@@ -83,7 +84,7 @@
     for (int r = 0; r < DecodeLds::kRep; ++r) v += L.sum[r * DecodeLds::kUS + threadIdx.x];
     if (v) atomicAdd(&o.misc[kMiscSums + threadIdx.x], v);
   }
-  uint32_t* dst = o.part_cnt + (size_t)(o.blk_base + blockIdx.x) * kKeyTypes * kParts;
+  uint32_t* dst = o.part_cnt + (size_t)(o.blk_base + bid) * kKeyTypes * kParts;
   for (int i = threadIdx.x; i < kKeyTypes * kParts; i += NT) {
     uint32_t v = 0;
 #pragma unroll
@@ -176,7 +177,7 @@
     const uint32_t svcnode = ((uint32_t)e.svc_id << 16) | e.node_id;
     decode_one(i, cap, e.ts_ns, val, slot, e.trace_h, e.pod_id, e.pid, svcnode, ch, o, l, unsupported, zero_ts, i < n_local, o.cols.rec + i);
   }
-  lds_flush<NT>(L, o, unsupported, zero_ts);
+  lds_flush<NT>(L, o, unsupported, zero_ts, (int)blockIdx.x);
 }
 
 __device__ __forceinline__ bool shard_owns(uint32_t svcnode, int rank, int world) {
@@ -250,19 +251,20 @@
     }
     __syncthreads();
   }
-  lds_flush<NT>(L, o, unsupported, zero_ts);
-}
-
-
-__global__ __launch_bounds__(256) void k_ring_defs(const uint8_t* __restrict__ framed, const int* __restrict__ n_ptr,
-                                                   uint4* __restrict__ ctx_tab, uint32_t ctx_rows,
-                                                   const uint32_t* __restrict__ pod_sn, uint32_t n_pods, TraceIds tt,
-                                                   uint32_t* __restrict__ rs) {
+  lds_flush<NT>(L, o, unsupported, zero_ts, (int)blockIdx.x);
+}
+
+
+template <int NT>
+__device__ __forceinline__ void ring_defs_body(const uint8_t* __restrict__ framed, const int* __restrict__ n_ptr,
+                                               uint4* __restrict__ ctx_tab, uint32_t ctx_rows,
+                                               const uint32_t* __restrict__ pod_sn, uint32_t n_pods, const TraceIds& tt,
+                                               uint32_t* __restrict__ rs, int bid, int nblk, uint32_t* s_acc) {
   const int n = n_ptr[15];
   uint32_t foreign = 0, dctx = 0, dtr = 0, disc = 0, busy = 0xFFFFFFFFu;
   constexpr int kU = 4;
-  const int stride = gridDim.x * 256;
-  for (int i0 = blockIdx.x * 256 + threadIdx.x; i0 < n; i0 += stride * kU) {
+  const int stride = nblk * NT;
+  for (int i0 = bid * NT + threadIdx.x; i0 < n; i0 += stride * kU) {
     uint2 h[kU], a[kU], b[kU];
 #pragma unroll
     for (int u = 0; u < kU; ++u) {
@@ -316,7 +318,6 @@
     disc += __shfl_xor(disc, off);
     busy = min(busy, (uint32_t)__shfl_xor((int)busy, off));
   }
-  __shared__ uint32_t s_acc[5];
   if (threadIdx.x < 5) s_acc[threadIdx.x] = threadIdx.x == 0 ? 0xFFFFFFFFu : 0u;
   __syncthreads();
   if ((threadIdx.x & 63) == 0) {
@@ -336,15 +337,23 @@
   }
 }
 
-template <int NT>
-__global__ __launch_bounds__(NT) void k_decode_window(const uint8_t* __restrict__ framed,
-                                                      const Event* __restrict__ user, const int* __restrict__ n_ptr,
-                                                      const int* __restrict__ rows, int cap,
-                                                      const SigRec* __restrict__ imp,
-                                                      const uint4* __restrict__ ctx_tab, int n_ctx, TraceIds tt,
-                                                      uint32_t* __restrict__ rs, unsigned long long* __restrict__ tmax,
-                                                      const uint32_t* __restrict__ pod_sn, uint32_t n_pods, int seg,
-                                                      int sh_rank, int sh_world, DecodeOut o) {
+__global__ __launch_bounds__(256) void k_ring_defs(const uint8_t* __restrict__ framed, const int* __restrict__ n_ptr,
+                                                   uint4* __restrict__ ctx_tab, uint32_t ctx_rows,
+                                                   const uint32_t* __restrict__ pod_sn, uint32_t n_pods, TraceIds tt,
+                                                   uint32_t* __restrict__ rs) {
+  __shared__ uint32_t s_acc[5];
+  ring_defs_body<256>(framed, n_ptr, ctx_tab, ctx_rows, pod_sn, n_pods, tt, rs, (int)blockIdx.x, (int)gridDim.x, s_acc);
+}
+
+template <int NT>
+__device__ __forceinline__ void decode_window_body(const uint8_t* __restrict__ framed, const Event* __restrict__ user,
+                                                   const int* __restrict__ n_ptr, const int* __restrict__ rows,
+                                                   int cap, const SigRec* __restrict__ imp,
+                                                   const uint4* __restrict__ ctx_tab, int n_ctx, const TraceIds& tt,
+                                                   uint32_t* __restrict__ rs, unsigned long long* __restrict__ tmax,
+                                                   const uint32_t* __restrict__ pod_sn, uint32_t n_pods, int seg,
+                                                   int sh_rank, int sh_world, const DecodeOut& o, int bid, int nblk,
+                                                   uint4* s_stage) {
   __shared__ DecodeLds L;
   __shared__ uint32_t s_cnt2[3];
   __shared__ unsigned long long s_t[3];
@@ -366,15 +375,14 @@
   auto base_at = [&](int lo) { return (int64_t)(((uint64_t)(uint32_t)n_ptr[lo + 1] << 32) | (uint32_t)n_ptr[lo]); };
   const int64_t t_base[4] = {base_at(4), base_at(8), base_at(10), base_at(12)};
   const int64_t u_base = max(max(t_base[0], t_base[1]), max(t_base[2], t_base[3]));
-  const int chunk = (n - seg_beg + gridDim.x - 1) / gridDim.x;
-  const int beg = seg_beg + blockIdx.x * chunk, end = min(n, beg + chunk);
+  const int chunk = (n - seg_beg + nblk - 1) / nblk;
+  const int beg = seg_beg + bid * chunk, end = min(n, beg + chunk);
   int unsupported = 0, zero_ts = 0, events = 0, other = 0;
   uint32_t n_sel = 0;
   unsigned long long t_hi = 0;
   uint64_t tr[2] = {~0ull, 0ull};
   const uint32_t cur = cur_slot(o.cols);
   SigRec* const rec_out = o.cols.rec + (size_t)cur * (size_t)o.cols.stride;
-  __shared__ uint4 s_stage[NT * 5];
   const int lane = threadIdx.x & 63, wbase = threadIdx.x & ~63;
   const int trips = end > beg ? (end - beg + NT - 1) / NT : 0;
   int i = beg + threadIdx.x;
@@ -492,7 +500,7 @@
       }
       const unsigned long long m = __ballot(sel);
       if (lane == 0) {
-        o.sel_mask[(size_t)blockIdx.x * o.sel_stride + (size_t)it * (NT / 64) + (threadIdx.x >> 6)] = m;
+        o.sel_mask[(size_t)bid * o.sel_stride +(size_t)it * (NT / 64) + (threadIdx.x >> 6)] = m;
         n_sel += (uint32_t)__popcll(m);
       }
     }
@@ -526,17 +534,54 @@
       atomicMax(&s_t[2], (unsigned long long)tr[1]);
     }
   }
-  lds_flush<NT>(L, o, unsupported, zero_ts);
+  lds_flush<NT>(L, o, unsupported, zero_ts, bid);
   if (threadIdx.x == 0) {
     if (s_cnt2[0]) atomicAdd(&rs[kRsEvents], s_cnt2[0]);
     if (s_cnt2[1]) atomicAdd(&rs[kRsOtherShard], s_cnt2[1]);
-    if (o.sel_cnt) o.sel_cnt[blockIdx.x] = s_cnt2[2];
+    if (o.sel_cnt) o.sel_cnt[bid] = s_cnt2[2];
     if (s_t[0]) atomicMax(tmax, s_t[0]);
     if (o.cols.gen && s_t[1] <= s_t[2]) {
       atomicMin(reinterpret_cast<unsigned long long*>(&o.cols.gen->tlo[cur]), s_t[1]);
       atomicMax(reinterpret_cast<unsigned long long*>(&o.cols.gen->thi[cur]), s_t[2]);
     }
   }
+}
+
+template <int NT>
+__global__ __launch_bounds__(NT) void k_decode_window(const uint8_t* __restrict__ framed,
+                                                      const Event* __restrict__ user, const int* __restrict__ n_ptr,
+                                                      const int* __restrict__ rows, int cap,
+                                                      const SigRec* __restrict__ imp,
+                                                      const uint4* __restrict__ ctx_tab, int n_ctx, TraceIds tt,
+                                                      uint32_t* __restrict__ rs, unsigned long long* __restrict__ tmax,
+                                                      const uint32_t* __restrict__ pod_sn, uint32_t n_pods, int seg,
+                                                      int sh_rank, int sh_world, DecodeOut o) {
+  __shared__ uint4 s_stage[NT * 5];
+  decode_window_body<NT>(framed, user, n_ptr, rows, cap, imp, ctx_tab, n_ctx, tt, rs, tmax, pod_sn, n_pods, seg, sh_rank,
+                         sh_world, o, (int)blockIdx.x, (int)gridDim.x, s_stage);
+}
+
+template <int NT>
+__global__ __launch_bounds__(NT) void k_front_decode(const uint8_t* __restrict__ framed, const Event* __restrict__ user,
+                                                     const int* __restrict__ n_ptr, const int* __restrict__ rows,
+                                                     int cap, const SigRec* __restrict__ imp,
+                                                     const uint4* __restrict__ ctx_tab, int n_ctx, TraceIds tt,
+                                                     uint32_t* __restrict__ rs, unsigned long long* __restrict__ tmax,
+                                                     const uint32_t* __restrict__ pod_sn, uint32_t n_pods, int sh_rank,
+                                                     int sh_world, DecodeOut o, const uint32_t* __restrict__ s_part_blk,
+                                                     int s_nblk, uint32_t* __restrict__ s_part_off,
+                                                     uint32_t* __restrict__ s_part_tot) {
+  static_assert(NT == kScanCols * kScanRG, "the scan body's workgroup is the decode's");
+  static_assert(sizeof(uint4) * NT * 5 >= sizeof(uint32_t) * kScanRG * kScanCols, "the staging buffer holds the scan's sums");
+  __shared__ uint4 s_stage[NT * 5];
+  const FrontSlot fs = front_slot2((int)blockIdx.x, front_scan_blocks(), (int)gridDim.x);
+  if (fs.body == 0) {
+    part_scan_body(s_part_blk, s_nblk, s_part_off, s_part_tot, fs.bid,
+                   reinterpret_cast<uint32_t(*)[kScanCols]>(s_stage));
+    return;
+  }
+  decode_window_body<NT>(framed, user, n_ptr, rows, cap, imp, ctx_tab, n_ctx, tt, rs, tmax, pod_sn, n_pods, 0, sh_rank,
+                         sh_world, o, fs.bid, fs.nblk, s_stage);
 }
 
 template <int NT>
@@ -561,23 +606,26 @@
     const uint64_t ch = conn_hash(e.conn_src_port, e.conn_dst_port, e.conn_dst_ip);
     decode_one(i, cap, (int64_t)e.timestamp_ns, val, slot, trace_h, pod, e.pid, svcnode, ch, o, l, unsupported, zero_ts, i < n_local, o.cols.rec + i);
   }
-  lds_flush<NT>(L, o, unsupported, zero_ts);
+  lds_flush<NT>(L, o, unsupported, zero_ts, (int)blockIdx.x);
 }
 
 constexpr int kSliLds = 1024;
 
-template <int NT>
-__global__ __launch_bounds__(NT) void k_decode_spans(const void* __restrict__ sp_raw, const int* __restrict__ n_ptr,
-                                                     int cap, SpanCols c, uint32_t* part_cnt,
-                                                     const uint4* __restrict__ ctx_tab, int n_ctx, SpanMap sm) {
+constexpr int kSpanDecodeLds = kKeyTypes * kParts + 5 * kSliLds;
+
+template <int NT>
+__device__ __forceinline__ void decode_spans_body(const void* __restrict__ sp_raw, const int* __restrict__ n_ptr,
+                                                  int cap, const SpanCols& c, uint32_t* part_cnt,
+                                                  const uint4* __restrict__ ctx_tab, int n_ctx, const SpanMap& sm,
+                                                  int bid, int nblk, uint32_t* lds) {
   const Span* __restrict__ sp = static_cast<const Span*>(sp_raw);
   const SpanC20* __restrict__ sp20 = static_cast<const SpanC20*>(sp_raw);
   const bool compact = n_ptr[6] == 20;
   if (n_ptr[5] > 0) n_ctx = min(n_ptr[5], n_ctx);
-  __shared__ uint32_t s_part[kKeyTypes * kParts];
-  __shared__ uint32_t s_sli[2 * kSliLds];
-  __shared__ uint32_t s_app[2 * kSliLds];
-  __shared__ uint32_t s_late[kSliLds];
+  uint32_t* s_part = lds;
+  uint32_t* s_sli = s_part + kKeyTypes * kParts;
+  uint32_t* s_app = s_sli + 2 * kSliLds;
+  uint32_t* s_late = s_app + 2 * kSliLds;
   const bool sli_lds = sm.grp_sli && sm.n_groups <= kSliLds;
   const bool app_lds = sm.grp_app && sm.n_groups <= kSliLds;
   for (int i = threadIdx.x; i < kKeyTypes * kParts; i += NT) s_part[i] = 0;
@@ -590,8 +638,8 @@
     for (int i = threadIdx.x; i < sm.n_groups; i += NT) s_late[i] = 0;
   __syncthreads();
   const int n = min(*n_ptr, cap);
-  const int chunk = (n + gridDim.x - 1) / gridDim.x;
-  const int beg = blockIdx.x * chunk, end = min(n, beg + chunk);
+  const int chunk = (n + nblk - 1) / nblk;
+  const int beg = bid * chunk, end = min(n, beg + chunk);
   uint64_t t_lo = ~0ull, t_hi = 0ull;
   for (int i = beg + threadIdx.x; i < end; i += NT) {
     SpanRec r;
@@ -667,7 +715,7 @@
     }
   }
   __syncthreads();
-  store_counts<NT>(s_part, part_cnt + (size_t)blockIdx.x * kKeyTypes * kParts);
+  store_counts<NT>(s_part, part_cnt + (size_t)bid * kKeyTypes * kParts);
   if (sli_lds)
     for (int i = threadIdx.x; i < 2 * sm.n_groups; i += NT)
       if (s_sli[i]) atomicAdd(&sm.grp_sli[i], s_sli[i]);
@@ -679,6 +727,30 @@
       if (s_late[i]) atomicAdd(&sm.grp_late[2 * i], s_late[i]);
 }
 
+template <int NT>
+__global__ __launch_bounds__(NT) void k_decode_spans(const void* __restrict__ sp_raw, const int* __restrict__ n_ptr,
+                                                     int cap, SpanCols c, uint32_t* part_cnt,
+                                                     const uint4* __restrict__ ctx_tab, int n_ctx, SpanMap sm) {
+  __shared__ uint32_t s_lds[kSpanDecodeLds];
+  decode_spans_body<NT>(sp_raw, n_ptr, cap, c, part_cnt, ctx_tab, n_ctx, sm, (int)blockIdx.x, (int)gridDim.x, s_lds);
+}
+
+template <int NT>
+__global__ __launch_bounds__(NT) void k_front_defs_spans(const uint8_t* __restrict__ framed,
+                                                         const int* __restrict__ n_ptr, uint4* ctx_tab,
+                                                         uint32_t ctx_rows, const uint32_t* __restrict__ pod_sn,
+                                                         uint32_t n_pods, TraceIds tt, uint32_t* __restrict__ rs,
+                                                         const void* __restrict__ sp_raw, int s_cap, SpanCols c,
+                                                         uint32_t* s_part_cnt, int s_nblk, SpanMap sm) {
+  __shared__ uint32_t s_lds[kSpanDecodeLds];
+  const FrontSlot fs = front_slot2((int)blockIdx.x, s_nblk, (int)gridDim.x);
+  if (fs.body == 0) {
+    decode_spans_body<NT>(sp_raw, n_ptr + 1, s_cap, c, s_part_cnt, ctx_tab, (int)ctx_rows, sm, fs.bid, fs.nblk, s_lds);
+    return;
+  }
+  ring_defs_body<NT>(framed, n_ptr, ctx_tab, ctx_rows, pod_sn, n_pods, tt, rs, fs.bid, fs.nblk, s_lds);
+}
+
 constexpr int kDecodeNT = 1024;
 
 int decode_sel_stride(int cap) {
@@ -735,10 +807,29 @@
 void launch_ring_defs(const uint8_t* framed, const int* n_dev, int cap, uint32_t* ctx_tab, uint32_t ctx_rows,
                       const uint32_t* pod_sn, uint32_t n_pods, const TraceIds& tt, uint32_t* ring_state,
                       hipStream_t stream) {
-  int g = (cap + 1023) / 1024;
-  g = g < 1 ? 1 : (g > 2048 ? 2048 : g);
-  hipLaunchKernelGGL(k_ring_defs, dim3(g), dim3(256), 0, stream, framed, n_dev, reinterpret_cast<uint4*>(ctx_tab),
-                     ctx_rows, pod_sn, n_pods, tt, ring_state);
+  hipLaunchKernelGGL(k_ring_defs, dim3(ring_defs_grid(cap)), dim3(256), 0, stream, framed, n_dev,
+                     reinterpret_cast<uint4*>(ctx_tab), ctx_rows, pod_sn, n_pods, tt, ring_state);
+}
+
+void launch_front_defs_spans(const uint8_t* framed, const int* counts, int sig_cap, uint32_t* ctx_tab,
+                             uint32_t ctx_rows, const uint32_t* pod_sn, uint32_t n_pods, const TraceIds& tt,
+                             uint32_t* ring_state, const FrontSpans& fs, const SpanMap& sm, hipStream_t stream) {
+  hipLaunchKernelGGL((k_front_defs_spans<kFrontNT>), dim3(front_grid_defs_spans(fs.nblk, sig_cap)), dim3(kFrontNT), 0,
+                     stream, framed, counts, reinterpret_cast<uint4*>(ctx_tab), ctx_rows, pod_sn, n_pods, tt, ring_state,
+                     fs.sp, fs.cap, fs.cols, fs.part_blk, fs.nblk, sm);
+}
+
+void launch_front_decode(const uint8_t* framed, const void* user, const int* n_dev, const int* rows, int cap,
+                         const SigRec* imp, const uint32_t* ctx_tab, int n_ctx, const TraceIds& tt, uint32_t* ring_state,
+                         unsigned long long* tmax, const uint32_t* pod_sn, uint32_t n_pods, const SignalCols& cols,
+                         uint32_t* hist, uint32_t* status_cnt, uint32_t* part_cnt, unsigned long long* misc,
+                         int sh_rank, int sh_world, const FrontSpans& fs, hipStream_t stream) {
+  static_assert(kFrontNT == kDecodeNT, "the fused decode keeps the decode's workgroup");
+  DecodeOut o{cols, hist, status_cnt, part_cnt, misc};
+  hipLaunchKernelGGL((k_front_decode<kFrontNT>), dim3(front_grid_decode(kKeyTypes * kParts, decode_grid(cap))),
+                     dim3(kFrontNT), 0, stream, framed, (const Event*)user, n_dev, rows, cap, imp,
+                     reinterpret_cast<const uint4*>(ctx_tab), n_ctx, tt, ring_state, tmax, pod_sn, n_pods, sh_rank,
+                     sh_world, o, fs.part_blk, fs.nblk, fs.part_off, fs.part_tot);
 }
 
 void launch_decode_window(const uint8_t* framed, const void* user, const int* n_dev, const int* rows, int cap,
diff --git a/llm_slo_ebpf_toolkit_amd/ops/csrc/engine.h b/llm_slo_ebpf_toolkit_amd/ops/csrc/engine.h
--- a/llm_slo_ebpf_toolkit_amd/ops/csrc/engine.h
+++ b/llm_slo_ebpf_toolkit_amd/ops/csrc/engine.h
@@ -115,6 +115,8 @@
   ResultView results(int64_t k) const { return layout().view<const uint8_t>(bufs_[k % nb_].res_host); }
   ResultLayout layout() const { return ResultLayout{(size_t)cfg_.group_cap}; }
   std::pair<float, float> window_ms(int64_t k);
+  float front_ms(int64_t k);
+  bool front_fused() const { return front_fused_ && overlap_ && !branch_; }
   std::vector<float> copy_ms(int64_t k);
 
   void set_model_bytes(const void* bytes, size_t n);
@@ -169,6 +171,7 @@
   void run_join_back(const Buf& buf, int n_groups, bool with_labels, bool learn, hipStream_t st);
   void run_span_branch(const Buf& buf, hipStream_t st);
   void run_spans(const Buf& buf, hipStream_t st);
+  void run_front_fused(const Buf& buf, hipStream_t st);
   void launch_part(Stage part, const Buf& buf, int n_groups, bool with_labels, bool learn);
   void merge_remote(const Buf& buf, const uint8_t* blocks, size_t stride, int world, int me, hipStream_t st);
   void refit(const double* add);
@@ -219,6 +222,8 @@
   hipStream_t side_ = nullptr;
   hipStream_t front_ = nullptr;
   bool overlap_ = false;
+  bool front_fused_ = false;
+  bool front_timing_ = false;
   struct BufSet {
     GenMeta* gen;
     int* rows;
@@ -246,6 +251,7 @@
     const GenMeta* gen_prev;
     hipEvent_t head_done, front_done, compute_done, comm_done, xchg_done;
     hipEvent_t t_comp0, t_comp1, t_end;
+    hipEvent_t t_front1 = nullptr;
     const int* counts() const { return reinterpret_cast<const int*>(in); }
   };
   std::vector<Buf> bufs_;
diff --git a/llm_slo_ebpf_toolkit_amd/ops/csrc/engine.hip b/llm_slo_ebpf_toolkit_amd/ops/csrc/engine.hip
--- a/llm_slo_ebpf_toolkit_amd/ops/csrc/engine.hip
+++ b/llm_slo_ebpf_toolkit_amd/ops/csrc/engine.hip
@@ -191,6 +191,8 @@
   overlap_ = env_int("MISLO_WINDOW_OVERLAP", !one_stream) == 1 && !one_stream &&
              !(cfg_.xchg_cap > 0 && cfg_.import_cap > 0);
   if (overlap_) front_ = mk_stream();
+  front_fused_ = overlap_ && env_int("MISLO_FRONT_FUSED", 1) == 1;
+  front_timing_ = overlap_ && env_int("MISLO_FRONT_TIMING", 0) == 1;
   copy_ahead_ = overlap_ && env_int("MISLO_COPY_AHEAD", kCopyAheadDefault) == 1;
   const char* lanes_env = getenv("MISLO_COPY_LANES");
   lanes_ = overlap_ && (lanes_env ? atoi(lanes_env) == 2 : nb_ >= 4) ? 2 : 1;
@@ -216,6 +218,7 @@
     for (hipEvent_t* e : {&buf.head_done, &buf.compute_done, &buf.comm_done, &buf.front_done, &buf.xchg_done})
       *e = mk_event(kEvWait);
     for (hipEvent_t* e : {&buf.t_comp0, &buf.t_comp1, &buf.t_end}) *e = mk_event(hipEventDefault);
+    if (front_timing_) buf.t_front1 = mk_event(hipEventDefault);
     buf.res_host = static_cast<uint8_t*>(host_block(lay.bytes()));
     buf.res_dev = dalloc<uint8_t>(lay.bytes(), true);
     buf.res = lay.view(buf.res_dev);
@@ -499,6 +502,25 @@
   launch_span_sort(span_cols(buf), s.s_items, s.s_part_base, s.s_pre, st);
 }
 
+void WindowEngine::run_front_fused(const Buf& buf, hipStream_t st) {
+  const BufSet& s = *buf.set;
+  const int* counts = buf.counts();
+  const int N = n_rows_, S = cfg_.span_cap, G = cfg_.group_cap;
+  run_begin(buf, st);
+  const TraceIds tt{trace_hash_, kTraceIdRows};
+  const SpanMap sm{1, buf.res.sli, G, cfg_.ttft_slo_ms, cfg_.shard_rank, cfg_.shard_world,
+                   s.gen, buf.res.app, buf.res.late};
+  const FrontSpans fs{buf.in + off_span_, counts + 1, S, nblk_span_, span_cols(buf), s_part_blk_, s_part_off_,
+                      s_part_tot_, s.s_part_base, s.s_items, s.s_pre};
+  launch_front_defs_spans(buf.in + off_kern_, counts, cfg_.sig_cap, ctx_tab_, kCtxRows, pod_sn_, kPodRows, tt,
+                          s.ring_state, fs, sm, st);
+  launch_front_decode(buf.in + off_kern_, buf.in + off_user_, counts, s.rows, N, buf.imp, ctx_tab_, (int)kCtxRows, tt,
+                      s.ring_state, tmax_, pod_sn_, kPodRows, sig_cols(buf), s.hist, s.status, g_part_blk_, s.misc,
+                      rec_shard_rank(), rec_shard_world(), fs, st);
+  launch_front_join(sig_cols(buf), s.rows, N, nblk_sig_, g_part_blk_, g_part_off_, g_part_tot_, fs, jp_, s.probe_work,
+                    st);
+}
+
 void WindowEngine::run_span_branch(const Buf& buf, hipStream_t st) {
   HIPCHECK(hipEventRecord(ev_fork_, st));
   HIPCHECK(hipStreamWaitEvent(side_, ev_fork_, 0));
@@ -520,6 +542,7 @@
       case Stage::XchgSpans: return run_spans(buf, cs);
       case Stage::XchgHead: return run_begin(buf, cs);
       case Stage::Front:
+        if (front_fused()) return run_front_fused(buf, cs);
         run_part1(buf, cs, false);
         return run_join_front(buf, cs, false);
       case Stage::Back: return run_join_back(buf, n_groups, with_labels, learn, cs);
@@ -685,6 +708,7 @@
     if (xchg) throw std::logic_error("the exchange path does not run with overlapped windows");
     launch_part(Stage::Front, buf, n_groups, with_labels, learn);
     HIPCHECK(hipEventRecord(buf.front_done, front_));
+    if (front_timing_) HIPCHECK(hipEventRecord(buf.t_front1, front_));
     HIPCHECK(hipStreamWaitEvent(compute_, buf.front_done, 0));
     launch_part(Stage::Back, buf, n_groups, with_labels, learn);
   } else if (!xchg) {
@@ -775,6 +799,15 @@
   return {total, comp};
 }
 
+float WindowEngine::front_ms(int64_t k) {
+  const Buf& buf = bufs_[k % nb_];
+  if (!overlap_ || !front_timing_ || !buf.t_front1) return -1.f;
+  float ms = 0.f;
+  HIPCHECK(hipEventSynchronize(buf.t_front1));
+  HIPCHECK(hipEventElapsedTime(&ms, buf.t_comp0, buf.t_front1));
+  return ms;
+}
+
 void WindowEngine::set_model_bytes(const void* bytes, size_t n) {
   if (n != sizeof(PosteriorModel)) throw std::invalid_argument("model image must be POSTERIOR_MODEL_BYTES bytes");
   uint8_t* h = model_host_[model_slot_++ % model_host_.size()];
diff --git a/llm_slo_ebpf_toolkit_amd/ops/csrc/join.hip b/llm_slo_ebpf_toolkit_amd/ops/csrc/join.hip
--- a/llm_slo_ebpf_toolkit_amd/ops/csrc/join.hip
+++ b/llm_slo_ebpf_toolkit_amd/ops/csrc/join.hip
@@ -2,6 +2,7 @@
 
 #include "mislo_common.h"
 #include "mislo_launch.h"
+#include "mislo_scan.h"
 
 namespace mislo {
 
@@ -9,63 +10,46 @@
 constexpr int kChunk = 256;
 
 
-constexpr int kScanCols = 32, kScanRG = 32;
 __global__ __launch_bounds__(kScanCols * kScanRG) void k_part_scan(const uint32_t* __restrict__ part_blk, int nblk,
                                                                   uint32_t* __restrict__ part_off,
                                                                   uint32_t* __restrict__ part_tot) {
   __shared__ uint32_t s_sum[kScanRG][kScanCols];
-  const int cl = threadIdx.x % kScanCols, r = threadIdx.x / kScanCols;
-  const int c = blockIdx.x * kScanCols + cl;
-  const int per = (nblk + kScanRG - 1) / kScanRG;
-  const int b0 = min(nblk, r * per), b1 = min(nblk, b0 + per);
-  constexpr size_t W = (size_t)kKeyTypes * kParts;
-  uint32_t sum = 0;
-  for (int b = b0; b < b1; ++b) sum += part_blk[(size_t)b * W + c];
-  s_sum[r][cl] = sum;
-  __syncthreads();
-  uint32_t run = 0, tot = 0;
-  for (int q = 0; q < kScanRG; ++q) {
-    const uint32_t v = s_sum[q][cl];
-    run += q < r ? v : 0u;
-    tot += v;
-  }
-  for (int b = b0; b < b1; ++b) {
-    const size_t idx = (size_t)b * W + c;
-    const uint32_t v = part_blk[idx];
-    part_off[idx] = run;
-    run += v;
-  }
-  if (r == 0) part_tot[c] = tot;
-}
-
-constexpr int kBaseNT = kKeyTypes * kParts / 4;
+  part_scan_body(part_blk, nblk, part_off, part_tot, (int)blockIdx.x, s_sum);
+}
+
 __global__ __launch_bounds__(kBaseNT) void k_base_scan(const uint32_t* __restrict__ tot, uint32_t* __restrict__ base,
                                                       const GenMeta* __restrict__ gen) {
-  if (gen) base += (size_t)gen->cur * kBaseLen;
   __shared__ uint32_t s[kBaseNT];
-  const int t = threadIdx.x;
-  uint32_t v[4];
-  uint32_t sum = 0;
-#pragma unroll
-  for (int j = 0; j < 4; ++j) {
-    v[j] = tot[t * 4 + j];
-    sum += v[j];
-  }
-  s[t] = sum;
+  base_scan_body(tot, base, gen, s);
+}
+
+template <int NT>
+__device__ __forceinline__ void scatter_body(const PartCodes* __restrict__ codes, const int* __restrict__ n_ptr,
+                                             int cap, const uint32_t* __restrict__ part_off,
+                                             const uint32_t* __restrict__ base, uint32_t* __restrict__ items,
+                                             int nblk_a, int bid, int nblk, uint32_t* s_pos) {
+  {
+    const uint32_t* my_off = part_off + (size_t)bid * kKeyTypes * kParts;
+    for (int i = threadIdx.x; i < kKeyTypes * kParts; i += NT) s_pos[i] = base[i] + my_off[i];
+  }
   __syncthreads();
-  for (int off = 1; off < kBaseNT; off <<= 1) {
-    uint32_t x = t >= off ? s[t - off] : 0;
-    __syncthreads();
-    s[t] += x;
-    __syncthreads();
-  }
-  uint32_t run = s[t] - sum;
-#pragma unroll
-  for (int j = 0; j < 4; ++j) {
-    base[t * 4 + j] = run;
-    run += v[j];
-  }
-  if (t == kBaseNT - 1) base[kKeyTypes * kParts] = s[kBaseNT - 1];
+  const int n0 = min(n_ptr[0], cap);
+  const bool two = nblk_a < nblk;
+  const bool second = two && bid >= nblk_a;
+  const int s_beg = second ? n0 : 0;
+  const int s_end = second ? max(n0, min(n_ptr[1], cap)) : n0;
+  const int g = two ? (second ? nblk - nblk_a : nblk_a) : nblk;
+  const int bi = second ? bid - nblk_a : bid;
+  const int chunk = (s_end - s_beg + g - 1) / g;
+  const int beg = s_beg + bi * chunk, end = min(s_end, beg + chunk);
+  for (int i = beg + threadIdx.x; i < end; i += NT) {
+    const PartCodes pc = codes[i];
+#pragma unroll
+    for (int k = 0; k < kKeyTypes; ++k) {
+      if (pc.p[k] == kNoPart) continue;
+      items[atomicAdd(&s_pos[k * kParts + pc.p[k]], 1u)] = (uint32_t)i;
+    }
+  }
 }
 
 template <int NT>
@@ -74,28 +58,7 @@
                                                 const uint32_t* __restrict__ base, uint32_t* __restrict__ items,
                                                 int nblk_a) {
   __shared__ uint32_t s_pos[kKeyTypes * kParts];
-  {
-    const uint32_t* my_off = part_off + (size_t)blockIdx.x * kKeyTypes * kParts;
-    for (int i = threadIdx.x; i < kKeyTypes * kParts; i += NT) s_pos[i] = base[i] + my_off[i];
-  }
-  __syncthreads();
-  const int n0 = min(n_ptr[0], cap);
-  const bool two = nblk_a < (int)gridDim.x;
-  const bool second = two && (int)blockIdx.x >= nblk_a;
-  const int s_beg = second ? n0 : 0;
-  const int s_end = second ? max(n0, min(n_ptr[1], cap)) : n0;
-  const int g = two ? (second ? (int)gridDim.x - nblk_a : nblk_a) : (int)gridDim.x;
-  const int bi = second ? (int)blockIdx.x - nblk_a : (int)blockIdx.x;
-  const int chunk = (s_end - s_beg + g - 1) / g;
-  const int beg = s_beg + bi * chunk, end = min(s_end, beg + chunk);
-  for (int i = beg + threadIdx.x; i < end; i += NT) {
-    const PartCodes pc = codes[i];
-#pragma unroll
-    for (int k = 0; k < kKeyTypes; ++k) {
-      if (pc.p[k] == kNoPart) continue;
-      items[atomicAdd(&s_pos[k * kParts + pc.p[k]], 1u)] = (uint32_t)i;
-    }
-  }
+  scatter_body<NT>(codes, n_ptr, cap, part_off, base, items, nblk_a, (int)blockIdx.x, (int)gridDim.x, s_pos);
 }
 
 template <int NT>
@@ -486,6 +449,34 @@
       store_prespan(out + c0 + i, s_kt[i].h, s_kt[i].t, rr, my_s, rid | (s_ok[rid] << 16));
     }
   }
+}
+
+
+__global__ __launch_bounds__(kFrontNT) void k_front_scan(const uint32_t* __restrict__ part_blk, int nblk,
+                                                         uint32_t* __restrict__ part_off,
+                                                         uint32_t* __restrict__ part_tot,
+                                                         const uint32_t* __restrict__ s_tot,
+                                                         uint32_t* __restrict__ s_base) {
+  static_assert(kScanCols * kScanRG == kFrontNT && kBaseNT == kFrontNT, "one workgroup size for both bodies");
+  __shared__ uint32_t s_sum[kScanRG][kScanCols];
+  const FrontSlot fs = front_slot2((int)blockIdx.x, 1, (int)gridDim.x);
+  if (fs.body == 0) return base_scan_body(s_tot, s_base, nullptr, &s_sum[0][0]);
+  part_scan_body(part_blk, nblk, part_off, part_tot, fs.bid, s_sum);
+}
+
+template <int NT>
+__global__ __launch_bounds__(NT) void k_front_base_scatter(const uint32_t* __restrict__ tot, uint32_t* __restrict__ base,
+                                                           const GenMeta* __restrict__ gen,
+                                                           const PartCodes* __restrict__ s_codes,
+                                                           const int* __restrict__ s_n_ptr, int s_cap,
+                                                           const uint32_t* __restrict__ s_part_off,
+                                                           const uint32_t* __restrict__ s_base,
+                                                           uint32_t* __restrict__ s_items) {
+  static_assert(NT == kBaseNT && kBaseNT <= kKeyTypes * kParts, "the scan's sums fit the scatter's array");
+  __shared__ uint32_t s_pos[kKeyTypes * kParts];
+  const FrontSlot fs = front_slot2((int)blockIdx.x, 1, (int)gridDim.x);
+  if (fs.body == 0) return base_scan_body(tot, base, gen, s_pos);
+  scatter_body<NT>(s_codes, s_n_ptr, s_cap, s_part_off, s_base, s_items, fs.nblk, fs.bid, fs.nblk, s_pos);
 }
 
 template <int NT, bool LG>
@@ -1024,6 +1015,21 @@
                      items, nblk_a > 0 && nblk_a < nblk ? nblk_a : nblk);
 }
 
+void launch_front_join(const SignalCols& gc, const int* rows, int cap, int nblk_sig, const uint32_t* part_blk,
+                       uint32_t* part_off, uint32_t* part_tot, const FrontSpans& fs, const JoinParams& jp,
+                       uint32_t* work, hipStream_t stream) {
+  constexpr int kLists = kKeyTypes * kParts;
+  hipLaunchKernelGGL(k_front_scan, dim3(front_grid_scan(kLists)), dim3(kFrontNT), 0, stream, part_blk, nblk_sig,
+                     part_off, part_tot, fs.part_tot, fs.part_base);
+  hipLaunchKernelGGL((k_front_base_scatter<kFrontNT>), dim3(front_grid_base_scatter(fs.nblk)), dim3(kFrontNT), 0,
+                     stream, part_tot, gc.base, gc.gen, fs.cols.part, fs.n_dev, fs.cap, fs.part_off, fs.part_base,
+                     fs.items);
+  hipLaunchKernelGGL((k_scatter_sig_work<1024>), dim3(nblk_sig + 1), dim3(1024), 0, stream, gc, rows, cap, part_off,
+                     nblk_sig, fs.part_base, jp, probe_item_signals(), work);
+  hipLaunchKernelGGL((k_span_sort<kChunk>), dim3(kLists), dim3(kChunk), 0, stream, fs.cols, fs.items, fs.part_base,
+                     fs.pre);
+}
+
 void launch_probe(const SpanCols& sc, const uint32_t* span_items, const uint32_t* span_base, const SignalCols& gc,
                   int span_cap, const JoinParams& jp, unsigned long long* top3, uint32_t* cnt, int n_groups,
                   unsigned long long* gsum, uint32_t* gcnt, unsigned long long* dbg, uint32_t* work,
diff --git a/llm_slo_ebpf_toolkit_amd/ops/csrc/mislo_front.h b/llm_slo_ebpf_toolkit_amd/ops/csrc/mislo_front.h
--- /dev/null
+++ b/llm_slo_ebpf_toolkit_amd/ops/csrc/mislo_front.h
@@ -0,0 +1,38 @@
+#pragma once
+
+#include <cstddef>
+#include <cstdint>
+
+#if defined(__HIPCC__) || defined(__CUDACC__)
+#define MISLO_FRONT_HD __host__ __device__
+#else
+#define MISLO_FRONT_HD
+#endif
+
+namespace mislo {
+
+constexpr int kFrontNT = 1024;
+constexpr int kScanCols = 32, kScanRG = 32;
+
+struct FrontSlot {
+  int body, bid, nblk;
+};
+
+MISLO_FRONT_HD inline FrontSlot front_slot2(int block, int n_first, int grid) {
+  return block < n_first ? FrontSlot{0, block, n_first} : FrontSlot{1, block - n_first, grid - n_first};
+}
+
+inline int ring_defs_grid(int cap) {
+  int g = (cap + 1023) / 1024;
+  return g < 1 ? 1 : (g > 2048 ? 2048 : g);
+}
+inline int ring_defs_grid_wide(int cap) { return (ring_defs_grid(cap) * 256 + kFrontNT - 1) / kFrontNT; }
+
+constexpr int front_scan_grid(int lists) { return lists / kScanCols; }
+
+inline int front_grid_defs_spans(int nblk_span, int sig_cap) { return nblk_span + ring_defs_grid_wide(sig_cap); }
+inline int front_grid_decode(int lists, int nblk_sig) { return front_scan_grid(lists) + nblk_sig; }
+inline int front_grid_scan(int lists) { return 1 + front_scan_grid(lists); }
+inline int front_grid_base_scatter(int nblk_span) { return 1 + nblk_span; }
+
+}
diff --git a/llm_slo_ebpf_toolkit_amd/ops/csrc/mislo_launch.h b/llm_slo_ebpf_toolkit_amd/ops/csrc/mislo_launch.h
--- a/llm_slo_ebpf_toolkit_amd/ops/csrc/mislo_launch.h
+++ b/llm_slo_ebpf_toolkit_amd/ops/csrc/mislo_launch.h
@@ -122,6 +122,27 @@
 constexpr int kProbePhaseItems = kMaxGens * kParts * kProbeMaxSplit;
 constexpr int kProbeProfOff = 4 + 4 * kProbePhaseItems;
 constexpr int kProbeWorkLen = kProbeProfOff + 64;
+struct FrontSpans {
+  const void* sp;
+  const int* n_dev;
+  int cap, nblk;
+  SpanCols cols;
+  uint32_t *part_blk, *part_off, *part_tot;
+  uint32_t *part_base, *items;
+  PreSpan* pre;
+};
+void launch_front_defs_spans(const uint8_t* framed, const int* counts, int sig_cap, uint32_t* ctx_tab,
+                             uint32_t ctx_rows, const uint32_t* pod_sn, uint32_t n_pods, const TraceIds& tt,
+                             uint32_t* ring_state, const FrontSpans& fs, const SpanMap& sm, hipStream_t stream);
+void launch_front_decode(const uint8_t* framed, const void* user, const int* n_dev, const int* rows, int cap,
+                         const SigRec* imp, const uint32_t* ctx_tab, int n_ctx, const TraceIds& tt, uint32_t* ring_state,
+                         unsigned long long* tmax, const uint32_t* pod_sn, uint32_t n_pods, const SignalCols& cols,
+                         uint32_t* hist, uint32_t* status_cnt, uint32_t* part_cnt, unsigned long long* misc,
+                         int sh_rank, int sh_world, const FrontSpans& fs, hipStream_t stream);
+void launch_front_join(const SignalCols& gc, const int* rows, int cap, int nblk_sig, const uint32_t* part_blk,
+                       uint32_t* part_off, uint32_t* part_tot, const FrontSpans& fs, const JoinParams& jp,
+                       uint32_t* work, hipStream_t stream);
+
 void launch_finalize(const int* ns_dev, int span_cap, const unsigned long long* top3, const uint32_t* cnt,
                      const SignalCols& gc, const SpanCols& sc, const JoinParams& jp, const float* base_attrs,
                      float* attrs, float* conf, float* kernel_ms, int n_groups, unsigned long long* gsum, uint32_t* gcnt,
diff --git a/llm_slo_ebpf_toolkit_amd/ops/csrc/mislo_scan.h b/llm_slo_ebpf_toolkit_amd/ops/csrc/mislo_scan.h
--- /dev/null
+++ b/llm_slo_ebpf_toolkit_amd/ops/csrc/mislo_scan.h
@@ -0,0 +1,66 @@
+#pragma once
+
+#include "mislo_common.h"
+#include "mislo_front.h"
+
+namespace mislo {
+
+constexpr int front_scan_blocks() { return front_scan_grid(kKeyTypes * kParts); }
+
+__device__ __forceinline__ void part_scan_body(const uint32_t* __restrict__ part_blk, int nblk,
+                                               uint32_t* __restrict__ part_off, uint32_t* __restrict__ part_tot,
+                                               int bid, uint32_t (*s_sum)[kScanCols]) {
+  const int cl = threadIdx.x % kScanCols, r = threadIdx.x / kScanCols;
+  const int c = bid * kScanCols + cl;
+  const int per = (nblk + kScanRG - 1) / kScanRG;
+  const int b0 = min(nblk, r * per), b1 = min(nblk, b0 + per);
+  constexpr size_t W = (size_t)kKeyTypes * kParts;
+  uint32_t sum = 0;
+  for (int b = b0; b < b1; ++b) sum += part_blk[(size_t)b * W + c];
+  s_sum[r][cl] = sum;
+  __syncthreads();
+  uint32_t run = 0, tot = 0;
+  for (int q = 0; q < kScanRG; ++q) {
+    const uint32_t v = s_sum[q][cl];
+    run += q < r ? v : 0u;
+    tot += v;
+  }
+  for (int b = b0; b < b1; ++b) {
+    const size_t idx = (size_t)b * W + c;
+    const uint32_t v = part_blk[idx];
+    part_off[idx] = run;
+    run += v;
+  }
+  if (r == 0) part_tot[c] = tot;
+}
+
+constexpr int kBaseNT = kKeyTypes * kParts / 4;
+__device__ __forceinline__ void base_scan_body(const uint32_t* __restrict__ tot, uint32_t* __restrict__ base,
+                                               const GenMeta* __restrict__ gen, uint32_t* s) {
+  if (gen) base += (size_t)gen->cur * kBaseLen;
+  const int t = threadIdx.x;
+  uint32_t v[4];
+  uint32_t sum = 0;
+#pragma unroll
+  for (int j = 0; j < 4; ++j) {
+    v[j] = tot[t * 4 + j];
+    sum += v[j];
+  }
+  s[t] = sum;
+  __syncthreads();
+  for (int off = 1; off < kBaseNT; off <<= 1) {
+    uint32_t x = t >= off ? s[t - off] : 0;
+    __syncthreads();
+    s[t] += x;
+    __syncthreads();
+  }
+  uint32_t run = s[t] - sum;
+#pragma unroll
+  for (int j = 0; j < 4; ++j) {
+    base[t * 4 + j] = run;
+    run += v[j];
+  }
+  if (t == kBaseNT - 1) base[kKeyTypes * kParts] = s[kBaseNT - 1];
+}
+
+}
```
